# hdelan/MSc-HPC-Final-Project

Measured on AMD Instinct MI355X. Metric: lanczos_iterations_per_sec, higher is better.
Workload: dtype f64

## Files before the change

### msc-hpc-final-project_amd/__init__.py

```python
from __future__ import annotations

import ctypes
import os

import numpy as np

_HERE = os.path.dirname(os.path.abspath(__file__))
LIB_PATH = os.path.join(_HERE, "liblzx.so")
DBG_LIB_PATH = os.path.join(_HERE, "liblzx_dbg.so")
PRODUCT_OPTIONS = ("hub_entries", "propagation_blocking", "overlap_exchange", "sparse_exchange", "exchange_fp32",
                   "lazy_normalisation", "timing_marks_every", "reorthogonalise", "basis_fp32", "reference_order", "placement_trials",
                   "sharded_ingest", "operator")

SHAPE_OPTIONS = ("pb_reduce", "pb_target", "pb_unit", "pb_column_band", "pb_run_align", "pb_taper", "pb_dyn_share", "pb_carry_scan", "pb_scatter_nt", "pb_gather_grid", "pb_gather_nt", "spmv_wgs", "pb_group", "pb_group_force",
                 "narrow_slices", "tie_sort", "long_row", "item_len", "exchange_at_world_1", "isolated_rows", "unnormalised_basis", "fuse_staged", "start_vector_scan", "defer_finish",
                 "multi_row_chunk", "eig_basis_bytes", "solve_state_bytes", "solve_poll", "bfs_state_bytes", "tri_long_list", "tri_state_bytes", "core_long_row", "core_state_bytes",
                 "truss_long_row", "truss_state_bytes", "color_long_row", "lpa_group_row", "lpa_table_row", "lpa_state_bytes")

LZX_COLOR_TIES_BY_ID = 1

_u64p = ctypes.POINTER(ctypes.c_uint64)
_u32p = ctypes.POINTER(ctypes.c_uint32)
_i32p = ctypes.POINTER(ctypes.c_int32)
_u8p = ctypes.POINTER(ctypes.c_uint8)
_f64p = ctypes.POINTER(ctypes.c_double)
_h = ctypes.c_void_p
_hp = ctypes.POINTER(ctypes.c_void_p)


class LzxStats(ctypes.Structure):
    _fields_ = [("loop_ms", ctypes.c_double), ("spmv_ms", ctypes.c_double),
                ("spmv_ms_min", ctypes.c_double), ("vec_ms", ctypes.c_double),
                ("comm_ms", ctypes.c_double), ("iters", ctypes.c_uint32),
                ("spmv_kernels", ctypes.c_uint32), ("spmv_bytes", ctypes.c_uint64)]

    def as_dict(self):
        return {f: getattr(self, f) for f, _ in self._fields_}


class LzxGraphInfo(ctypes.Structure):
    _fields_ = [("n", ctypes.c_uint64), ("nnz", ctypes.c_uint64), ("max_degree", ctypes.c_uint64),
                ("rows_local", ctypes.c_uint64), ("nnz_local", ctypes.c_uint64),
                ("long_rows", ctypes.c_uint64), ("sell_padded", ctypes.c_uint64),
                ("pb_entries", ctypes.c_uint64), ("active_vertices", ctypes.c_uint64),
                ("exchange_slice", ctypes.c_uint64), ("hub_entries", ctypes.c_uint32), ("world", ctypes.c_uint32), ("rank", ctypes.c_uint32),
                ("reserved_", ctypes.c_uint32), ("pb_values", ctypes.c_uint64), ("pb_reduced_entries", ctypes.c_uint64),
                ("exchange_chunk0", ctypes.c_uint64), ("exchange_recv", ctypes.c_uint64),
                ("placement_tried", ctypes.c_uint32), ("placement_kept", ctypes.c_uint32), ("placement_us", ctypes.c_uint32 * 8)]

    def as_dict(self):
        d = {f: getattr(self, f) for f, _ in self._fields_}
        d["placement_us"] = list(d["placement_us"])[:d["placement_tried"]]
        return d


class LzxEigInfo(ctypes.Structure):
    _fields_ = [("converged", ctypes.c_uint32), ("restarts", ctypes.c_uint32), ("matvecs", ctypes.c_uint32), ("m", ctypes.c_uint32),
                ("loop_ms", ctypes.c_double), ("spmv_ms", ctypes.c_double), ("orth_ms", ctypes.c_double), ("host_ms", ctypes.c_double),
                ("norm_est", ctypes.c_double)]

    def as_dict(self):
        return {f: getattr(self, f) for f, _ in self._fields_}


class LzxSolveInfo(ctypes.Structure):
    _fields_ = [("iterations", ctypes.c_uint32), ("launched", ctypes.c_uint32), ("converged", ctypes.c_uint32), ("ns", ctypes.c_uint32),
                ("loop_ms", ctypes.c_double), ("spmv_ms", ctypes.c_double), ("vec_ms", ctypes.c_double), ("bnorm", ctypes.c_double)]

    def as_dict(self):
        return {f: getattr(self, f) for f, _ in self._fields_}


class LzxSolveMultiInfo(ctypes.Structure):
    _fields_ = [("iterations", ctypes.c_uint32), ("launched", ctypes.c_uint32), ("converged", ctypes.c_uint32), ("nb", ctypes.c_uint32),
                ("loop_ms", ctypes.c_double), ("spmv_ms", ctypes.c_double), ("vec_ms", ctypes.c_double), ("bnorm", ctypes.c_double * 16)]

    def as_dict(self):
        d = {f: getattr(self, f) for f, _ in self._fields_}
        d["bnorm"] = np.array(list(d["bnorm"])[:d["nb"]])
        return d


class LzxPagerankInfo(ctypes.Structure):
    _fields_ = [("iterations", ctypes.c_uint32), ("launched", ctypes.c_uint32), ("converged", ctypes.c_uint32), ("nd", ctypes.c_uint32),
                ("loop_ms", ctypes.c_double), ("spmv_ms", ctypes.c_double), ("vec_ms", ctypes.c_double), ("mass", ctypes.c_double * 16)]

    def as_dict(self):
        d = {f: getattr(self, f) for f, _ in self._fields_}
        d["mass"] = np.array(list(d["mass"])[:d["nd"]])
        return d


class LzxComponentsInfo(ctypes.Structure):
    _fields_ = [("n_components", ctypes.c_uint64), ("largest_size", ctypes.c_uint64), ("largest_label", ctypes.c_uint32),
                ("rounds", ctypes.c_uint32), ("loop_ms", ctypes.c_double), ("sweep_ms", ctypes.c_double)]

    def as_dict(self):
        return {f: getattr(self, f) for f, _ in self._fields_}


class LzxBfsInfo(ctypes.Structure):
    _fields_ = [("ns", ctypes.c_uint32), ("batches", ctypes.c_uint32), ("max_level", ctypes.c_uint32), ("sweeps", ctypes.c_uint32),
                ("loop_ms", ctypes.c_double), ("sweep_ms", ctypes.c_double)]

    def as_dict(self):
        return {f: getattr(self, f) for f, _ in self._fields_}


class LzxTrianglesInfo(ctypes.Structure):
    _fields_ = [("triangles", ctypes.c_uint64), ("wedges", ctypes.c_uint64), ("max_triangles", ctypes.c_uint64),
                ("oriented_entries", ctypes.c_uint64), ("oriented_max_degree", ctypes.c_uint32), ("reserved_", ctypes.c_uint32),
                ("avg_clustering", ctypes.c_double), ("loop_ms", ctypes.c_double), ("orient_ms", ctypes.c_double), ("count_ms", ctypes.c_double)]

    def as_dict(self):
        return {f: getattr(self, f) for f, _ in self._fields_ if f != "reserved_"}


class LzxCoreInfo(ctypes.Structure):
    _fields_ = [("main_core_size", ctypes.c_uint64), ("core0", ctypes.c_uint64), ("degeneracy", ctypes.c_uint32), ("levels", ctypes.c_uint32),
                ("rounds", ctypes.c_uint32), ("reserved_", ctypes.c_uint32), ("loop_ms", ctypes.c_double), ("peel_ms", ctypes.c_double)]

    def as_dict(self):
        return {f: getattr(self, f) for f, _ in self._fields_ if f != "reserved_"}


class LzxTrussInfo(ctypes.Structure):
    _fields_ = [("edges", ctypes.c_uint64), ("triangles", ctypes.c_uint64), ("main_truss_edges", ctypes.c_uint64),
                ("max_support", ctypes.c_uint32), ("max_truss", ctypes.c_uint32), ("levels", ctypes.c_uint32), ("rounds", ctypes.c_uint32),
                ("loop_ms", ctypes.c_double), ("support_ms", ctypes.c_double), ("peel_ms", ctypes.c_double)]

    def as_dict(self):
        return {f: getattr(self, f) for f, _ in self._fields_}


class LzxColorInfo(ctypes.Structure):
    _fields_ = [("colors", ctypes.c_uint32), ("rounds", ctypes.c_uint32), ("largest_class", ctypes.c_uint32), ("reserved_", ctypes.c_uint32),
                ("loop_ms", ctypes.c_double), ("color_ms", ctypes.c_double)]

    def as_dict(self):
        return {f: getattr(self, f) for f, _ in self._fields_ if f != "reserved_"}


class LzxCommunitiesInfo(ctypes.Structure):
    _fields_ = [("n_communities", ctypes.c_uint64), ("largest_size", ctypes.c_uint64), ("updates", ctypes.c_uint64),
                ("inner_entries", ctypes.c_uint64), ("entries", ctypes.c_uint64), ("sum_degree_sq", ctypes.c_uint64),
                ("largest_label", ctypes.c_uint32), ("sweeps", ctypes.c_uint32), ("colors", ctypes.c_uint32), ("color_rounds", ctypes.c_uint32),
                ("modularity", ctypes.c_double), ("loop_ms", ctypes.c_double), ("color_ms", ctypes.c_double), ("sweep_ms", ctypes.c_double)]

    def as_dict(self):
        return {f: getattr(self, f) for f, _ in self._fields_}


class LzxModularityInfo(ctypes.Structure):
    _fields_ = [("communities", ctypes.c_uint64), ("inner_entries", ctypes.c_uint64), ("entries", ctypes.c_uint64),
                ("sum_degree_sq", ctypes.c_uint64), ("loop_ms", ctypes.c_double)]

    def as_dict(self):
        return {f: getattr(self, f) for f, _ in self._fields_}


SYMBOLS = [
    ("lzx_create", ctypes.c_int, [_hp, ctypes.c_int]),
    ("lzx_destroy", None, [_h]),
    ("lzx_last_error", ctypes.c_char_p, []),
    ("lzx_comm_unique_id", ctypes.c_int, [_u8p]),
    ("lzx_comm_init_rank", ctypes.c_int, [_h, _u8p, ctypes.c_int, ctypes.c_int]),
    ("lzx_comm_init_local", ctypes.c_int, [_hp, ctypes.c_int]),
    ("lzx_create_group", ctypes.c_int, [_hp, ctypes.c_int, ctypes.POINTER(ctypes.c_int)]),
    ("lzx_comm_ipc_export", ctypes.c_int, [_h, _u8p]),
    ("lzx_comm_ipc_init", ctypes.c_int, [_h, _u8p, ctypes.c_int, ctypes.c_int]),
    ("lzx_set_graph_csr", ctypes.c_int, [_h, ctypes.c_uint64, ctypes.c_uint64, _u64p, _u32p]),
    ("lzx_set_graph_csr32", ctypes.c_int, [_h, ctypes.c_uint32, ctypes.c_uint32, _u32p, _u32p]),
    ("lzx_set_graph_edges", ctypes.c_int, [_h, ctypes.c_uint64, ctypes.c_uint64, _u32p, _u32p]),
    ("lzx_gen_graph", ctypes.c_int, [_h, ctypes.c_int, ctypes.c_uint32, ctypes.c_uint64, ctypes.c_uint64,
                                     ctypes.c_uint64, ctypes.c_uint32, ctypes.c_uint32, ctypes.c_uint32]),
    ("lzx_get_graph_info", ctypes.c_int, [_h, ctypes.POINTER(LzxGraphInfo)]),
    ("lzx_get_graph_csr", ctypes.c_int, [_h, _u64p, _u32p]),
    ("lzx_spmv_f64", ctypes.c_int, [_h, _f64p, _f64p]),
    ("lzx_spmv_f64_local", ctypes.c_int, [_hp, ctypes.c_int, _f64p, _f64p]),
    ("lzx_lanczos_f64", ctypes.c_int, [_h, _f64p, ctypes.c_uint32, _f64p, _f64p, _f64p, _f64p,
                                       ctypes.POINTER(LzxStats)]),
    ("lzx_lanczos_f64_local", ctypes.c_int, [_hp, ctypes.c_int, _f64p, ctypes.c_uint32, _f64p, _f64p, _f64p,
                                             _f64p, ctypes.POINTER(LzxStats)]),
    ("lzx_lanczos_prepare_f64", ctypes.c_int, [_h, _f64p, ctypes.c_uint32, _f64p]),
    ("lzx_lanczos_run", ctypes.c_int, [_h, ctypes.POINTER(LzxStats)]),
    ("lzx_lanczos_fetch_f64", ctypes.c_int, [_h, ctypes.c_uint32, _f64p, _f64p, _f64p]),
    ("lzx_lanczos_fetch_f64_local", ctypes.c_int, [_hp, ctypes.c_int, ctypes.c_uint32, _f64p, _f64p, _f64p]),
    ("lzx_lanczos_run_steps", ctypes.c_int, [_h, ctypes.c_uint32, ctypes.POINTER(LzxStats)]),
    ("lzx_lanczos_run_steps_local", ctypes.c_int, [_hp, ctypes.c_int, ctypes.c_uint32, ctypes.POINTER(LzxStats)]),
    ("lzx_lanczos_prepare_f64_local", ctypes.c_int, [_hp, ctypes.c_int, _f64p, ctypes.c_uint32, _f64p]),
    ("lzx_lanczos_progress", ctypes.c_int, [_h, _u32p, _u32p]),
    ("lzx_multout_change_f64", ctypes.c_int, [_h, _f64p, ctypes.c_uint32, _f64p]),
    ("lzx_multout_change_f64_local", ctypes.c_int, [_hp, ctypes.c_int, _f64p, ctypes.c_uint32, _f64p]),
    ("lzx_device_count", ctypes.c_int, [ctypes.POINTER(ctypes.c_int)]),
    ("lzx_sync", ctypes.c_int, [_h]),
    ("lzx_multout_f64", ctypes.c_int, [_h, _f64p, ctypes.c_uint32, _f64p]),
    ("lzx_multout_f64_local", ctypes.c_int, [_hp, ctypes.c_int, _f64p, ctypes.c_uint32, _f64p]),
    ("lzx_bench_spmv", ctypes.c_int, [_h, ctypes.c_uint32, _f64p, _f64p]),
    ("lzx_bench_stream", ctypes.c_int, [_h, ctypes.c_uint64, ctypes.c_uint32, _f64p, _f64p]),
    ("lzx_set_option", ctypes.c_int, [_h, ctypes.c_char_p, ctypes.c_int64]),
    ("lzx_lanczos_multi_f64", ctypes.c_int, [_h, ctypes.c_uint32, _f64p, ctypes.c_uint32, _f64p, _f64p, _u32p, _f64p, _f64p,
                                             ctypes.POINTER(LzxStats)]),
    ("lzx_multout_multi_f64", ctypes.c_int, [_h, ctypes.c_uint32, _f64p, ctypes.c_uint32, _f64p]),
    ("lzx_spmm_f64", ctypes.c_int, [_h, ctypes.c_uint32, _f64p, _f64p]),
    ("lzx_multi_release", ctypes.c_int, [_h]),
    ("lzx_probes_f64", ctypes.c_int, [_h, ctypes.c_uint64, ctypes.c_uint64, ctypes.c_uint32, _f64p]),
    ("lzx_lanczos_probes_f64", ctypes.c_int, [_h, ctypes.c_uint64, ctypes.c_uint64, ctypes.c_uint32, ctypes.c_uint32, ctypes.c_uint32,
                                              _f64p, _f64p, _u32p, ctypes.POINTER(LzxStats)]),
    ("lzx_probe_diag_f64", ctypes.c_int, [_h, _f64p, ctypes.c_uint32, _f64p]),
    ("lzx_eigsh_f64", ctypes.c_int, [_h, ctypes.c_uint32, ctypes.c_int, ctypes.c_uint32, ctypes.c_double, ctypes.c_uint32, _f64p,
                                     ctypes.c_uint64, _f64p, ctypes.c_uint32, _f64p, _f64p, _f64p, ctypes.POINTER(LzxEigInfo)]),
    ("lzx_solve_shifted_f64", ctypes.c_int, [_h, _f64p, ctypes.c_uint32, _f64p, ctypes.c_double, ctypes.c_uint32, _f64p, ctypes.c_uint32,
                                             _f64p, _u32p, _f64p, ctypes.POINTER(LzxSolveInfo)]),
    ("lzx_solve_multi_f64", ctypes.c_int, [_h, ctypes.c_uint32, _f64p, _f64p, ctypes.c_double, ctypes.c_uint32, _f64p, ctypes.c_uint32,
                                           _f64p, _u32p, _f64p, _u32p, ctypes.POINTER(LzxSolveMultiInfo)]),
    ("lzx_pagerank_f64", ctypes.c_int, [_h, _f64p, ctypes.c_uint32, _f64p, ctypes.c_double, ctypes.c_uint32, _f64p, _u32p, _f64p,
                                        ctypes.POINTER(LzxPagerankInfo)]),
    ("lzx_components", ctypes.c_int, [_h, _u32p, ctypes.POINTER(LzxComponentsInfo)]),
    ("lzx_set_graph_induced", ctypes.c_int, [_h, _h, _u8p, _u32p, _u64p]),
    ("lzx_bfs_multi", ctypes.c_int, [_h, ctypes.c_uint32, _u32p, _i32p, _f64p, _u64p, _u64p, _f64p, _u32p, ctypes.POINTER(LzxBfsInfo)]),
    ("lzx_betweenness_f64", ctypes.c_int, [_h, ctypes.c_uint32, _u32p, _f64p, ctypes.POINTER(LzxBfsInfo)]),
    ("lzx_triangles", ctypes.c_int, [_h, _u64p, _f64p, ctypes.POINTER(LzxTrianglesInfo)]),
    ("lzx_core_numbers", ctypes.c_int, [_h, _u32p, _u32p, ctypes.POINTER(LzxCoreInfo)]),
    ("lzx_truss", ctypes.c_int, [_h, _u32p, _u32p, _u32p, _u32p, ctypes.POINTER(LzxTrussInfo)]),
    ("lzx_color", ctypes.c_int, [_h, ctypes.c_uint64, ctypes.c_uint32, _u32p, ctypes.POINTER(LzxColorInfo)]),
    ("lzx_label_propagation", ctypes.c_int, [_h, ctypes.c_uint64, ctypes.c_uint32, ctypes.c_uint32, _u32p, ctypes.POINTER(LzxCommunitiesInfo)]),
    ("lzx_modularity", ctypes.c_int, [_h, _u32p, _f64p, ctypes.POINTER(LzxModularityInfo)]),
]

_LIB = None
_DBG_LIB = None


class LzxError(RuntimeError):
    pass


def _load(path: str, mode: int) -> ctypes.CDLL:
    if not os.path.exists(path):
        raise LzxError(f"{path} is missing: run __graft_entry__.build() (make -C {_HERE})")
    L = ctypes.CDLL(path, mode=mode)
    for name, res, args in SYMBOLS:
        fn = getattr(L, name)
        fn.restype = res
        fn.argtypes = args
    L.lzx_test_set_shape.restype = ctypes.c_int
    L.lzx_test_set_shape.argtypes = [_h, ctypes.c_char_p, ctypes.c_int64]
    L.lzx_test_get_shape.restype = ctypes.c_int
    L.lzx_test_get_shape.argtypes = [_h, ctypes.c_char_p, ctypes.POINTER(ctypes.c_int64)]
    L.lzx_test_allreduce_latency.restype = ctypes.c_int
    L.lzx_test_allreduce_latency.argtypes = [_h, ctypes.c_uint32, ctypes.POINTER(ctypes.c_double)]
    L.lzx_test_rank_row_sums.restype = ctypes.c_int
    L.lzx_test_rank_row_sums.argtypes = [_h, _f64p, _u32p, _u64p]
    L.lzx_test_sym_eig.restype = ctypes.c_int
    L.lzx_test_sym_eig.argtypes = [ctypes.c_uint32, _f64p, _f64p, _f64p]
    L.lzx_test_eig_ops.restype = ctypes.c_int
    L.lzx_test_eig_ops.argtypes = [_h, ctypes.c_uint32, ctypes.c_uint32, _f64p, _f64p, _f64p, _f64p, _f64p, _f64p, _f64p]
    return L


def lib(debug: bool = False) -> ctypes.CDLL:
    global _LIB, _DBG_LIB
    if debug:
        if _DBG_LIB is None:
            _DBG_LIB = _load(DBG_LIB_PATH, ctypes.RTLD_LOCAL)
        return _DBG_LIB
    if _LIB is None:
        _LIB = _load(LIB_PATH, ctypes.RTLD_GLOBAL)
    return _LIB


def _p(a, ty):
    return a.ctypes.data_as(ty)


def _check(rc: int, what: str, L=None):
    if rc != 0:
        raise LzxError(f"{what} failed ({rc}): {(L or lib()).lzx_last_error().decode(errors='replace')}")


OP_ADJACENCY = 0
OP_LAPLACIAN = 1


def _expm_coefficients(alpha, beta, x_norm, s):
    k = len(alpha)
    kb = k
    zero = np.flatnonzero(np.asarray(beta[:k - 1]) == 0.0)
    if zero.size:
        kb = int(zero[0]) + 1
    T = np.diag(np.asarray(alpha[:kb], dtype=np.float64))
    if kb > 1:
        T += np.diag(beta[:kb - 1], 1) + np.diag(beta[:kb - 1], -1)
    lam, V = np.linalg.eigh(T)
    t = np.zeros(k)
    t[:kb] = V @ (np.exp(s * lam) * (x_norm * V[0, :]))
    return t


PROBE_KEEP_BASIS = 1
EIG_LARGEST = 0
EIG_SMALLEST = 1
ERR_LIMIT = -6
PROBE_BATCH = 16


def _probe_ritz(alpha, beta, m):
    T = np.diag(np.asarray(alpha[:m], dtype=np.float64))
    if m > 1:
        T += np.diag(beta[:m - 1], 1) + np.diag(beta[:m - 1], -1)
    return np.linalg.eigh(T)


def _logsumexp(x):
    m = x.max()
    return m + np.log(np.sum(np.exp(x - m)))

# ... 886 lines not shown
```

### msc-hpc-final-project_amd/csrc/lzx_api.hip

```cpp
#include <algorithm>
#include <atomic>
#include <chrono>
#include <cmath>
#include <cstdlib>
#include <cstring>
#include <string>
#include <thread>

#include "lzx_internal.h"

static thread_local std::string g_err;

void lzx_set_error(const char *fmt, ...)
{
    char buf[1024];
    va_list ap;
    va_start(ap, fmt);
    vsnprintf(buf, sizeof buf, fmt, ap);
    va_end(ap);
    g_err = buf;
}

extern "C" const char *lzx_last_error(void) { return g_err.c_str(); }

extern "C" int lzx_create(lzx_handle *out, int device_id)
{
    if (!out) LZX_FAIL(LZX_ERR_ARG, "lzx_create: null out");
    *out = nullptr;
    int count = 0;
    LZX_HIP(hipGetDeviceCount(&count));
    if (device_id < 0 || device_id >= count)
        LZX_FAIL(LZX_ERR_ARG, "lzx_create: device %d not present (%d visible)", device_id, count);
    LZX_HIP(hipSetDevice(device_id));
    lzx_ctx *c = new (std::nothrow) lzx_ctx;
    if (!c) LZX_FAIL(LZX_ERR_NOMEM, "lzx_create: host allocation failed");
    c->device = device_id;
    hipDeviceProp_t prop;
    hipError_t e = hipGetDeviceProperties(&prop, device_id);
    if (e == hipSuccess) e = hipStreamCreateWithFlags(&c->stream, hipStreamNonBlocking);
    if (e == hipSuccess) e = hipEventCreate(&c->ev_a);
    if (e == hipSuccess) e = hipEventCreate(&c->ev_b);
    if (e == hipSuccess) e = hipEventCreateWithFlags(&c->ev_phase, hipEventDisableTiming);
    if (e == hipSuccess) e = hipStreamCreateWithFlags(&c->stream2, hipStreamNonBlocking);
    if (e == hipSuccess) e = hipEventCreateWithFlags(&c->ev_phase2, hipEventDisableTiming);
    if (e == hipSuccess) e = hipStreamCreateWithFlags(&c->stream3, hipStreamNonBlocking);
    if (e == hipSuccess) e = hipEventCreateWithFlags(&c->ev_fork, hipEventDisableTiming);
    if (e == hipSuccess) e = hipEventCreateWithFlags(&c->ev_join, hipEventDisableTiming);
    if (e == hipSuccess) e = hipEventCreateWithFlags(&c->ev_q, hipEventDisableTiming);
    if (e == hipSuccess) e = hipEventCreateWithFlags(&c->ev_c0, hipEventDisableTiming);
    if (e == hipSuccess) e = hipEventCreateWithFlags(&c->ev_c1, hipEventDisableTiming);
    if (e == hipSuccess) e = hipMalloc(reinterpret_cast<void **>(&c->d_scal), sizeof(double) * (8 + 64));
    if (e != hipSuccess) {
        lzx_set_error("lzx_create: %s", hipGetErrorString(e));
        lzx_destroy(c);
        return LZX_ERR_HIP;
    }
    c->cu_count = prop.multiProcessorCount > 0 ? prop.multiProcessorCount : 256;
    *out = c;
    return LZX_OK;
}

extern "C" void lzx_destroy(lzx_handle c)
{
    if (!c) return;
    (void)hipSetDevice(c->device);
    if (c->stream) (void)hipStreamSynchronize(c->stream);
    lzx_graph_release(c);
    lzx_comm_release(c);
    if (c->d_alpha) (void)hipFree(c->d_alpha);
    if (c->d_beta) (void)hipFree(c->d_beta);
    if (c->d_scal) (void)hipFree(c->d_scal);
    if (c->d_iso) (void)hipFree(c->d_iso);
    if (c->d_Qf) (void)hipFree(c->d_Qf);
    for (double *&r : c->d_ring) { if (r) (void)hipFree(r); r = nullptr; }
    for (double *&r : c->d_ymon) { if (r) (void)hipFree(r); r = nullptr; }
    for (hipEvent_t ev : c->ev_pool) (void)hipEventDestroy(ev);
    for (hipEvent_t ev : {c->ev_a, c->ev_b, c->ev_phase, c->ev_phase2, c->ev_fork, c->ev_join, c->ev_q, c->ev_c0, c->ev_c1})
        if (ev) (void)hipEventDestroy(ev);
    if (c->stream2) { (void)hipStreamSynchronize(c->stream2); (void)hipStreamDestroy(c->stream2); }
    if (c->stream3) { (void)hipStreamSynchronize(c->stream3); (void)hipStreamDestroy(c->stream3); }
    if (c->stream) (void)hipStreamDestroy(c->stream);
    delete c;
}

enum : unsigned { OPT_PRODUCT = 1, OPT_KNOB = 2, OPT_SHAPE = 4, OPT_LOOP = 8 };
struct Option {
    const char *name;
    int64_t lzx_ctx::*field;
    unsigned flags;
};
static const Option g_options[] = {
    {"hub_entries", &lzx_ctx::hub_opt, OPT_PRODUCT},
    {"propagation_blocking", &lzx_ctx::pb_opt, OPT_PRODUCT},
    {"overlap_exchange", &lzx_ctx::overlap_opt, OPT_PRODUCT},
    {"lazy_normalisation", &lzx_ctx::lazy_opt, OPT_PRODUCT},
    {"sparse_exchange", &lzx_ctx::sparse_opt, OPT_PRODUCT},
    {"exchange_fp32", &lzx_ctx::xfp32_opt, OPT_PRODUCT},
    {"timing_marks_every", &lzx_ctx::marks_every_opt, OPT_PRODUCT},
    {"reorthogonalise", &lzx_ctx::reorth_opt, OPT_PRODUCT | OPT_LOOP},
    {"basis_fp32", &lzx_ctx::qf32_opt, OPT_PRODUCT | OPT_LOOP},
    {"reference_order", &lzx_ctx::ref_order_opt, OPT_PRODUCT | OPT_LOOP},
    {"operator", &lzx_ctx::op_opt, OPT_PRODUCT | OPT_LOOP},
    {"placement_trials", &lzx_ctx::place_opt, OPT_PRODUCT},
    {"sharded_ingest", &lzx_ctx::shard_opt, OPT_PRODUCT},
    {"pb_reduce", &lzx_ctx::pb_reduce_opt, OPT_SHAPE | OPT_KNOB},
    {"pb_target", &lzx_ctx::pb_target_opt, OPT_SHAPE | OPT_KNOB},
    {"pb_unit", &lzx_ctx::pb_unit_opt, OPT_SHAPE | OPT_KNOB},
    {"pb_column_band", &lzx_ctx::pb_cb_opt, OPT_SHAPE | OPT_KNOB},
    {"pb_run_align", &lzx_ctx::pb_align_opt, OPT_SHAPE | OPT_KNOB},
    {"pb_taper", &lzx_ctx::pb_taper_opt, OPT_SHAPE | OPT_KNOB},
    {"pb_dyn_share", &lzx_ctx::pb_dyn_opt, OPT_SHAPE | OPT_KNOB},
    {"pb_carry_scan", &lzx_ctx::pb_scan_opt, OPT_SHAPE},
    {"pb_scatter_nt", &lzx_ctx::pb_scatter_nt_opt, OPT_SHAPE},
    {"pb_gather_grid", &lzx_ctx::pb_grid_cap_opt, OPT_SHAPE | OPT_KNOB},
    {"pb_gather_nt", &lzx_ctx::pb_gather_nt_opt, OPT_SHAPE | OPT_KNOB},
    {"spmv_wgs", &lzx_ctx::spmv_wgs_opt, OPT_SHAPE | OPT_KNOB},
    {"pb_group", &lzx_ctx::pb_group_opt, OPT_SHAPE | OPT_KNOB},
    {"pb_group_force", &lzx_ctx::pb_group_force_opt, OPT_SHAPE | OPT_KNOB},
    {"narrow_slices", &lzx_ctx::narrow_opt, OPT_SHAPE | OPT_KNOB},
    {"tie_sort", &lzx_ctx::tie_sort_opt, OPT_SHAPE | OPT_KNOB},
    {"long_row", &lzx_ctx::long_row_opt, OPT_SHAPE | OPT_KNOB},
    {"item_len", &lzx_ctx::item_opt, OPT_SHAPE | OPT_KNOB},
    {"exchange_at_world_1", nullptr, OPT_SHAPE | OPT_KNOB},
    {"isolated_rows", &lzx_ctx::iso_opt, OPT_SHAPE | OPT_KNOB},
    {"unnormalised_basis", &lzx_ctx::basis_u_opt, OPT_SHAPE | OPT_KNOB},
    {"fuse_staged", &lzx_ctx::fuse_opt, OPT_SHAPE | OPT_KNOB},
    {"start_vector_scan", &lzx_ctx::x0_scan_opt, OPT_SHAPE | OPT_KNOB},
    {"defer_finish", &lzx_ctx::defer_opt, OPT_SHAPE | OPT_KNOB},
    {"multi_row_chunk", &lzx_ctx::multi_chunk_opt, OPT_SHAPE},
    {"eig_basis_bytes", &lzx_ctx::eig_basis_cap_opt, OPT_SHAPE},
    {"solve_state_bytes", &lzx_ctx::solve_cap_opt, OPT_SHAPE},
    {"solve_poll", &lzx_ctx::solve_poll_opt, OPT_SHAPE},
    {"bfs_state_bytes", &lzx_ctx::bfs_cap_opt, OPT_SHAPE},
    {"tri_long_list", &lzx_ctx::tri_long_opt, OPT_SHAPE},
    {"tri_state_bytes", &lzx_ctx::tri_cap_opt, OPT_SHAPE},
    {"core_long_row", &lzx_ctx::core_long_opt, OPT_SHAPE},
    {"core_state_bytes", &lzx_ctx::core_cap_opt, OPT_SHAPE},
    {"truss_long_row", &lzx_ctx::truss_long_opt, OPT_SHAPE},
    {"truss_state_bytes", &lzx_ctx::truss_cap_opt, OPT_SHAPE},
    {"color_long_row", &lzx_ctx::color_long_opt, OPT_SHAPE},
    {"lpa_group_row", &lzx_ctx::lpa_group_opt, OPT_SHAPE},
    {"lpa_table_row", &lzx_ctx::lpa_table_opt, OPT_SHAPE},
    {"lpa_state_bytes", &lzx_ctx::lpa_cap_opt, OPT_SHAPE},
#ifdef LZX_DEBUG_KNOBS
    {"wgs_per_cu", &lzx_ctx::wgs_per_cu_opt, OPT_KNOB},
    {"nt_index_loads", &lzx_ctx::nt_opt, OPT_KNOB},
    {"side_stream", &lzx_ctx::side_opt, OPT_KNOB},
    {"pb_stamps", &lzx_ctx::pb_stamps_opt, OPT_KNOB},
    {"pb_order", &lzx_ctx::pb_order_opt, OPT_KNOB},
    {"spmv_deep", &lzx_ctx::deep_opt, OPT_KNOB},
    {"stage_burst", &lzx_ctx::burst_opt, OPT_KNOB},
    {"vec_blocks_per_cu", &lzx_ctx::vec_per_cu_opt, OPT_KNOB},
    {"pb_gather_waves", &lzx_ctx::pb_gwaves_opt, OPT_KNOB},
    {"phase_mask", &lzx_ctx::phase_mask_opt, OPT_KNOB},
#endif
};

static const Option *find_option(const char *name, unsigned accepted)
{
    for (const Option &o : g_options)
        if ((o.flags & accepted) && !strcmp(name, o.name)) return &o;
    return nullptr;
}

static void store_option(lzx_ctx *c, const Option &o, int64_t value)
{
    if (!o.field) c->force_multi = value > 0;
    else if (o.field == &lzx_ctx::shard_opt) c->shard_opt = value < 0 ? 0 : value;
    else c->*o.field = value;
}

extern "C" int lzx_set_option(lzx_handle c, const char *name, int64_t value)
{
    if (!c || !name) LZX_FAIL(LZX_ERR_ARG, "lzx_set_option: bad argument");
#ifdef LZX_DEBUG_KNOBS
    const Option *o = find_option(name, OPT_PRODUCT | OPT_KNOB);
#else
    const Option *o = find_option(name, OPT_PRODUCT);
#endif
    const bool loop_option = o && (o->flags & OPT_LOOP);
    if (o && o->field == &lzx_ctx::op_opt && value != LZX_OP_ADJACENCY && value != LZX_OP_LAPLACIAN)
        LZX_FAIL(LZX_ERR_ARG, "lzx_set_option: operator must be LZX_OP_ADJACENCY (0) or LZX_OP_LAPLACIAN (1), got %lld", (long long)value);
    if (c->d_row_ptr && !loop_option) LZX_FAIL(LZX_ERR_STATE, "options must be set before the graph is handed over");
    if (!o) LZX_FAIL(LZX_ERR_ARG, "lzx_set_option: unknown option '%s'", name);
    if (loop_option) c->k_prep = 0;
    store_option(c, *o, value);
    return LZX_OK;
}

extern "C" int lzx_test_set_shape(lzx_handle c, const char *name, int64_t value)
{
    if (!c || !name) LZX_FAIL(LZX_ERR_ARG, "lzx_test_set_shape: bad argument");
    if (c->d_row_ptr) LZX_FAIL(LZX_ERR_STATE, "shapes must be set before the graph is handed over");
    const Option *o = find_option(name, OPT_SHAPE);
    if (!o) LZX_FAIL(LZX_ERR_ARG, "lzx_test_set_shape: unknown shape '%s'", name);
    store_option(c, *o, value);
    return LZX_OK;
}

extern "C" int lzx_test_get_shape(lzx_handle c, const char *name, int64_t *value)
{
    if (!c || !name || !value) LZX_FAIL(LZX_ERR_ARG, "lzx_test_get_shape: bad argument");
    if (!strcmp(name, "gather_items_dealt")) *value = c->pb ? c->pb_n_static : 0;
    else if (!strcmp(name, "gather_items_drawn")) *value = c->pb ? c->pb_n_dyn : 0;
    else if (!strcmp(name, "gather_workgroups")) *value = c->pb ? c->pb_gather_grid : 0;
    else if (!strcmp(name, "placement_tried")) *value = c->place_tried;
    else if (!strcmp(name, "placement_kept")) *value = c->place_kept;
    else if (!strcmp(name, "start_vector_was_constant")) *value = c->x0_was_constant ? 1 : 0;
    else if (!strcmp(name, "finish_deferrable")) *value = c->pb && c->pb_defer_ok ? 1 : 0;
    else if (!strcmp(name, "finish_launched")) *value = c->pb && c->pb_finish_grid ? 1 : 0;
    else if (!strncmp(name, "placement_us_", 13) && name[13] >= '0' && name[13] <= '7' && !name[14]) *value = (int64_t)(c->place_ms[name[13] - '0'] * 1e3f);
    else LZX_FAIL(LZX_ERR_ARG, "lzx_test_get_shape: unknown shape '%s'", name);
    return LZX_OK;
}

extern "C" int lzx_test_allreduce_latency(lzx_handle c, uint32_t reps, double *us_each)
{
    if (!c || !us_each || reps == 0) LZX_FAIL(LZX_ERR_ARG, "lzx_test_allreduce_latency: bad argument");
    if (c->comm_kind < 2 || !lzx_exchanges(c)) LZX_FAIL(LZX_ERR_STATE, "lzx_test_allreduce_latency: needs a one-process-per-rank communicator");
    std::vector<lzx_ctx *> cs(1, c);
    LZX_HIP(hipSetDevice(c->device));
    LZX_HIP(hipMemsetAsync(c->d_scal, 0, sizeof(double) * 2, c->stream));
    for (u32 i = 0; i < 5; ++i) LZX_TRY(lzx_comm_allreduce_sum(cs, 0, 2));
    LZX_HIP(hipEventRecord(c->ev_a, c->stream));
    for (u32 i = 0; i < reps; ++i) LZX_TRY(lzx_comm_allreduce_sum(cs, 0, 2));
    LZX_HIP(hipEventRecord(c->ev_b, c->stream));
    LZX_HIP(hipStreamSynchronize(c->stream));
    LZX_TRY(lzx_comm_ipc_check(c));
    float ms = 0.f;
    LZX_HIP(hipEventElapsedTime(&ms, c->ev_a, c->ev_b));
    *us_each = (double)ms * 1e3 / reps;
    return LZX_OK;
}

extern "C" int lzx_test_rank_row_sums(lzx_handle c, double *v_local, uint32_t *layout_pos, uint64_t *n_loc_pad)
{
    if (!c || !v_local || !layout_pos || !n_loc_pad) LZX_FAIL(LZX_ERR_ARG, "lzx_test_rank_row_sums: bad argument");
    if (!c->d_row_ptr || !c->d_v) LZX_FAIL(LZX_ERR_STATE, "no graph has been handed over");
    double avg = 0.0;
    LZX_TRY(lzx_bench_spmv(c, 1, &avg, nullptr));
    LZX_HIP(hipSetDevice(c->device));
    LZX_HIP(hipMemcpy(v_local, c->d_v, sizeof(double) * c->n_loc_real, hipMemcpyDeviceToHost));
    LZX_HIP(hipMemcpy(layout_pos, c->d_gidx_of_old, sizeof(u32) * c->n, hipMemcpyDeviceToHost));
    *n_loc_pad = c->n_loc_pad;
    return LZX_OK;
}

static int gather_handles(lzx_handle h, std::vector<lzx_ctx *> &cs)
{
    if (!h) LZX_FAIL(LZX_ERR_ARG, "null handle");
    if (h->comm_kind == 1 && h->world > 1)
        LZX_FAIL(LZX_ERR_STATE, "handle belongs to an in-process communicator: use the *_local entry point");
    cs.assign(1, h);
    return LZX_OK;
}

static int gather_handles_local(lzx_handle *hs, int world, std::vector<lzx_ctx *> &cs)
{
    if (!hs || world < 1) LZX_FAIL(LZX_ERR_ARG, "bad handle list");
    cs.clear();
    for (int p = 0; p < world; ++p) {
        if (!hs[p]) LZX_FAIL(LZX_ERR_ARG, "null handle in list");
        if (hs[p]->world != world || hs[p]->rank != p || (world > 1 && hs[p]->comm_kind != 1))
            LZX_FAIL(LZX_ERR_STATE, "handles are not wired as an in-process communicator of %d", world);
        cs.push_back(hs[p]);
    }
    return LZX_OK;
}

static int check_graphs(std::vector<lzx_ctx *> &cs)
{
    for (lzx_ctx *c : cs) {
        if (!c->d_row_ptr || !c->d_v) LZX_FAIL(LZX_ERR_STATE, "no graph has been handed over");
        if (c->n != cs[0]->n || c->nnz != cs[0]->nnz) LZX_FAIL(LZX_ERR_STATE, "handles hold different graphs");
    }
    if (cs.size() > 1 && cs[0]->comm_kind == 1) LZX_TRY(lzx_comm_check_sparse_local(cs));
    return LZX_OK;
}

static int sync_all(std::vector<lzx_ctx *> &cs)
{
    for (lzx_ctx *c : cs) {
        LZX_HIP(hipSetDevice(c->device));
        LZX_HIP(hipStreamSynchronize(c->stream));
        LZX_HIP(hipStreamSynchronize(c->stream2));
        LZX_TRY(lzx_comm_ipc_check(c));
    }
    return LZX_OK;
}

template <class T>
static void drop(T *&buf, u32 &count)
{
    if (buf) (void)hipFree(buf);
    buf = nullptr;
    count = 0;
}

static int ensure_capacity(lzx_ctx *c, u32 k, bool qf32)
{
    LZX_HIP(hipSetDevice(c->device));
    if (k > c->k_cap) {
        drop(c->d_alpha, c->k_cap);
        drop(c->d_beta, c->k_cap);
        LZX_HIP(hipMalloc(reinterpret_cast<void **>(&c->d_alpha), sizeof(double) * k));
        LZX_HIP(hipMalloc(reinterpret_cast<void **>(&c->d_beta), sizeof(double) * k));
        c->k_cap = k;
    }
    if (qf32) {
        drop(c->d_Q, c->q_cols);
        if (k > c->qf_cols) {
            drop(c->d_Qf, c->qf_cols);
            LZX_HIP(hipMalloc(reinterpret_cast<void **>(&c->d_Qf), sizeof(float) * (size_t)k * c->ldq));
            c->qf_cols = k;
        }
        for (double *&r : c->d_ring)
            if (!r) LZX_HIP(hipMalloc(reinterpret_cast<void **>(&r), sizeof(double) * c->ldq));
        return LZX_OK;
    }
    drop(c->d_Qf, c->qf_cols);
    for (double *&r : c->d_ring) { if (r) (void)hipFree(r); r = nullptr; }
    if (k > c->q_cols) {
        drop(c->d_Q, c->q_cols);
        LZX_HIP(hipMalloc(reinterpret_cast<void **>(&c->d_Q), sizeof(double) * (size_t)k * c->ldq));
        c->q_cols = k;
    }
    return LZX_OK;
}

static bool loop_is_lazy(const lzx_ctx *c0)
{
    if (c0->reorth_opt > 0) return false;
    if (c0->ref_order_opt > 0) return false;
    if (c0->qf32_opt > 0 && c0->lazy_opt != 0) return true;
    return c0->lazy_opt > 0 || (c0->lazy_opt < 0 && (lzx_exchanges(c0) || c0->codes16));
}
static inline double *basis_col(const lzx_ctx *c, u32 j)
{
    return c->qf32 ? c->d_ring[j % 3] : c->d_Q + (size_t)j * c->ldq;
}

enum { CAT_NONE = 0, CAT_SPMV = 1, CAT_VEC = 2, CAT_COMM = 3 };
struct Marks {
    lzx_ctx *c;
    size_t used = 0;
    std::vector<int> cat;
    bool on = true;
    u32 sampled = 0;
    int begin_iteration(u32 j, u32 every)
    {
        on = every <= 1 || j % every == 0;
        if (on) ++sampled;
        return tick(CAT_NONE);
    }
    int tick(int category)
    {
        if (!on) return LZX_OK;
        LZX_HIP(hipSetDevice(c->device));
        if (used == c->ev_pool.size()) {
            hipEvent_t ev;
            LZX_HIP(hipEventCreate(&ev));
            c->ev_pool.push_back(ev);
        }
        LZX_HIP(hipEventRecord(c->ev_pool[used], c->stream));
        cat.push_back(category);
        ++used;
        return LZX_OK;
    }
};

static u64 spmv_algorithmic_bytes(const lzx_ctx *c)
{
    return 4ull * c->nnz_local + 4ull * ((u64)c->n_loc_real + 1) + 8ull * c->n + 8ull * c->n_loc_real;
}

struct X0Scan {
    bool constant = false, exact = false;
    double sum_sq = 0.0;
};
static X0Scan scan_start_vector(const double *x0, u64 n)
{
    X0Scan out;
    if (n == 0) return out;
    const u32 hw = std::max(1u, std::thread::hardware_concurrency());
    const u32 T = (u32)std::min<u64>(std::min<u32>(8u, hw), n / (1u << 18) + 1);
    std::vector<double> part(T, 0.0);
    std::atomic<bool> all_const{true}, all_int{true};
    const double first = x0[0];
    auto work = [&](u32 t) {
        const u64 a = n * t / T, b = n * (t + 1) / T;
        double acc[4] = {0.0, 0.0, 0.0, 0.0};
        bool cst = true, itg = true;
        for (u64 i0 = a; i0 < b; i0 += 4096) {
            const u64 i1 = std::min<u64>(b, i0 + 4096);
            u64 i = i0;
            for (; i + 4 <= i1; i += 4) {
#pragma unroll
                for (int u = 0; u < 4; ++u) {
                    const double v = x0[i + u];
                    cst &= v == first;
                    const bool small = std::fabs(v) <= 67108864.0;
                    itg &= small && (double)(int64_t)(small ? v : 0.0) == v;
                    acc[u] += v * v;
                }
            }
            for (; i < i1; ++i) {
                const double v = x0[i];
                cst &= v == first;
                const bool small = std::fabs(v) <= 67108864.0;
                itg &= small && (double)(int64_t)(small ? v : 0.0) == v;
                acc[0] += v * v;
            }
            if (!cst) all_const.store(false, std::memory_order_relaxed);
            if (!itg) all_int.store(false, std::memory_order_relaxed);
            if (!all_const.load(std::memory_order_relaxed) && !all_int.load(std::memory_order_relaxed)) return;
        }
        part[t] = (acc[0] + acc[1]) + (acc[2] + acc[3]);
    };
    {
        std::vector<std::thread> th;
        for (u32 t = 1; t < T; ++t) th.emplace_back(work, t);
        work(0);
        for (auto &t : th) t.join();
    }
    out.constant = all_const.load();
    if (all_int.load()) {
        double s = 0.0;
        for (u32 t = 0; t < T; ++t) s += part[t];
        if (s < 9007199254740992.0) {
            out.exact = true;
            out.sum_sq = s;
        }
    }
    return out;
}

static int lanczos_prepare(std::vector<lzx_ctx *> &cs, const double *x0, u32 k, double *x_norm_out)
{
    if (!x0 || k == 0) LZX_FAIL(LZX_ERR_ARG, "lzx_lanczos: bad argument");
    LZX_TRY(check_graphs(cs));
    lzx_ctx *c0 = cs[0];
    const u64 n = c0->n;
    const bool multi = lzx_exchanges(c0);
    const bool lazy = loop_is_lazy(c0);
    static const bool trace = getenv("LZX_TRACE_PREPARE") != nullptr;
    auto t_last = std::chrono::steady_clock::now();
    auto lap = [&](const char *what) {
        if (!trace) return;
        for (lzx_ctx *c : cs) { (void)hipSetDevice(c->device); (void)hipStreamSynchronize(c->stream); }
        const auto t = std::chrono::steady_clock::now();
        fprintf(stderr, "[lzx prepare] %-34s %8.3f ms\n", what, std::chrono::duration<double, std::milli>(t - t_last).count());
        t_last = t;
    };
    for (lzx_ctx *c : cs) {
        if (c->reorth_opt != c0->reorth_opt || c->qf32_opt != c0->qf32_opt) LZX_FAIL(LZX_ERR_STATE, "handles carry different loop options");
        if (c->qf32_opt > 0 && c->op_opt == LZX_OP_LAPLACIAN)
            LZX_FAIL(LZX_ERR_STATE, "basis_fp32 stores the unnormalised basis, which operator laplacian does not keep (its breakdown stop leaves beta = 0 to divide by)");
        if (c->qf32_opt > 0 && (!lazy || c->basis_u_opt == 0))
            LZX_FAIL(LZX_ERR_STATE, "basis_fp32 needs the lazy loop (not with lazy_normalisation = 0, not together with reorthogonalise)");
        if (c->ref_order_opt > 0 && (multi || cs.size() > 1))
            LZX_FAIL(LZX_ERR_STATE, "option reference_order runs on one rank");
        if (c->ref_order_opt > 0 && c->qf32_opt > 0)
            LZX_FAIL(LZX_ERR_STATE, "option reference_order keeps the fp64 basis (not together with basis_fp32)");
        if (c->op_opt != c0->op_opt) LZX_FAIL(LZX_ERR_STATE, "handles carry different operators");
        if (c->op_opt == LZX_OP_LAPLACIAN) LZX_TRY(lzx_ensure_degrees(c));
    }
    for (lzx_ctx *c : cs) {
        c->k_prep = 0;
        c->k_last = c->k_done = 0;
        c->ymon_valid = 0;
        c->qf32 = false;
    }
    const bool want_qf32 = c0->qf32_opt > 0;
    for (lzx_ctx *c : cs) LZX_TRY(ensure_capacity(c, k, want_qf32));
    for (lzx_ctx *c : cs) c->qf32 = want_qf32;
    lap("checks, basis sized");

    const X0Scan scan = c0->x0_scan_opt != 0 ? scan_start_vector(x0, n) : X0Scan{};
    lap("look at x0");
    double ss = scan.sum_sq;
    struct Joiner {
        std::thread t;
        ~Joiner() { if (t.joinable()) t.join(); }
    } norm_thread;
    if (!scan.exact)
        norm_thread.t = std::thread([&ss, x0, n]() {
            double acc = 0.0;
            for (u64 i = 0; i < n; ++i) acc += x0[i] * x0[i];
            ss = acc;
        });

    for (lzx_ctx *c : cs) {
        LZX_HIP(hipSetDevice(c->device));
        if (c->qf32) {
            for (double *r : c->d_ring) LZX_HIP(hipMemsetAsync(r, 0, sizeof(double) * c->ldq, c->stream));
        } else {
            LZX_HIP(hipMemsetAsync(c->d_Q, 0, sizeof(double) * c->ldq, c->stream));
            if (k > 1)
                LZX_HIP(hipMemset2DAsync(c->d_Q + c->ldq + c->n_loc_pad, sizeof(double) * c->ldq, 0, sizeof(double) * LZX_TAIL, k - 1, c->stream));
        }
        if (scan.constant) LZX_TRY(lzx_launch_fill(c, c->d_io, x0[0], n));
        else LZX_HIP(hipMemcpyAsync(c->d_io, x0, sizeof(double) * n, hipMemcpyHostToDevice, c->stream));
        c->x0_was_constant = scan.constant;
    }
    lap("clears + x0 on the device");
    if (norm_thread.t.joinable()) norm_thread.t.join();
    lap("serial norm chain (if any)");
    const double x_norm = std::sqrt(ss);
// ... 906 lines not shown
```

### msc-hpc-final-project_amd/csrc/lzx_internal.h

```cpp
#pragma once

#include <hip/hip_runtime.h>

#include <algorithm>
#include <chrono>
#include <cmath>
#include <cstdarg>
#include <cstdint>
#include <cstdio>
#include <vector>

#include "lzx.h"

typedef uint32_t u32;
typedef uint64_t u64;
typedef unsigned long long ull;

void lzx_set_error(const char *fmt, ...);

#define LZX_HIP(call)                                                                          \
    do {                                                                                       \
        hipError_t e_ = (call);                                                                \
        if (e_ != hipSuccess) {                                                                \
            lzx_set_error("%s:%d: %s -> %s", __FILE__, __LINE__, #call, hipGetErrorString(e_)); \
            return (e_ == hipErrorOutOfMemory) ? LZX_ERR_NOMEM : LZX_ERR_HIP;                   \
        }                                                                                      \
    } while (0)

#define LZX_TRY(call)              \
    do {                           \
        int rc_ = (call);          \
        if (rc_ != LZX_OK) return rc_; \
    } while (0)

#define LZX_FAIL(code, ...)       \
    do {                          \
        lzx_set_error(__VA_ARGS__); \
        return (code);            \
    } while (0)

static constexpr u32 LZX_SLICE = 64;
static constexpr u32 LZX_LONG_ROW = 128;
static constexpr u32 LZX_ITEM = 2048;
static constexpr u32 LZX_SPMV_BLOCK = 1024;
static constexpr u32 LZX_VEC_BLOCK = 256;
static constexpr u32 LZX_TAIL = 64;
static constexpr u32 LZX_PB_CB = 16384;
static constexpr u32 LZX_PB_CB_WIDE = 18432;
static constexpr u32 LZX_PB_RB = 1024;
static constexpr u32 LZX_PB_TARGET = 32768;
static constexpr u32 LZX_PB_ALIGN = 4;
static constexpr u32 LZX_PB_GATHER_BLOCK = 512;
static constexpr u32 LZX_PB_GROUP = 16384;
static constexpr unsigned long long LZX_PB_NT_BYTES = 128ull << 20;
static constexpr u32 LZX_PB_DYN_SHARE = 0;
static constexpr u32 LZX_PB_ITEM_GROUP = 0xfffffffeu, LZX_PB_ITEM_NONE = 0xfffffffdu;
static constexpr u64 LZX_PB_SLOT_LIMIT = (1ull << 32) - (1ull << 24);
static constexpr u32 LZX_PBR_STEP = 512;
static constexpr u32 LZX_PBR_MIN_RUN = 384;
static constexpr bool LZX_PB_SCATTER_NT = true;
static constexpr bool LZX_PB_CARRY_SCAN = true;

static constexpr int LZX_IPC_BUFS = 3;
struct lzx_ipc_state {
    void *win = nullptr;
    bool finegrained = false;
    void *peer_win[64] = {};
    bool win_opened[64] = {};
    u64 seq[2] = {0, 0};
    u64 mail_seq = 0, board_seq = 0;
    u64 deadline = 0;
    bool broken = false;
    struct Buf { void *mine = nullptr; size_t bytes = 0; void *peer[64] = {}; size_t peer_bytes[64] = {}; bool opened[64] = {}; } buf[LZX_IPC_BUFS];
    std::vector<u64> sx_dst_off;
};

struct lzx_ctx {
    int device = 0;
    int cu_count = 256;
    hipStream_t stream = nullptr;
    hipStream_t stream2 = nullptr;
    hipEvent_t ev_q = nullptr, ev_c0 = nullptr, ev_c1 = nullptr;
    hipStream_t stream3 = nullptr;
    hipEvent_t ev_fork = nullptr, ev_join = nullptr;
    hipEvent_t ev_phase2 = nullptr;
    hipEvent_t ev_a = nullptr, ev_b = nullptr;
    hipEvent_t ev_phase = nullptr;
    std::vector<hipEvent_t> ev_pool;
    hipEvent_t trace_ev[6] = {};
    bool trace = false;

    int world = 1, rank = 0;
    int comm_kind = 0;
    struct lzx_ipc_state *ipc = nullptr;
    bool publish_pending = false;
    lzx_ctx **peers = nullptr;
    void *nccl_comm = nullptr;
    double *d_mail = nullptr;
    bool mail_ok = false;
    void *nccl_comm2 = nullptr;
    bool agree_pending = false;

    u64 n = 0, nnz = 0, max_degree = 0;
    u64 *d_row_ptr = nullptr;
    u32 *d_col_idx = nullptr;
    struct lzx_key_source {
        int kind = -1;
        u32 scale = 0, ta = 0, tab = 0, tabc = 0;
        u64 n = 0, draws = 0, seed = 0;
        const u32 *d_src = nullptr, *d_dst = nullptr;
        u64 m = 0;
        const u64 *h_row_ptr = nullptr;
        const u32 *h_col_idx = nullptr;
    } shard;
    u32 *d_shard_deg = nullptr;
    bool sharded = false;
    int64_t shard_opt = 0;

    u32 n_loc_real = 0;
    u32 n_loc_pad = 0;
    u32 ldq = 0;
    u32 xs = 0;
    u32 xs0 = 0;
    int64_t sparse_opt = -1;
    bool sparse = false;
    u64 xc1 = 0;
    std::vector<u32> sx_recv_off;
    std::vector<u32> sx_send_off;
    std::vector<u64> sx_send_hash, sx_recv_hash;
    u32 *d_sx_send_idx = nullptr;
    double *d_sx_sendbuf = nullptr;
    u32 *d_sx_map = nullptr;
    int64_t xfp32_opt = -1;
    bool xfp32 = false;
    float *d_xf32_send = nullptr;
    float *d_xf32_full = nullptr;
    u64 n_active = 0;
    u32 rows_live = 0;
    u64 xlen = 0;
    u64 iolen = 0;
    u64 nnz_local = 0;
    u32 *d_gidx_of_old = nullptr;
    u32 hub = 0;
    int64_t hub_opt = -1;
    int64_t wgs_per_cu_opt = -1;
    int64_t nt_opt = -1;
    int64_t pb_opt = -1;
    int64_t overlap_opt = -1;
    bool overlap = false;
    u32 pb_units0 = 0;
    int64_t pb_target_opt = -1;
    int64_t pb_align_opt = -1;
    int64_t marks_every_opt = -1;
    bool force_multi = false;
    int64_t lazy_opt = -1;
    int64_t side_opt = -1;
    int64_t pb_cb_opt = -1;
    u32 pb_cb = LZX_PB_CB;
    int64_t pb_taper_opt = -1;
    int64_t pb_unit_opt = -1;
    int64_t pb_reduce_opt = -1;
    int64_t long_row_opt = -1;
    int64_t phase_mask_opt = 3;

    u32 n_long64 = 0;
    u32 n_long_true = 0;
    u32 n_slices = 0;
    u64 sell_elems = 0;
    u64 *d_slice_off = nullptr;
    u32 *d_slice_w = nullptr;
    u32 *d_slice_perm = nullptr;
    u32 ns_wide = 0, ns_w8 = 0, ns_w4 = 0;
    std::vector<u32> h_slice_w0;
    int64_t fuse_opt = -1;
    int64_t narrow_opt = -1;
    bool codes16 = false;
    u32 *d_sell_cols = nullptr;

    u32 n_items = 0;
    u64 long_elems = 0;
    u32 *d_long_cols = nullptr;
    u64 *d_item_beg = nullptr;
    u32 *d_item_len = nullptr;
    u32 *d_item_first = nullptr;
    double *d_long_partial = nullptr;

    bool pb = false;
    u32 hub_real = 0;
    u64 pb_entries = 0;
    u32 pb_nr = 0;
    u32 pb_units = 0;
    uint16_t *d_pb_lcol = nullptr;
    u32 *d_pb_dst = nullptr;
    uint16_t *d_pb_lrow = nullptr;
    double *d_pb_val = nullptr;
    u32 *d_pb_unit = nullptr;
    u32 *d_pb_row0 = nullptr;
    u32 *d_pb_rep = nullptr;
    u32 *d_pb_beg = nullptr;
    u32 *d_pb_items = nullptr;
    u32 *d_pb_multi = nullptr;
    double *d_pb_part = nullptr;
    uint8_t *d_pb_long_multi = nullptr;
    int64_t pb_stamps_opt = -1;
    unsigned long long *d_pb_gstamps = nullptr;
    int64_t tie_sort_opt = -1;
    int64_t item_opt = -1;
    int64_t vec_per_cu_opt = -1;
    int64_t burst_opt = -1;
    int64_t deep_opt = -1;
    int64_t pb_order_opt = -1;
    int64_t pb_group_opt = -1;
    int64_t pb_group_force_opt = -1;
    int64_t pb_gwaves_opt = -1;
    u32 pb_gather_block = 512;
    u32 pb_n_items = 0, pb_n_multi = 0;
    u32 pb_gather_grid = 0, pb_finish_grid = 0;
    uint4 *d_pb_mrow = nullptr;
    u32 pb_multi_limit = 0;
    bool pb_defer_ok = false, pb_deferring = false;
    int64_t defer_opt = -1;
    double *d_pb_item_dot = nullptr;
    u32 pb_n_static = 0, pb_n_dyn = 0;
    u32 *d_pb_gcounter = nullptr;
    int64_t spmv_wgs_opt = -1;
    int64_t pb_gather_nt_opt = -1;
    int64_t pb_grid_cap_opt = -1;
    int64_t pb_scatter_nt_opt = -1;
    int64_t pb_scan_opt = -1;
    int64_t pb_dyn_opt = -1;
    u64 pb_values = 0;
    u64 pbr_entries = 0;
    uint4 *d_pbr_code = nullptr;
    u32 *d_pbr_base = nullptr;
    u32 pbr_steps = 0;

    double *d_v = nullptr;
    u32 np2_last = 0;
    bool basis_u = false;
    int64_t basis_u_opt = -1;
    bool iso_on = false;
    bool iso_filled = false;
    u32 iso_cols_filled = 1;
    double *d_iso = nullptr;
    u32 iso_cap = 0;
    int64_t iso_opt = -1;
    double *d_u[2] = {nullptr, nullptr};
    double *d_Q = nullptr;
    u32 q_cols = 0;
    u32 k_last = 0;
    u32 k_prep = 0;
    u32 k_done = 0;
    int64_t reorth_opt = -1;
    int64_t ref_order_opt = -1;
    int64_t op_opt = 0;
    u32 *d_deg = nullptr;
    int64_t place_opt = -1;
    int64_t x0_scan_opt = -1;
    bool x0_was_constant = false;
    u32 place_tried = 0;
    float place_ms[8] = {};
    u32 place_kept = 0;
    int64_t qf32_opt = -1;
    bool qf32 = false;
    float *d_Qf = nullptr;
    u32 qf_cols = 0;
    double *d_ring[3] = {nullptr, nullptr, nullptr};
    double *d_ymon[2] = {nullptr, nullptr};
    u32 ymon_valid = 0;
    double *d_xbuf = nullptr;
    double *d_ybuf = nullptr;
    double *d_io = nullptr;
    double *d_partials = nullptr;
    double *d_partials2 = nullptr;
    double *d_partials3 = nullptr;
    u32 np_cap = 0;
    double *d_alpha = nullptr, *d_beta = nullptr;
    u32 k_cap = 0;
    double *d_scal = nullptr;

    u32 spmv_grid = 0;
    u32 fin_grid = 0;
    size_t spmv_lds = 0;

    struct lzx_multi_state *multi = nullptr;
    int64_t multi_chunk_opt = -1;
    int64_t eig_basis_cap_opt = -1;
    int64_t solve_cap_opt = -1;
    int64_t solve_poll_opt = -1;
    int64_t bfs_cap_opt = -1;
    int64_t tri_long_opt = -1;
    int64_t tri_cap_opt = -1;
    int64_t core_long_opt = -1;
    int64_t truss_long_opt = -1;
    int64_t truss_cap_opt = -1;
    int64_t core_cap_opt = -1;
    int64_t color_long_opt = -1;
    int64_t lpa_group_opt = -1;
    int64_t lpa_table_opt = -1;
    int64_t lpa_cap_opt = -1;
};

int lzx_graph_release(lzx_ctx *c);
int lzx_graph_prepare(lzx_ctx *c);

void lzx_multi_free(lzx_ctx *c, bool with_tables);

struct LzxCgsScratch {
    u32 G;
    double *part;
    double *h1, *h2;
    double *npart;
};
u32 lzx_cgs_grid(const lzx_ctx *c);
int lzx_cgs2(lzx_ctx *c, const double *Q, u32 J, double *w, const LzxCgsScratch &s, double *hsum = nullptr, u32 nw = 0);
int lzx_cgs_normalise(lzx_ctx *c, const double *w, double *q, const LzxCgsScratch &s, double *beta_out, double stop);
int lzx_cgs_orthonormalise(lzx_ctx *c, double *Q, u32 i, const LzxCgsScratch &s, double *beta_out);

static constexpr u32 LZX_SOLVE_MAX_NS = 16;
struct CgState {
    double rr;
    double alpha_prev, beta_prev;
    double curv;
    double zeta[LZX_SOLVE_MAX_NS];
    double zeta_prev[LZX_SOLVE_MAX_NS];
    u32 live;
    u32 done;
    u32 err_iter;
    u32 iters[LZX_SOLVE_MAX_NS];
};
struct CgMid {
    double alpha, curv;
    u32 err;
};
struct CgArgs {
    double *r, *p, *x0;
    const double *w;
    const u32 *deg;
    double *X, *P;
    u32 ldq, n;
    u32 ns;
    double sigma0, sgn;
    double tolb;
    double delta[LZX_SOLVE_MAX_NS];
    const double *pp;
    u32 npp;
    const double *pm;
    u32 npm;
    double *rr_part, *pp_part;
    CgState *st;
    CgMid *mid;
};
__device__ __forceinline__ double lzx_deg_weight(u32 d) { return d ? (double)d : 1.0; }

struct LzxCgRun {
    lzx_ctx *c = nullptr;
    double *d_V = nullptr;
    double *d_s = nullptr;
    std::vector<hipEvent_t> ev;
    void release()
    {
        if (c) {
            (void)hipSetDevice(c->device);
            (void)hipStreamSynchronize(c->stream);
        }
        if (d_V) (void)hipFree(d_V);
        if (d_s) (void)hipFree(d_s);
        for (hipEvent_t e : ev) (void)hipEventDestroy(e);
        d_V = d_s = nullptr;
        ev.clear();
    }
    ~LzxCgRun() { release(); }
};
struct LzxCgLoop {
    u32 launched = 0;
    double spmv_ms = 0.0, vec_ms = 0.0;
};
inline double lzx_ms_since(std::chrono::steady_clock::time_point t)
{
    return std::chrono::duration<double, std::milli>(std::chrono::steady_clock::now() - t).count();
}
std::vector<double> lzx_cg_distinct(const double *v, u32 n, bool descending, std::vector<u32> &slot);
int lzx_cg_multishift(LzxCgRun &run, CgArgs a, const double *b, double bb, bool lap, u32 maxiter, CgState &hs, LzxCgLoop &t);

template <typename State, typename Op, typename Vec, typename Over>
int lzx_cg_polled_loop(LzxCgRun &run, const State *d_st, State &hs, u32 maxiter, LzxCgLoop &t, Op op, Vec vec, Over over)
{
    lzx_ctx *c = run.c;
    const u32 poll = c->solve_poll_opt > 0 ? (u32)std::min<int64_t>(c->solve_poll_opt, 1024) : 16;
    for (u32 i = 0; i < 2 * poll + 1; ++i) {
        hipEvent_t ev;
        LZX_HIP(hipEventCreate(&ev));
        run.ev.push_back(ev);
    }
    u32 k = 0;
    LZX_HIP(hipEventRecord(run.ev[0], c->stream));
    for (u32 j = 0; j < maxiter; ++j) {
        LZX_TRY(op(j));
        LZX_HIP(hipEventRecord(run.ev[2 * k + 1], c->stream));
        LZX_TRY(vec(j));
        LZX_HIP(hipGetLastError());
        LZX_HIP(hipEventRecord(run.ev[2 * k + 2], c->stream));
        ++k;
        t.launched = j + 1;
        if (k == poll || t.launched == maxiter) {
            LZX_HIP(hipMemcpyAsync(&hs, d_st + (t.launched & 1), sizeof(hs), hipMemcpyDeviceToHost, c->stream));
            LZX_HIP(hipStreamSynchronize(c->stream));
            for (u32 i = 0; i < k; ++i) {
                float x = 0.f, y = 0.f;
                LZX_HIP(hipEventElapsedTime(&x, run.ev[2 * i], run.ev[2 * i + 1]));
                LZX_HIP(hipEventElapsedTime(&y, run.ev[2 * i + 1], run.ev[2 * i + 2]));
                t.spmv_ms += x;
                t.vec_ms += y;
            }
            k = 0;
            if (over(hs)) break;
            LZX_HIP(hipEventRecord(run.ev[0], c->stream));
        }
    }
    return LZX_OK;
}

int lzx_pb_prepare(lzx_ctx *c, const u32 *d_code, const u32 *d_old_of_local, const u32 *d_deg_local,
                   const u32 *d_nh_off, const std::vector<u32> &h_nh, u64 total);
void lzx_pb_release(lzx_ctx *c);
int lzx_pb_place_values(lzx_ctx *c);
struct SpmvArgs;
bool lzx_pb_can_fuse(const lzx_ctx *c);
int lzx_pb_launch(lzx_ctx *c, const double *x, const double *q_loc, double *v, double *partials, hipEvent_t chunk1_ready,
                  hipEvent_t v_ready, int phases = 3, const struct SpmvArgs *fuse = nullptr, u32 fuse_blocks = 0, bool *fused = nullptr);
u32 lzx_pb_partials(const lzx_ctx *c);

struct SpmvLaunch {
    const double *x;
    const double *q_loc;
    double *v;
    double *partials;
    hipEvent_t chunk1_ready = nullptr;
    bool live_rows_only = false;
};
int lzx_launch_spmv(lzx_ctx *c, const SpmvLaunch &a);
u32 lzx_spmv_partials(const lzx_ctx *c);
int lzx_launch_reduce(lzx_ctx *c, const double *partials, u32 np, double *out, int do_sqrt);
int lzx_launch_reduce2(lzx_ctx *c, const double *pa, u32 na, const double *pb, u32 nb, double *out2);
struct MailPeers { double *slot[64]; };
int lzx_launch_reduce2_mail(lzx_ctx *c, const double *pa, u32 na, const double *pb, u32 nb, const MailPeers &peers, u32 world);
int lzx_launch_iso_prepare(lzx_ctx *c, u32 k);
int lzx_launch_iso_fill(lzx_ctx *c, u32 k);
struct LazyDeferred {
    const uint4 *mrow = nullptr;
    u32 limit = 0;
    const double *part = nullptr;
    const u32 *item_first = nullptr;
    const double *long_partial = nullptr;
    const uint8_t *long_mode = nullptr;
    u32 n_long = 0;
};
int lzx_launch_lazy_update(lzx_ctx *c, const double *w, u32 w_rows, const double *u, const double *q_prev, const double *scal2, int first,
                           double *alpha_out, double *beta_out, double *q_out, double *u_next, double *partials_out, u32 *np_out, const double *prev_div = nullptr,
                           float *f32_next = nullptr, u32 mail_world = 0);
int lzx_launch_lazy_update_local(lzx_ctx *c, const double *w, u32 w_rows, const double *u, const double *q_prev, const double *pa, u32 na,
                                 const double *pb, u32 nb, int first, double *alpha_out, double *beta_out, double *q_out,
                                 double *u_next, double *partials_out, u32 *np_out, const double *prev_div = nullptr, float *f32_next = nullptr);
int lzx_launch_axpy_norm(lzx_ctx *c, double *v, const double *qj, const double *qjm1,
                         const double *partials_in, u32 np_in, double *alpha_out,
                         const double *beta_prev, double *partials_out, u32 *np_out);
int lzx_launch_scale(lzx_ctx *c, const double *v, double *q_next, const double *partials_in,
                     u32 np_in, double *beta_out, double stop = -1.0);
int lzx_ensure_degrees(lzx_ctx *c);
int lzx_launch_lap_apply(lzx_ctx *c, double *v, const double *q, double *partials, u32 np, u32 rows);
inline double lzx_stop_threshold(const lzx_ctx *c) { return c->op_opt == LZX_OP_LAPLACIAN ? ldexp(2.0 * (double)c->max_degree, -40) : -1.0; }
int lzx_launch_permute_in(lzx_ctx *c, const double *io_old_order, double *full, double scale);
int lzx_launch_fill(lzx_ctx *c, double *out, double value, u64 count);
int lzx_launch_permute_out(lzx_ctx *c, const double *full, double *io_old_order, const double *div = nullptr);
int lzx_launch_relayout(lzx_ctx *c, const double *io_layout, double *exchange_layout);
int lzx_launch_multout(lzx_ctx *c, const double *t_dev, u32 k, double *out_loc);
int lzx_launch_mgs_step(lzx_ctx *c, double *v, const double *q_m, const double *d_partials, u32 d_np, const double *d_scal,
                        const double *q_next, double *partials_out, u32 *np_out);
int lzx_launch_change(lzx_ctx *c, const double *y, const double *y_prev, double *out2);
int lzx_launch_ref_spmv(lzx_ctx *c, const double *x, double *y);
int lzx_launch_ref_dot(lzx_ctx *c, const double *a, const double *b, double *out);
int lzx_launch_widen_col(lzx_ctx *c, u32 col, double *out);

__host__ __device__ __forceinline__ double lzx_probe_value(u64 seed, u64 p, u64 i)
{
    u64 h = seed + 0x9E3779B97F4A7C15ull * ((p << 32) + i + 1);
    h ^= h >> 30;
    h *= 0xBF58476D1CE4E5B9ull;
    h ^= h >> 27;
    h *= 0x94D049BB133111EBull;
    h ^= h >> 31;
    return (h >> 63) ? -1.0 : 1.0;
}

inline u64 lzx_mix64(u64 z)
{
    z = (z ^ (z >> 30)) * 0xBF58476D1CE4E5B9ull;
    z = (z ^ (z >> 27)) * 0x94D049BB133111EBull;
    return z ^ (z >> 31);
}
void lzx_sx_check_message(const lzx_ctx *c, std::vector<u32> &mine);
int lzx_sx_check_pairs(const std::vector<u32> &all, u32 world);
inline bool lzx_exchanges(const lzx_ctx *c) { return c->world > 1 || (c->force_multi && c->comm_kind >= 2); }
int lzx_comm_allreduce_sum(std::vector<lzx_ctx *> &cs, u32 slot, u32 count = 1);
int lzx_comm_allgather(std::vector<lzx_ctx *> &cs, const double *const *src_loc, double *const *dst_full, size_t count,
                       bool on_stream2 = false, bool peers_idle = false);
int lzx_comm_sparse_chunk1(std::vector<lzx_ctx *> &cs, const double *const *slice_loc, bool peers_idle = false);
int lzx_launch_sx_pack(lzx_ctx *c, const double *slice_loc, hipStream_t st);
int lzx_comm_check_sparse(lzx_ctx *c);
int lzx_comm_check_sparse_local(std::vector<lzx_ctx *> &cs);
int lzx_comm_agree(lzx_ctx *c, bool ok, bool *all_ok);
int lzx_comm_ipc_publish(lzx_ctx *c, bool ok);
struct lzx_agree_guard {
    lzx_ctx *c;
    explicit lzx_agree_guard(lzx_ctx *c_) : c(c_) { if (c) c->agree_pending = c->comm_kind >= 2 && lzx_exchanges(c); }
    ~lzx_agree_guard()
    {
        if (c && c->agree_pending) {
            bool all = false;
            c->agree_pending = false;
            (void)lzx_comm_agree(c, false, &all);
        }
        if (c && c->publish_pending) {
            c->publish_pending = false;
            (void)lzx_comm_ipc_publish(c, false);
        }
    }
    lzx_agree_guard(const lzx_agree_guard &) = delete;
    lzx_agree_guard &operator=(const lzx_agree_guard &) = delete;
};
int lzx_comm_allgather_fp32(std::vector<lzx_ctx *> &cs, const double *const *slice_loc, bool peers_idle = false);
int lzx_launch_to_f32(lzx_ctx *c, const double *in, float *out, u64 count);
int lzx_launch_to_f64(lzx_ctx *c, const float *in, double *out, u64 count);
int lzx_comm_order(std::vector<lzx_ctx *> &cs, bool from_stream2, bool to_stream2);
bool lzx_comm_mail_usable(std::vector<lzx_ctx *> &cs);
int lzx_comm_mail_reduce2(std::vector<lzx_ctx *> &cs, u32 parity, bool first);
bool lzx_comm_fused_reduce2(const lzx_ctx *c);
int lzx_comm_reduce2_allreduce(lzx_ctx *c, const double *pa, u32 na, const double *pb, u32 nb);
// ... 12 lines not shown
```

### msc-hpc-final-project_amd/csrc/lzx_pb.hip

```cpp
#include <hipcub/hipcub.hpp>

#include <algorithm>
#include <cstdlib>
#include <queue>
#include <utility>

#include "lzx_internal.h"
#include "lzx_spmv_body.h"
#include "lzx_pb_shared.h"

namespace {

constexpr u32 KEY_LCOL_BITS = 15, KEY_LROW_SHIFT = KEY_LCOL_BITS, KEY_CBAND_SHIFT = KEY_LROW_SHIFT + 10, KEY_RBAND_SHIFT = KEY_CBAND_SHIFT + 16;
constexpr u32 KEY_LCOL_MASK = (1u << KEY_LCOL_BITS) - 1u;
__device__ __forceinline__ u64 pack_key(u32 rband, u32 cband, u32 lrow, u32 lcol)
{
    return ((u64)rband << KEY_RBAND_SHIFT) | ((u64)cband << KEY_CBAND_SHIFT) | ((u64)lrow << KEY_LROW_SHIFT) | (u64)lcol;
}

__global__ void __launch_bounds__(64)
k_pb_emit(const u64 *row_ptr, const u32 *col_idx, const u32 *code_of_old, const u32 *old_of_local,
          const u32 *deg_local, const u32 *nh_off, u32 n_rows, u32 hub, const u32 *band_row0, u32 nr, u32 cb, u64 *keys)
{
    const u32 lane = threadIdx.x;
    for (u32 l = blockIdx.x; l < n_rows; l += gridDim.x) {
        const u32 d = deg_local[l];
        u32 lo = 0, hi = nr;
        while (hi - lo > 1) {
            const u32 mid = (lo + hi) >> 1;
            if (band_row0[mid] <= l) lo = mid; else hi = mid;
        }
        const u32 R = lo, lrow = l - band_row0[lo];
        const u64 base = row_ptr[old_of_local[l]];
        u32 out = nh_off[l];
        for (u32 k0 = 0; k0 < d; k0 += 64) {
            const u32 k = k0 + lane;
            u32 cde = 0;
            bool keep = false;
            if (k < d) {
                cde = code_of_old[col_idx[base + k]];
                keep = cde >= hub;
            }
            const unsigned long long m = __ballot(keep);
            if (keep) {
                const u32 p = cde - hub;
                const u32 pre = __popcll(m & ((1ull << lane) - 1ull));
                keys[out + pre] = pack_key(R, p / cb, lrow, p % cb);
            }
            out += __popcll(m);
        }
    }
}

__global__ void k_pb_heads(const u64 *keys, u64 count, u32 *head)
{
    const u64 i = (u64)blockIdx.x * blockDim.x + threadIdx.x;
    if (i >= count) return;
    head[i] = (i == 0 || (keys[i] >> KEY_CBAND_SHIFT) != (keys[i - 1] >> KEY_CBAND_SHIFT)) ? 1u : 0u;
}

__global__ void k_pb_runstarts(const u32 *head, const u32 *runid_incl, u64 count, u32 *runstart)
{
    const u64 i = (u64)blockIdx.x * blockDim.x + threadIdx.x;
    if (i >= count) return;
    if (head[i]) runstart[runid_incl[i] - 1] = (u32)i;
}

__global__ void k_pb_run_format(const u32 *runstart, u32 nruns, u64 count, u32 min_run, uint8_t *fmt, u32 *epad)
{
    const u32 r = blockIdx.x * blockDim.x + threadIdx.x;
    if (r >= nruns) return;
    const u32 len = ((r + 1 < nruns) ? runstart[r + 1] : (u32)count) - runstart[r];
    const bool red = len >= min_run;
    fmt[r] = red ? 1 : 0;
    epad[r] = red ? ((len + LZX_PBR_STEP - 1) & ~(LZX_PBR_STEP - 1)) : 0u;
}

__global__ void k_pb_run_values(const u32 *runstart, u32 nruns, u64 count, const uint8_t *fmt, const u32 *estart,
                                const u32 *step_excl, u32 align, u32 *vcount)
{
    const u32 r = blockIdx.x * blockDim.x + threadIdx.x;
    if (r >= nruns) return;
    u32 n;
    if (fmt[r]) n = step_excl[estart[r + 1] / LZX_PBR_STEP] - step_excl[estart[r] / LZX_PBR_STEP];
    else n = ((r + 1 < nruns) ? runstart[r + 1] : (u32)count) - runstart[r];
    vcount[r] = (n + align - 1u) & ~(align - 1u);
}

__global__ void k_pb_place(const u64 *keys, const u32 *runid_incl, const u32 *runstart, const u32 *vpos, const uint8_t *fmt,
                           u64 count, uint16_t *prow, uint16_t *plcol, uint16_t *quad_cband)
{
    const u64 i = (u64)blockIdx.x * blockDim.x + threadIdx.x;
    if (i >= count) return;
    const u32 r = runid_incl[i] - 1;
    if (fmt[r]) return;
    const u32 pos = vpos[r] + ((u32)i - runstart[r]);
    const u64 k = keys[i];
    prow[pos] = (uint16_t)((k >> KEY_LROW_SHIFT) & 0x3ffu);
    plcol[pos] = (uint16_t)(k & KEY_LCOL_MASK);
    if ((pos & 3u) == 0) quad_cband[pos >> 2] = (uint16_t)((k >> KEY_CBAND_SHIFT) & 0xffffu);
}

__global__ void k_pb_fill16(uint16_t *a, u64 count, uint16_t v)
{
    const u64 i = (u64)blockIdx.x * blockDim.x + threadIdx.x;
    if (i < count) a[i] = v;
}

__global__ void k_pb_iota_widen(const uint16_t *in, u64 count, u32 *key, u32 *idx)
{
    const u64 i = (u64)blockIdx.x * blockDim.x + threadIdx.x;
    if (i < count) {
        key[i] = in[i];
        idx[i] = (u32)i;
    }
}

__global__ void k_pb_quads(const u32 *qsorted, const uint16_t *plcol, u64 nquads, uint2 *q_lcol, u32 *q_dst)
{
    const u64 j = (u64)blockIdx.x * blockDim.x + threadIdx.x;
    if (j >= nquads) return;
    const u32 q = qsorted[j];
    q_lcol[j] = *reinterpret_cast<const uint2 *>(plcol + (size_t)q * 4);
    q_dst[j] = q * 4u;
}

__global__ void k_pb_bounds_u32(const u32 *keys, u64 count, u32 targets, u32 *out)
{
    const u32 t = blockIdx.x * blockDim.x + threadIdx.x;
    if (t > targets) return;
    u64 lo = 0, hi = count;
    while (lo < hi) {
        const u64 mid = (lo + hi) >> 1;
        if (keys[mid] < t) lo = mid + 1; else hi = mid;
    }
    out[t] = (u32)lo;
}

__global__ void k_pb_bounds_u64(const u64 *keys, u64 count, u32 shift, u32 targets, u32 *out)
{
    const u32 t = blockIdx.x * blockDim.x + threadIdx.x;
    if (t > targets) return;
    u64 lo = 0, hi = count;
    while (lo < hi) {
        const u64 mid = (lo + hi) >> 1;
        if ((keys[mid] >> shift) < t) lo = mid + 1; else hi = mid;
    }
    out[t] = (u32)lo;
}

__global__ void k_pb_band_pos(const u32 *rstart, const u32 *runid_incl, const u32 *vpos, u32 nr, u64 count, u32 len, u32 *band_pos)
{
    const u32 R = blockIdx.x * blockDim.x + threadIdx.x;
    if (R > nr) return;
    const u32 i = rstart[R];
    band_pos[R] = i < count ? vpos[runid_incl[i] - 1] : len;
}

__device__ __forceinline__ u32 pb_group_position(u32 band_beg, u32 band_end, u32 g, u32 lane)
{
    const u32 whole = (band_end - band_beg) / 128u;
    if (g < whole * 2u) return band_beg + (g >> 1) * 128u + lane * 2u + (g & 1u);
    return band_beg + whole * 128u + (g - whole * 2u) * 64u + lane;
}

__global__ void __launch_bounds__(64)
k_pb_occurrence(const uint16_t *prow, const u32 *rstart_pad, const u32 *band_step0, u32 nr, uint8_t *occ, u32 *band_rep)
{
    const u32 step = blockIdx.x, lane = threadIdx.x;
    u32 lo = 0, hi = nr;
    while (hi - lo > 1) {
        const u32 mid = (lo + hi) >> 1;
        if (band_step0[mid] <= step) lo = mid; else hi = mid;
    }
    const u32 R = lo;
    const u32 i = pb_group_position(rstart_pad[R], rstart_pad[R + 1], step - band_step0[R], lane);
    const u32 r = i < rstart_pad[R + 1] ? (u32)prow[i] : 0xffffu;
    const bool live = r != 0xffffu;
    u32 k = 0;
    unsigned long long todo = __ballot(live);
    while (todo) {
        const int leader = __builtin_ctzll(todo);
        const u32 r0 = __shfl(r, leader, 64);
        const unsigned long long same = __ballot(live && r == r0);
        if (live && r == r0) k = __popcll(same & ((1ull << lane) - 1ull));
        todo &= ~same;
    }
    if (live) occ[i] = (uint8_t)k;
    u32 m = live ? k + 1 : 0;
    for (int o = 32; o > 0; o >>= 1) m = max(m, (u32)__shfl_xor((int)m, o, 64));
    if (lane == 0 && m > 1) atomicMax(&band_rep[R], m);
}

__global__ void k_pb_slots(const uint16_t *prow, const uint8_t *occ, const u32 *rstart_pad, const u32 *band_rep, u32 nr,
                           u64 count, uint16_t *lslot, const u32 no_rounds )
{
    const u64 p = (u64)blockIdx.x * blockDim.x + threadIdx.x;
    if (p >= count) return;
    const u32 r = prow[p];
    if (r == 0xffffu) {
        lslot[p] = 0;
        return;
    }
    u32 lo = 0, hi = nr;
    while (hi - lo > 1) {
        const u32 mid = (lo + hi) >> 1;
        if (rstart_pad[mid] <= p) lo = mid; else hi = mid;
    }
    const u32 rep = band_rep[lo];
    lslot[p] = (uint16_t)((r * rep + (occ[p] % rep)) | (no_rounds ? 0u : (occ[p] / rep) << 10));
}


__global__ void k_pbr_place(const u64 *keys, const u32 *runid_incl, const u32 *runstart, const u32 *estart, const uint8_t *fmt,
                            u64 count, uint16_t *rcode, uint16_t *rrow, uint16_t *step_cband, u32 *step_run)
{
    const u64 i = (u64)blockIdx.x * blockDim.x + threadIdx.x;
    if (i >= count) return;
    const u32 r = runid_incl[i] - 1;
    if (!fmt[r]) return;
    const u32 off = (u32)i - runstart[r];
    const u32 pos = estart[r] + off;
    const u64 k = keys[i];
    const u32 lrow = (u32)((k >> KEY_LROW_SHIFT) & 0x3ffu);
    const bool last = (off & (LZX_PBR_STEP - 1)) == LZX_PBR_STEP - 1 || i + 1 == count || runid_incl[i + 1] - 1 != r ||
                      (u32)((keys[i + 1] >> KEY_LROW_SHIFT) & 0x3ffu) != lrow;
    rcode[pos] = (uint16_t)((k & KEY_LCOL_MASK) | (last ? 0x8000u : 0u));
    rrow[pos] = (uint16_t)lrow;
    if ((off & (LZX_PBR_STEP - 1)) == 0) {
        step_cband[pos / LZX_PBR_STEP] = (uint16_t)((k >> KEY_CBAND_SHIFT) & 0xffffu);
        step_run[pos / LZX_PBR_STEP] = r;
    }
}

__global__ void k_pbr_step_base(const u32 *step_run, const u32 *estart, const u32 *step_excl, const u32 *vpos, u32 nsteps, u32 *step_base)
{
    const u32 s = blockIdx.x * blockDim.x + threadIdx.x;
    if (s >= nsteps) return;
    const u32 r = step_run[s];
    step_base[s] = vpos[r] + step_excl[s] - step_excl[estart[r] / LZX_PBR_STEP];
}

__global__ void __launch_bounds__(64) k_pbr_count(const uint4 *rcode, u32 *cnt)
{
    const uint4 c = rcode[(size_t)blockIdx.x * 64 + threadIdx.x];
    u32 n = __popc(c.x & 0x80008000u) + __popc(c.y & 0x80008000u) + __popc(c.z & 0x80008000u) + __popc(c.w & 0x80008000u);
    for (int o = 32; o > 0; o >>= 1) n += (u32)__shfl_xor((int)n, o, 64);
    if (threadIdx.x == 0) cnt[blockIdx.x] = n;
}

__global__ void __launch_bounds__(64) k_pbr_rows(const uint4 *rcode, const uint4 *rrow, const u32 *step_base, uint16_t *prow)
{
    const uint4 c = rcode[(size_t)blockIdx.x * 64 + threadIdx.x];
    const uint4 r = rrow[(size_t)blockIdx.x * 64 + threadIdx.x];
    u32 base = step_base[blockIdx.x];
#pragma unroll
    for (int e = 0; e < 8; ++e) {
        const bool f = pbr_flag(c, e) != 0;
        const unsigned long long m = __ballot(f);
        if (f) prow[base + lanes_below(m)] = (uint16_t)pbr_half(r, e);
        base += (u32)__popcll(m);
    }
}

__global__ void __launch_bounds__(64) k_pbr_steps(const u32 *ssorted, const uint4 *rcode, const u32 *step_base, uint4 *scode, u32 *sbase)
{
    const u32 s = ssorted[blockIdx.x];
    scode[(size_t)blockIdx.x * 64 + threadIdx.x] = rcode[(size_t)s * 64 + threadIdx.x];
    if (threadIdx.x == 0) sbase[blockIdx.x] = step_base[s];
}

template <int CTRL, int ROW_MASK>
__device__ __forceinline__ double dpp_f64(double v)
{
    const int lo = __builtin_amdgcn_update_dpp(0, __double2loint(v), CTRL, ROW_MASK, 0xf, false);
    const int hi = __builtin_amdgcn_update_dpp(0, __double2hiint(v), CTRL, ROW_MASK, 0xf, false);
    return __hiloint2double(hi, lo);
}
template <int CTRL, int ROW_MASK>
__device__ __forceinline__ u32 dpp_u32(u32 v)
{
    return (u32)__builtin_amdgcn_update_dpp(0, (int)v, CTRL, ROW_MASK, 0xf, false);
}
__device__ __forceinline__ double pbr_carry_scan(double tail, bool has)
{
    double P = tail;
    u32 F = has ? 1u : 0u;
#define LZX_SCAN_STEP(CTRL, RM)                          \
    {                                                    \
        const double ps = dpp_f64<CTRL, RM>(P);          \
        const u32 fs = dpp_u32<CTRL, RM>(F);             \
        P += F ? 0.0 : ps;                               \
        F |= fs;                                         \
    }
    const unsigned long long nh = ~__ballot(has);
    if (nh) {
        LZX_SCAN_STEP(0x111, 0xf)
        const unsigned long long q2 = nh & (nh << 1);
        if (q2) {
            LZX_SCAN_STEP(0x112, 0xf)
            const unsigned long long q4 = q2 & (q2 << 2);
            if (q4) {
                LZX_SCAN_STEP(0x114, 0xf)
                const unsigned long long q8 = q4 & (q4 << 4);
                if (q8) LZX_SCAN_STEP(0x118, 0xf)
            }
        }
        if (nh & ((1ull << 16) | (1ull << 48))) LZX_SCAN_STEP(0x142, 0xa)
        if (nh & ((1ull << 32) | (1ull << 48))) LZX_SCAN_STEP(0x143, 0xc)
    }
#undef LZX_SCAN_STEP
    return dpp_f64<0x138, 0xf>(P);
}

template <bool NTC> __device__ __forceinline__ uint4 sld(const uint4 *p)
{
    typedef unsigned int u4v __attribute__((ext_vector_type(4)));
    if (!NTC) return *p;
    const u4v t = __builtin_nontemporal_load(reinterpret_cast<const u4v *>(p));
    return make_uint4(t.x, t.y, t.z, t.w);
}
template <bool NTC> __device__ __forceinline__ uint2 sld(const uint2 *p)
{
    typedef unsigned int u2v __attribute__((ext_vector_type(2)));
    if (!NTC) return *p;
    const u2v t = __builtin_nontemporal_load(reinterpret_cast<const u2v *>(p));
    return make_uint2(t.x, t.y);
}
template <bool NTC> __device__ __forceinline__ u32 sld(const u32 *p) { return NTC ? __builtin_nontemporal_load(p) : *p; }

template <u32 CB, bool SCAN, bool NTC>
__device__ __forceinline__ void
pb_scatter_body(const u32 *unit, const uint4 *scode, const u32 *sbase, const uint2 *q_lcol, const u32 *q_dst,
                const double *__restrict__ x, u64 xlen, double *val, const u32 ublock)
{
    extern __shared__ __attribute__((aligned(16))) double tile[];
    const u32 band = unit[5 * ublock];
    const u64 base = (u64)band * CB;
    if (base + CB <= xlen) {
        const double2 *src = reinterpret_cast<const double2 *>(x + base);
        double2 t[CB / 2048];
#pragma unroll
        for (u32 u = 0; u < CB / 2048; ++u) t[u] = src[threadIdx.x + u * 1024];
#pragma unroll
        for (u32 u = 0; u < CB / 2048; ++u) reinterpret_cast<double2 *>(tile)[threadIdx.x + u * 1024] = t[u];
    } else {
        for (u32 j = threadIdx.x; j < CB; j += 1024) tile[j] = base + j < xlen ? x[base + j] : 0.0;
    }
    if (threadIdx.x < 2) tile[CB + threadIdx.x] = 0.0;
    if (!SCAN)
        for (u32 j = threadIdx.x; j < 16 * 66; j += 1024) tile[CB + 2 + j] = 0.0;
    __syncthreads();
    const u32 lane = threadIdx.x & 63;
    const u32 wv = (u32)__builtin_amdgcn_readfirstlane((int)(threadIdx.x >> 6));
    constexpr u32 W = 1024 / 64;

    {
        const u32 beg = unit[5 * ublock + 1], end = unit[5 * ublock + 2];
        double *carry = tile + CB + 2 + wv * 66;
        auto body_scan = [&](const uint4 &c, u32 pos) {
            const u32 w[4] = {c.x, c.y, c.z, c.w};
            double xv[8];
            bool f[8];
#pragma unroll
            for (int e = 0; e < 8; ++e) {
                xv[e] = tile[pbr_half(c, e) & 0x7fffu];
                f[e] = (e & 1) ? ((int)w[e >> 1] < 0) : ((w[e >> 1] & 0x8000u) != 0u);
            }
            const bool has = ((c.x | c.y | c.z | c.w) & 0x80008000u) != 0u;
            double pv[8];
            double run = 0.0;
#pragma unroll
            for (int e = 0; e < 8; ++e) {
                run += xv[e];
                pv[e] = run;
                run = f[e] ? 0.0 : run;
            }
            double carry = pbr_carry_scan(run, has);
            double *out = val + pos;
            u32 done = 0;
#pragma unroll
            for (int e = 0; e < 8; ++e) {
                const unsigned long long m = __ballot(f[e]);
                if (m) {
                    if (f[e]) {
                        out[done + lanes_below(m)] = pv[e] + carry;
                        carry = 0.0;
                    }
                    done += (u32)__popcll(m);
                }
            }
        };
        auto body_lds = [&](const uint4 &c, u32 pos) {
            double xv[8];
#pragma unroll
            for (int e = 0; e < 8; ++e) xv[e] = tile[pbr_half(c, e) & 0x7fffu];
            u32 ends = 0;
#pragma unroll
            for (int e = 0; e < 8; ++e) ends |= pbr_flag(c, e) << e;
            const bool has = ends != 0;
            const int last = has ? 31 - __clz((int)ends) : -1;
            double tail = 0.0;
#pragma unroll
            for (int e = 0; e < 8; ++e)
                if (e > last) tail += xv[e];
            double s;
            if (SCAN) {
                const double carried = pbr_carry_scan(tail, has);
                s = has ? carried : 0.0;
            } else {
                const unsigned long long holders = __ballot(has);
                const unsigned long long before = holders & ((1ull << lane) - 1ull);
                const u32 from = before ? 64u - (u32)__clzll((long long)before) : 0u;
                atomicAdd(&carry[has ? lane + 1 : from], tail);
                __builtin_amdgcn_wave_barrier();
                s = has ? carry[from] : 0.0;
                __builtin_amdgcn_wave_barrier();
                if (has) carry[from] = 0.0;
            }
            double *out = val + pos;
            u32 done = 0;
#pragma unroll
            for (int e = 0; e < 8; ++e) {
                const bool f = (ends >> e) & 1u;
                s += xv[e];
                const unsigned long long m = __ballot(f);
                if (m) {
                    if (f) {
                        out[done + lanes_below(m)] = s;
                        s = 0.0;
                    }
                    done += (u32)__popcll(m);
                }
            }
        };
        u32 s = beg + wv;
        for (; s + 3 * W < end; s += 4 * W) {
            uint4 c[4];
            u32 b[4];
#pragma unroll
            for (int u = 0; u < 4; ++u) {
                c[u] = sld<NTC>(scode + (size_t)(s + u * W) * 64 + lane);
                b[u] = (u32)__builtin_amdgcn_readfirstlane((int)sbase[s + u * W]);
            }
#pragma unroll
            for (int u = 0; u < 4; ++u) {
                if (SCAN) body_scan(c[u], b[u]);
                else body_lds(c[u], b[u]);
            }
        }
        if (s < end) {
            uint4 c[3];
            u32 b[3];
#pragma unroll
            for (int u = 0; u < 3; ++u) {
                if (s + u * W < end) {
                    c[u] = sld<NTC>(scode + (size_t)(s + u * W) * 64 + lane);
                    b[u] = (u32)__builtin_amdgcn_readfirstlane((int)sbase[s + u * W]);
                }
            }
#pragma unroll
            for (int u = 0; u < 3; ++u)
                if (s + u * W < end) {
                    if (SCAN) body_scan(c[u], b[u]);
                    else body_lds(c[u], b[u]);
                }
        }
    }

    {
        const u32 beg = unit[5 * ublock + 3], end = unit[5 * ublock + 4];
        for (u32 blk = beg + wv * 256u; blk < end; blk += W * 256u) {
        const u32 wend = blk + 256u < end ? blk + 256u : end;
        u32 j = blk + lane;
        for (; j + 3 * 64 < wend; j += 4 * 64) {
            uint2 c[4];
            u32 d[4];
#pragma unroll
            for (int u = 0; u < 4; ++u) {
                c[u] = sld<NTC>(q_lcol + j + u * 64);
                d[u] = sld<NTC>(q_dst + j + u * 64);
            }
#pragma unroll
            for (int u = 0; u < 4; ++u) {
                double2 lo, hi;
                lo.x = tile[c[u].x & 0xffffu];
                lo.y = tile[c[u].x >> 16];
                hi.x = tile[c[u].y & 0xffffu];
                hi.y = tile[c[u].y >> 16];
                double2 *out = reinterpret_cast<double2 *>(val + d[u]);
                out[0] = lo;
                out[1] = hi;
            }
        }
        if (wend < blk + 256u) {
            uint2 c[3];
            u32 d[3];
#pragma unroll
            for (int u = 0; u < 3; ++u) {
                const u32 jj = j + u * 64 < wend ? j + u * 64 : blk;
                c[u] = sld<NTC>(q_lcol + jj);
                d[u] = sld<NTC>(q_dst + jj);
            }
#pragma unroll
            for (int u = 0; u < 3; ++u) {
                if (j + u * 64 < wend) {
                    double2 lo, hi;
                    lo.x = tile[c[u].x & 0xffffu];
                    lo.y = tile[c[u].x >> 16];
                    hi.x = tile[c[u].y & 0xffffu];
                    hi.y = tile[c[u].y >> 16];
                    double2 *out = reinterpret_cast<double2 *>(val + d[u]);
                    out[0] = lo;
                    out[1] = hi;
                }
            }
        }
        }
    }
}

template <u32 CB, bool SCAN, bool NTC>
__global__ void __launch_bounds__(1024)
k_pb_scatter(const u32 *unit, const uint4 *scode, const u32 *sbase, const uint2 *q_lcol, const u32 *q_dst,
             const double *__restrict__ x, u64 xlen, double *val)
{
    pb_scatter_body<CB, SCAN, NTC>(unit, scode, sbase, q_lcol, q_dst, x, xlen, val, blockIdx.x);
}

template <u32 CB, bool SCAN, bool NTC>
__global__ void __launch_bounds__(1024)
k_pb_scatter_spmv(const u32 *unit, u32 n_units, const uint4 *scode, const u32 *sbase, const uint2 *q_lcol, const u32 *q_dst,
                  const double *__restrict__ x, u64 xlen, double *val, const SpmvArgs a, const u32 spmv_first)
{
    const u32 spmv_blocks = gridDim.x - n_units;
    if (spmv_first) {
        if (blockIdx.x < spmv_blocks) spmv_body<2, false>(a, blockIdx.x, spmv_blocks);
        else pb_scatter_body<CB, SCAN, NTC>(unit, scode, sbase, q_lcol, q_dst, x, xlen, val, blockIdx.x - spmv_blocks);
        return;
    }
    if (blockIdx.x < n_units) pb_scatter_body<CB, SCAN, NTC>(unit, scode, sbase, q_lcol, q_dst, x, xlen, val, blockIdx.x);
    else spmv_body<2, false>(a, blockIdx.x - n_units, spmv_blocks);
}

template <bool NT>
__device__ __forceinline__ double2 gld_val2(const double *p)
{
    typedef double d2v __attribute__((ext_vector_type(2)));
    const d2v t = NT ? __builtin_nontemporal_load(reinterpret_cast<const d2v *>(p)) : *reinterpret_cast<const d2v *>(p);
    return make_double2(t.x, t.y);
}
template <bool NT>
__device__ __forceinline__ u32 gld_slot2(const uint16_t *p)
{
    return NT ? __builtin_nontemporal_load(reinterpret_cast<const u32 *>(p)) : *reinterpret_cast<const u32 *>(p);
}

__device__ __forceinline__ void tile_add2(double *ytile, u32 lane, u32 sv, double ax, double ay)
{
    const u32 s0 = sv & 0xffffu, s1 = sv >> 16;
    const u32 spare = LZX_PB_RB + lane;
    atomicAdd(&ytile[min(s0, spare)], ax);
    atomicAdd(&ytile[min(s1, spare)], ay);
    if (__ballot((s0 | s1) >= 1024u)) {
        u32 r = 1;
        unsigned long long more;
        do {
            if ((s0 >> 10) == r) atomicAdd(&ytile[s0 & 1023u], ax);
            if ((s1 >> 10) == r) atomicAdd(&ytile[s1 & 1023u], ay);
            more = __ballot((s0 >> 10) > r || (s1 >> 10) > r);
            ++r;
        } while (more);
    }
}
__device__ __forceinline__ void tile_add1(double *ytile, u32 lane, u32 s0, double a)
{
    atomicAdd(&ytile[min(s0, LZX_PB_RB + lane)], a);
    if (__ballot(s0 >= 1024u)) {
        u32 r = 1;
        unsigned long long more;
        do {
            if ((s0 >> 10) == r) atomicAdd(&ytile[s0 & 1023u], a);
            more = __ballot((s0 >> 10) > r);
            ++r;
        } while (more);
    }
}

template <bool STAMP, bool NT, bool NOSLOT = false>
__global__ void __launch_bounds__(LZX_PB_GATHER_BLOCK, 4)
k_pb_gather(const uint4 *items, u32 n_static, u32 n_dyn, u32 *counter, double *item_dot, const u32 *band_row0, const u32 *band_rep,
            const u32 *band_beg, const uint16_t *lslot, const double *val, double *v, const double *__restrict__ q_loc, double *part,
            double *partials, unsigned long long *stamps, const u32 probe_l2g, const u32 *item_first, const double *long_partial,
            const uint8_t *long_mode, const u32 n_long)
{
    auto close_split_rows = [&](u32 row0, u32 rows, u32 first, u32 stride, double &dot, u32 mode) {
        if (row0 >= n_long) return;
        const u32 lim = min(rows, n_long - row0);
        for (u32 j = first; j < lim; j += stride) {
            const u32 row = row0 + j;
            if (long_mode[row] != mode) continue;
            double sl = 0.0;
            for (u32 it = item_first[row]; it < item_first[row + 1]; ++it) sl += long_partial[it];
            if (mode == 0) v[row] += sl;
            dot += sl * q_loc[row];
        }
    };
    unsigned long long t_start = 0, t_mark = 0, t_zero = 0, t_stream = 0, t_bar = 0, t_fold = 0, n_vals = 0;
    u32 n_it = 0;
#define GSTAMP(acc) do { if (STAMP) { const unsigned long long t_ = wall_clock64(); acc += t_ - t_mark; t_mark = t_; } } while (0)
    unsigned long long c_start = 0;
    if (STAMP) { t_start = t_mark = wall_clock64(); c_start = __builtin_amdgcn_s_memtime(); }
    extern __shared__ __attribute__((aligned(16))) double lds[];
    constexpr u32 WAVES = LZX_PB_GATHER_BLOCK / 64;
    constexpr u32 TILE = LZX_PB_RB + 64;
    const u32 tid = threadIdx.x, lane = tid & 63;
    const u32 wv = (u32)__builtin_amdgcn_readfirstlane((int)(tid >> 6));
    double *ytile = lds + (size_t)wv * TILE;
    double *wsum = lds + (size_t)WAVES * TILE;
    double dot = 0.0;
    constexpr u32 MAXR = 16;
    u32 *lrec = reinterpret_cast<u32 *>(wsum + WAVES);
    u32 *ltick = lrec + MAXR * WAVES * 8;
    auto uni = [](u32 x) { return (u32)__builtin_amdgcn_readfirstlane((int)x); };
    u32 it0 = blockIdx.x;
    bool dyn = false;
    for (;;) {
    if (!dyn && it0 >= n_static) dyn = true;
    if (dyn && n_dyn == 0) break;
    __syncthreads();
    u32 base = it0, stride = gridDim.x, limit = n_static, nrounds = MAXR, ticket = 0;
    if (dyn) {
        if (tid == 0) *ltick = atomicAdd(counter, 1u);
        __syncthreads();
        ticket = uni(*ltick);
        if (ticket >= n_dyn) {
            if (tid == 0 && ticket == n_dyn + gridDim.x - 1) *counter = 0u;
            break;
        }
        base = n_static + ticket; stride = 0; limit = base + 1; nrounds = 1;
        __syncthreads();
    }
    for (u32 t = tid; t < nrounds * WAVES; t += LZX_PB_GATHER_BLOCK) {
        const u32 r = t / WAVES, w = t % WAVES;
        const u32 it = base + r * stride;
        u32 *o = lrec + (size_t)t * 8;
        uint4 item = make_uint4(0u, 0u, 0u, LZX_PB_ITEM_NONE);
        if (it < limit) item = items[it];
        o[5] = item.w;
        o[6] = 0u;
        o[7] = 1u;
        if (item.w == LZX_PB_ITEM_GROUP) {
            const u32 y = item.y, split = y <= 1u ? 8u : y <= 2u ? 4u : y <= 4u ? 2u : 1u;
            o[7] = split;
            if (w < y * split) {
                const u32 R = item.x + w % y;
                const u32 r0 = band_row0[R];
                o[0] = band_beg[R]; o[1] = band_beg[R + 1]; o[2] = r0; o[3] = band_row0[R + 1] - r0; o[4] = band_rep[R]; o[6] = 1u + (w / y) + (y << 8);
            }
        } else if (item.w != LZX_PB_ITEM_NONE) {
            const u32 R = item.x;
            const u32 r0 = band_row0[R];
            o[0] = item.y; o[1] = item.z; o[2] = r0; o[3] = band_row0[R + 1] - r0; o[4] = band_rep[R];
            o[6] = 1u + (item.y == band_beg[R] ? 2u : 0u);
        }
    }
    __syncthreads();
    const double dot_static = dot;
    if (dyn) dot = 0.0;
    for (u32 rr = 0; rr < nrounds && base + rr * stride < limit; ++rr) {
        const u32 *rec = lrec + ((size_t)rr * WAVES + wv) * 8;
        const u32 r_beg = uni(rec[0]), r_end = uni(rec[1]), r_row0 = uni(rec[2]), r_rows = uni(rec[3]), r_rep = uni(rec[4]);
        const u32 item_w = uni(rec[5]), r_live = uni(rec[6]), r_split = uni(rec[7]);
        if (item_w == LZX_PB_ITEM_NONE) continue;
        if (item_w == LZX_PB_ITEM_GROUP) {
            __syncthreads();
            const u32 part = r_live ? (r_live & 0xffu) - 1u : 0u, gy = r_live >> 8;
            if (r_live) {
                const u32 rows = r_rows, rep = r_rep;
                const u32 beg = r_beg, end = r_end;
                const u32 slots = rows * rep;
                for (u32 j = lane; j < slots; j += 64) ytile[j] = 0.0;
                __builtin_amdgcn_wave_barrier();
                if (STAMP && part == 0) { ++n_it; n_vals += end - beg; }
                GSTAMP(t_zero);
                const u32 blocks = (end - beg) / 128u;
                u32 kb = part;
                for (; kb + 7 * r_split < blocks; kb += 8 * r_split) {
                    double2 av[8];
                    u32 sv[8];
#pragma unroll
                    for (int u = 0; u < 8; ++u) {
                        const u32 p = beg + (kb + u * r_split) * 128u + lane * 2;
                        av[u] = gld_val2<NT>(val + p);
                        sv[u] = NOSLOT ? (lane * 2u) | ((lane * 2u + 1u) << 16) : gld_slot2<NT>(lslot + p);
                    }
#pragma unroll
                    for (int u = 0; u < 8; ++u) tile_add2(ytile, lane, sv[u], av[u].x, av[u].y);
                }
                {
                    double2 av[7];
                    u32 sv[7];
                    double tv[2] = {0.0, 0.0};
                    u32 ts[2] = {0u, 0u};
#pragma unroll
                    for (int u = 0; u < 7; ++u) {
                        if (kb + u * r_split < blocks) {
                            const u32 p = beg + (kb + u * r_split) * 128u + lane * 2;
                            av[u] = gld_val2<NT>(val + p);
                            sv[u] = NOSLOT ? (lane * 2u) | ((lane * 2u + 1u) << 16) : gld_slot2<NT>(lslot + p);
                        }
                    }
#pragma unroll
                    for (int u = 0; u < 2; ++u) {
                        const u32 i = beg + blocks * 128u + lane + u * 64;
                        if (part == 0 && i < end) {
                            tv[u] = val[i];
                            ts[u] = lslot[i];
                        }
                    }
#pragma unroll
                    for (int u = 0; u < 7; ++u) {
                        if (kb + u * r_split < blocks) tile_add2(ytile, lane, sv[u], av[u].x, av[u].y);
                    }
                    tile_add1(ytile, lane, ts[0], tv[0]);
                    __builtin_amdgcn_wave_barrier();
                    tile_add1(ytile, lane, ts[1], tv[1]);
                }
#ifdef LZX_DEBUG_KNOBS
                if (probe_l2g) {
                    const double *xt = q_loc + 16384;
                    for (u32 i = lane; i < probe_l2g; i += 64 * 8) {
                        double t8[8];
                        u32 h8[8];
#pragma unroll
                        for (int u = 0; u < 8; ++u) {
                            h8[u] = ((i + u * 64) * 2654435761u + r_row0 * 40503u) >> 7;
                            t8[u] = xt[h8[u] & 0x1ffffu];
                        }
#pragma unroll
                        for (int u = 0; u < 8; ++u)
                            if (i + u * 64 < probe_l2g) tile_add1(ytile, lane, (h8[u] >> 17) % slots, t8[u]);
                    }
                }
#endif
                __builtin_amdgcn_wave_barrier();
                GSTAMP(t_stream);
            }
            if (r_split > 1u) __syncthreads();
            if (r_live && part == 0u) {
                const u32 row0 = r_row0, rows = r_rows, rep = r_rep;
                for (u32 j0 = lane; j0 < rows; j0 += 256) {
                    double vv[4], qq[4];
#pragma unroll
                    for (int u = 0; u < 4; ++u) {
                        const u32 j = j0 + u * 64;
                        vv[u] = j < rows ? v[row0 + j] : 0.0;
                        qq[u] = j < rows ? q_loc[row0 + j] : 0.0;
                    }
#pragma unroll
                    for (int u = 0; u < 4; ++u) {
                        const u32 j = j0 + u * 64;
                        if (j < rows) {
                            double y = 0.0;
                            for (u32 pt = 0; pt < r_split; ++pt)
                                for (u32 t = 0; t < rep; ++t) y += ytile[(size_t)pt * gy * TILE + j * rep + t];
                            v[row0 + j] = vv[u] + y;
                            dot += y * qq[u];
                        }
                    }
                }
                close_split_rows(row0, rows, lane, 64u, dot, 0u);
                GSTAMP(t_fold);
            }
            continue;
        }
        const u32 beg = r_beg, end = r_end;
        if (STAMP) { ++n_it; n_vals += end - beg; }
        const u32 row0 = r_row0, rows = r_rows;
        if (rows == 1) {
            double acc = 0.0;
            u32 i = beg + tid;
            for (; i + 7 * LZX_PB_GATHER_BLOCK < end; i += 8 * LZX_PB_GATHER_BLOCK) {
                double a[8];
#pragma unroll
                for (int u = 0; u < 8; ++u) a[u] = val[i + u * LZX_PB_GATHER_BLOCK];
#pragma unroll
                for (int u = 0; u < 8; ++u) acc += a[u];
            }
            for (; i < end; i += LZX_PB_GATHER_BLOCK) acc += val[i];
            acc = wave_sum_pb(acc);
            __syncthreads();
            if (lane == 0) wsum[wv] = acc;
            __syncthreads();
            if (tid == 0) {
                double t = 0.0;
                for (u32 w = 0; w < WAVES; ++w) t += wsum[w];
                if (item_w == 0xffffffffu) {
                    double vr = v[row0] + t;
                    dot += t * q_loc[row0];
                    if (row0 < n_long && long_mode[row0] == 0) {
                        double sl = 0.0;
                        for (u32 it = item_first[row0]; it < item_first[row0 + 1]; ++it) sl += long_partial[it];
                        vr += sl;
                        dot += sl * q_loc[row0];
                    }
                    v[row0] = vr;
                } else {
                    part[item_w] = t;
                    dot += t * q_loc[row0];
                    if ((r_live & 2u) && row0 < n_long && long_mode[row0] == 1) {
                        double sl = 0.0;
                        for (u32 it = item_first[row0]; it < item_first[row0 + 1]; ++it) sl += long_partial[it];
                        dot += sl * q_loc[row0];
                    }
                }
            }
            continue;
        }
        const u32 rep = r_rep;
        const u32 slots = rows * rep;
        __syncthreads();
        for (u32 j = lane; j < slots; j += 64) ytile[j] = 0.0;
        __builtin_amdgcn_wave_barrier();
        GSTAMP(t_zero);
        const u32 blocks = (end - beg) / 128u;
        u32 kb = wv;
        for (; kb + 7 * WAVES < blocks; kb += 8 * WAVES) {
            double2 av[8];
            u32 sv[8];
#pragma unroll
            for (int u = 0; u < 8; ++u) {
                const u32 p = beg + (kb + u * WAVES) * 128u + lane * 2;
                av[u] = gld_val2<NT>(val + p);
                sv[u] = NOSLOT ? (lane * 2u) | ((lane * 2u + 1u) << 16) : gld_slot2<NT>(lslot + p);
            }
#pragma unroll
            for (int u = 0; u < 8; ++u) tile_add2(ytile, lane, sv[u], av[u].x, av[u].y);
        }
        for (; kb < blocks; kb += WAVES) {
            const u32 p = beg + kb * 128u + lane * 2;
            const double2 a = gld_val2<NT>(val + p);
            const u32 s = NOSLOT ? (lane * 2u) | ((lane * 2u + 1u) << 16) : gld_slot2<NT>(lslot + p);
            tile_add2(ytile, lane, s, a.x, a.y);
        }
        if (wv == 0)
            for (u32 i0 = beg + blocks * 128u; i0 < end; i0 += 64) {
                const u32 i = i0 + lane;
                tile_add1(ytile, lane, i < end ? (u32)lslot[i] : 0u, i < end ? val[i] : 0.0);
            }
        GSTAMP(t_stream);
        __syncthreads();
        GSTAMP(t_bar);
        if (item_w == 0xffffffffu) {
            for (u32 j0 = tid; j0 < rows; j0 += 2 * LZX_PB_GATHER_BLOCK) {
                double vv[2], qq[2];
#pragma unroll
                for (int u = 0; u < 2; ++u) {
                    const u32 j = j0 + u * LZX_PB_GATHER_BLOCK;
                    vv[u] = j < rows ? v[row0 + j] : 0.0;
                    qq[u] = j < rows ? q_loc[row0 + j] : 0.0;
                }
#pragma unroll
                for (int u = 0; u < 2; ++u) {
                    const u32 j = j0 + u * LZX_PB_GATHER_BLOCK;
                    if (j < rows) {
                        double y = 0.0;
                        for (u32 w = 0; w < WAVES; ++w)
                            for (u32 t = 0; t < rep; ++t) y += lds[(size_t)w * TILE + j * rep + t];
                        v[row0 + j] = vv[u] + y;
                        dot += y * qq[u];
                    }
                }
            }
            close_split_rows(row0, rows, tid, LZX_PB_GATHER_BLOCK, dot, 0u);
        } else {
            for (u32 j = tid; j < rows; j += LZX_PB_GATHER_BLOCK) {
                double y = 0.0;
                for (u32 w = 0; w < WAVES; ++w)
                    for (u32 t = 0; t < rep; ++t) y += lds[(size_t)w * TILE + j * rep + t];
                part[item_w + j] = y;
                dot += y * q_loc[row0 + j];
            }
            if (r_live & 2u) close_split_rows(row0, rows, tid, LZX_PB_GATHER_BLOCK, dot, 1u);
        }
        GSTAMP(t_fold);
    }
    if (dyn) {
        const double idot = wave_sum_pb(dot);
        dot = dot_static;
        __syncthreads();
        if (lane == 0) wsum[wv] = idot;
        __syncthreads();
        if (tid == 0) {
            double t = 0.0;
            for (u32 w = 0; w < WAVES; ++w) t += wsum[w];
            item_dot[ticket] = t;
        }
    } else {
        it0 += MAXR * gridDim.x;
    }
    }
    if (STAMP && tid == 0) {
        unsigned long long *o = stamps + 8 * (size_t)blockIdx.x;
        o[0] = t_start; o[1] = wall_clock64(); o[2] = t_zero; o[3] = t_stream; o[4] = t_bar; o[5] = t_fold;
        o[6] = (unsigned long long)n_it | ((__builtin_amdgcn_s_memtime() - c_start) << 16);
        o[7] = n_vals;
    }
#undef GSTAMP
    dot = wave_sum_pb(dot);
    __syncthreads();
    if (lane == 0) wsum[wv] = dot;
    __syncthreads();
    if (tid == 0) {
        double s = 0.0;
        for (u32 i = 0; i < WAVES; ++i) s += wsum[i];
        partials[blockIdx.x] = s;
    }
}

__global__ void __launch_bounds__(LZX_VEC_BLOCK)
k_pb_finish(const uint4 *multi , u32 n_multi, const double *part,
            const u32 *item_first, const double *long_partial, const uint8_t *long_mode, u32 n_long, double *v,
            const double *q_loc, double *partials, const double *item_dot, u32 n_item_dot)
{
    __shared__ double sh[4];
    const u32 t = blockIdx.x * LZX_VEC_BLOCK + threadIdx.x;
    double dot = 0.0;
    const double idot = t < n_item_dot ? item_dot[t] : 0.0;
    if (t < n_multi) {
        const uint4 m = multi[t];
        const u32 row = m.x;
        double s = 0.0;
        for (u32 k = 0; k < m.z; ++k) s += part[m.y + (size_t)k * m.w];
        if (row < n_long)
            for (u32 it = item_first[row]; it < item_first[row + 1]; ++it) s += long_partial[it];
        v[row] += s;
    } else if (t - n_multi < n_long && long_mode[t - n_multi] == 2) {
        const u32 r = t - n_multi;
        double s = 0.0;
        for (u32 it = item_first[r]; it < item_first[r + 1]; ++it) s += long_partial[it];
        v[r] += s;
        dot = s * q_loc[r];
    }
    dot += idot;
    dot = wave_sum_pb(dot);
    if ((threadIdx.x & 63) == 0) sh[threadIdx.x >> 6] = dot;
    __syncthreads();
    if (threadIdx.x == 0) partials[blockIdx.x] = ((sh[0] + sh[1]) + sh[2]) + sh[3];
}



}

int lzx_pb_place_values(lzx_ctx *c)
{
    c->place_tried = c->place_kept = 0;
    const size_t bytes = sizeof(double) * (c->pb_values + 8);
    const u32 trials = (u32)std::min<u64>(c->place_opt >= 0 ? (u64)std::min<int64_t>(c->place_opt, 7) : 2ull,
                                          c->place_opt >= 0 ? 7ull : std::max<u64>(1, (16ull << 30) / std::max<size_t>(bytes, 1)));
    if (!c->pb || !c->d_pb_val || trials == 0 || bytes < LZX_PB_NT_BYTES) return LZX_OK;
    LZX_HIP(hipSetDevice(c->device));
    const bool multi = lzx_exchanges(c);
    SpmvLaunch l{multi ? c->d_xbuf : c->d_ybuf, c->d_ybuf + (size_t)c->rank * c->n_loc_pad, c->d_v, c->d_partials};
    auto time_spmv = [&](float *best) -> int {
        *best = 1e30f;
        for (int r = 0; r < 4; ++r) {
            LZX_HIP(hipEventRecord(c->ev_a, c->stream));
            LZX_TRY(lzx_launch_spmv(c, l));
            LZX_HIP(hipEventRecord(c->ev_b, c->stream));
            LZX_HIP(hipEventSynchronize(c->ev_b));
            float ms = 0.f;
            LZX_HIP(hipEventElapsedTime(&ms, c->ev_a, c->ev_b));
            if (r > 0 && ms < *best) *best = ms;
        }
        return LZX_OK;
    };
    double *best_buf = c->d_pb_val, *loser = nullptr;
    u32 kept = 0;
    int rc = time_spmv(&c->place_ms[0]);
    for (u32 t = 1; rc == LZX_OK && t <= trials; ++t) {
        size_t free_b = 0, total_b = 0;
        if (hipMemGetInfo(&free_b, &total_b) != hipSuccess || free_b < 2 * bytes + (4ull << 30)) break;
        double *fresh = nullptr;
        if (hipMalloc(reinterpret_cast<void **>(&fresh), bytes) != hipSuccess) { (void)hipGetLastError(); break; }
        if (loser) { (void)hipFree(loser); loser = nullptr; }
        if (hipMemsetAsync(fresh, 0, bytes, c->stream) != hipSuccess) { (void)hipGetLastError(); loser = fresh; break; }
        c->d_pb_val = fresh;
        rc = time_spmv(&c->place_ms[t]);
        if (rc != LZX_OK) { loser = fresh; break; }
        c->place_tried = t + 1;
        if (c->place_ms[t] < c->place_ms[kept]) {
            kept = t;
            loser = best_buf;
            best_buf = fresh;
        } else {
            loser = fresh;
        }
    }
    if (c->place_tried == 0) c->place_tried = 1;
    (void)hipStreamSynchronize(c->stream);
    if (loser) (void)hipFree(loser);
    c->d_pb_val = best_buf;
    c->place_kept = kept;
    LZX_HIP(hipMemsetAsync(c->d_v, 0, sizeof(double) * c->ldq, c->stream));
    LZX_HIP(hipMemsetAsync(c->d_pb_val, 0, bytes, c->stream));
    LZX_HIP(hipStreamSynchronize(c->stream));
    return rc;
}

void lzx_pb_release(lzx_ctx *c)
{
    pb_free(c->d_pb_lcol);
    pb_free(c->d_pb_dst);
    pb_free(c->d_pb_lrow);
    pb_free(c->d_pb_val);
    pb_free(c->d_pb_unit);
    pb_free(c->d_pb_row0);
    pb_free(c->d_pb_rep);
    pb_free(c->d_pb_beg);
    pb_free(c->d_pb_items);
    pb_free(c->d_pb_gstamps);
    pb_free(c->d_pb_item_dot);
    pb_free(c->d_pb_gcounter);
    pb_free(c->d_pb_multi);
    pb_free(c->d_pb_part);
    pb_free(c->d_pb_long_multi);
    pb_free(c->d_pb_mrow);
    c->pb_multi_limit = 0;
    c->pb_defer_ok = c->pb_deferring = false;
    pb_free(c->d_pbr_code);
    pb_free(c->d_pbr_base);
    c->pb = false;
    c->pb_entries = c->pb_values = c->pbr_entries = 0;
    c->pb_units = c->pb_units0 = c->pb_nr = c->pb_gather_grid = c->pb_n_items = c->pb_n_static = c->pb_n_dyn = c->pb_n_multi = c->pb_finish_grid = 0;
    c->pbr_steps = 0;
}

u32 lzx_pb_partials(const lzx_ctx *c) { return c->pb ? c->pb_gather_grid + c->pb_finish_grid : 0; }

namespace {
struct Arena {
    std::vector<void *> ptrs;
    template <typename T> int get(T **p, u64 count)
    {
        LZX_TRY(pb_alloc(p, count));
        ptrs.push_back(*p);
        return LZX_OK;
    }
    template <typename T> void drop(T *&p)
    {
        for (auto &q : ptrs)
            if (q == p) q = nullptr;
        pb_free(p);
    }
    ~Arena()
    {
        for (void *q : ptrs)
            if (q) (void)hipFree(q);
    }
};
#define GRID(n) dim3((u32)(((u64)(n) + 255) / 256)), dim3(256), 0, st

int pb_sort_keys(hipStream_t st, u64 *in, u64 *out, u64 count)
{
    size_t tb = 0;
    void *tmp = nullptr;
    LZX_HIP(hipcub::DeviceRadixSort::SortKeys(nullptr, tb, in, out, count, 0, 64, st));
    LZX_HIP(hipMalloc(&tmp, tb ? tb : 16));
    hipError_t e = hipcub::DeviceRadixSort::SortKeys(tmp, tb, in, out, count, 0, 64, st);
    if (e == hipSuccess) e = hipStreamSynchronize(st);
    (void)hipFree(tmp);
    LZX_HIP(e);
    return LZX_OK;
}
int pb_sort_pairs16(hipStream_t st, u32 *kin, u32 *kout, u32 *vin, u32 *vout, u64 count)
{
    size_t tb = 0;
    void *tmp = nullptr;
    LZX_HIP(hipcub::DeviceRadixSort::SortPairs(nullptr, tb, kin, kout, vin, vout, count, 0, 16, st));
    LZX_HIP(hipMalloc(&tmp, tb ? tb : 16));
    hipError_t e = hipcub::DeviceRadixSort::SortPairs(tmp, tb, kin, kout, vin, vout, count, 0, 16, st);
    if (e == hipSuccess) e = hipStreamSynchronize(st);
    (void)hipFree(tmp);
    LZX_HIP(e);
    return LZX_OK;
}
int pb_scan(hipStream_t st, bool inclusive, u32 *in, u32 *out, u64 count)
{
    size_t tb = 0;
    void *tmp = nullptr;
    if (inclusive) LZX_HIP(hipcub::DeviceScan::InclusiveSum(nullptr, tb, in, out, count, st));
    else LZX_HIP(hipcub::DeviceScan::ExclusiveSum(nullptr, tb, in, out, count, st));
    LZX_HIP(hipMalloc(&tmp, tb ? tb : 16));
    hipError_t e = inclusive ? hipcub::DeviceScan::InclusiveSum(tmp, tb, in, out, count, st)
                             : hipcub::DeviceScan::ExclusiveSum(tmp, tb, in, out, count, st);
    if (e == hipSuccess) e = hipStreamSynchronize(st);
    (void)hipFree(tmp);
    LZX_HIP(e);
    return LZX_OK;
}

int pb_units(lzx_ctx *c, hipStream_t st, const std::vector<u32> &sstart, const std::vector<u32> &qstart, u32 nb, u32 cap)
{
    std::vector<u32> units;
    u64 all = 0, done = 0;
    for (u32 b = 0; b < nb; ++b)
        all += (u64)((sstart.empty() ? 0 : sstart[b + 1] - sstart[b])) * LZX_PBR_STEP + (u64)((qstart.empty() ? 0 : qstart[b + 1] - qstart[b])) * 4;
    for (u32 b = 0; b < nb; ++b) {
        const u32 s0 = sstart.empty() ? 0 : sstart[b], s1 = sstart.empty() ? 0 : sstart[b + 1];
        const u32 q0 = qstart.empty() ? 0 : qstart[b], q1 = qstart.empty() ? 0 : qstart[b + 1];
        const u64 entries = (u64)(s1 - s0) * LZX_PBR_STEP + (u64)(q1 - q0) * 4;
        if (entries == 0) continue;
        u64 capb = cap;
        if (c->pb_taper_opt != 0) capb = done * 10 < all * 7 ? 2ull * cap : done * 10 < all * 9 ? cap : std::max<u64>(16384, cap / 2);
        done += entries;
        const u32 parts = (u32)((entries + capb - 1) / capb);
        for (u32 i = 0; i < parts; ++i) {
            units.push_back(b);
            units.push_back(s0 + (u32)((u64)(s1 - s0) * i / parts));
            units.push_back(s0 + (u32)((u64)(s1 - s0) * (i + 1) / parts));
            units.push_back(q0 + (u32)((u64)(q1 - q0) * i / parts));
            units.push_back(q0 + (u32)((u64)(q1 - q0) * (i + 1) / parts));
        }
    }
    c->pb_units = (u32)(units.size() / 5);
    c->pb_units0 = c->pb_units;
    if (c->overlap) {
        const u64 chunk0_end = (u64)c->world * c->xs0;
        u32 u0 = 0;
        while (u0 < c->pb_units && ((u64)units[5 * u0] + 1) * c->pb_cb <= chunk0_end) ++u0;
        c->pb_units0 = u0;
    }
    LZX_TRY(pb_alloc(&c->d_pb_unit, units.size()));
    if (!units.empty())
        LZX_HIP(hipMemcpyAsync(c->d_pb_unit, units.data(), sizeof(u32) * units.size(), hipMemcpyHostToDevice, st));
    LZX_HIP(hipStreamSynchronize(st));
    return LZX_OK;
}

int pb_download(hipStream_t st, const u32 *d, size_t count, std::vector<u32> &h)
{
    h.resize(count);
    LZX_HIP(hipMemcpyAsync(h.data(), d, sizeof(u32) * count, hipMemcpyDeviceToHost, st));
    LZX_HIP(hipStreamSynchronize(st));
    return LZX_OK;
}

int pb_prepare_impl(lzx_ctx *c, const u32 *d_code, const u32 *d_old_of_local, const u32 *d_deg_local,
                    const u32 *d_nh_off, const std::vector<u32> &h_nh, u64 total)
{
    hipStream_t st = c->stream;
    if (total >= LZX_PB_SLOT_LIMIT) LZX_FAIL(LZX_ERR_LIMIT, "propagation blocking: %llu entries do not fit 32-bit slots", (unsigned long long)total);
    c->pb_cb = (c->pb_cb_opt == 8192 || c->pb_cb_opt == 16384 || c->pb_cb_opt == LZX_PB_CB_WIDE) ? (u32)c->pb_cb_opt
               : (c->xlen * sizeof(double) <= (16u << 20) && (c->overlap || c->fuse_opt == 0) ? 8192u : LZX_PB_CB_WIDE);
    const u32 nb = (u32)((c->xlen + c->pb_cb - 1) / c->pb_cb);
    if (nb >= (1u << 16)) LZX_FAIL(LZX_ERR_LIMIT, "propagation blocking: %u column bands (limit 65535)", nb);
    u32 target = LZX_PB_TARGET;
    {
        const u64 want = total / ((u64)c->cu_count * 8);
        target = (u32)std::min<u64>(8 * LZX_PB_TARGET, std::max<u64>(LZX_PB_TARGET, (want + 1023) & ~1023ull));
    }
    if (c->pb_target_opt > 0) target = (u32)c->pb_target_opt;
    u32 unit_cap = (u32)std::min<u64>(131072, std::max<u64>(32768, (total / ((u64)c->cu_count * 4) + 511) & ~511ull));
    if (c->xlen * sizeof(double) <= (16u << 20))
        unit_cap = (u32)std::min<u64>(65536, std::max<u64>(8192, (total / ((u64)c->cu_count * 2) + 511) & ~511ull));
    if (c->pb_unit_opt > 0) unit_cap = (u32)c->pb_unit_opt;

    const bool reduce = c->pb_reduce_opt != 0;
    const u32 min_run = !reduce ? 0xffffffffu : c->pb_reduce_opt > 1 ? (u32)c->pb_reduce_opt : LZX_PBR_MIN_RUN;
    const u32 band_rows = std::min(c->n_loc_real, c->rows_live);
    std::vector<u32> row0;
    row0.push_back(0);
    if (reduce) {
        u32 l = 0;
        while (l < band_rows) {
            u32 rep = 1;
            for (;;) {
                const u32 e = (u32)std::min<u64>((u64)l + LZX_PB_RB / rep, band_rows);
                u32 heaviest = 0;
                for (u32 j = l; j < e; ++j) heaviest = std::max(heaviest, h_nh[j]);
                u32 need = rep;
                while (need < 64 && (u64)need * 2 * nb < heaviest) need <<= 1;
                if (need == rep) break;
                rep = need;
            }
            l = (u32)std::min<u64>((u64)l + LZX_PB_RB / rep, band_rows);
            row0.push_back(l);
        }
    } else {
        u32 rows = 0;
        u64 cnt = 0;
        for (u32 l = 0; l < band_rows; ++l) {
            const u32 nh = h_nh[l];
            if (rows > 0 && (cnt + nh > target || rows == LZX_PB_RB)) {
                row0.push_back(l);
                rows = 0;
                cnt = 0;
            }
            ++rows;
            cnt += nh;
        }
        if (rows > 0) row0.push_back(band_rows);
    }
    if (row0.size() == 1) row0.push_back(band_rows);
    const u32 nr = (u32)row0.size() - 1;
    if (nr >= (1u << 24)) LZX_FAIL(LZX_ERR_LIMIT, "propagation blocking: %u row bands (limit 2^24)", nr);
    LZX_TRY(pb_alloc(&c->d_pb_row0, (u64)nr + 1));
    LZX_HIP(hipMemcpyAsync(c->d_pb_row0, row0.data(), sizeof(u32) * ((size_t)nr + 1), hipMemcpyHostToDevice, st));

    Arena ar;
    u64 *d_keys = nullptr, *d_sorted = nullptr;
    LZX_TRY(ar.get(&d_keys, total)); LZX_TRY(ar.get(&d_sorted, total));
    if (c->n_loc_real)
        hipLaunchKernelGGL(k_pb_emit, dim3(std::min<u32>(c->n_loc_real, 1u << 22)), dim3(64), 0, st, c->d_row_ptr, c->d_col_idx, d_code,
                           d_old_of_local, d_deg_local, d_nh_off, c->n_loc_real, c->hub_real, c->d_pb_row0, nr, c->pb_cb, d_keys);
    LZX_TRY(pb_sort_keys(st, d_keys, d_sorted, total));
    ar.drop(d_keys);

    u32 *d_head = nullptr, *d_runid = nullptr, *d_runstart = nullptr, *d_epad = nullptr, *d_estart = nullptr;
    uint8_t *d_fmt = nullptr;
    u32 nruns = 0, epad_total = 0;
    LZX_TRY(ar.get(&d_head, total)); LZX_TRY(ar.get(&d_runid, total));
    hipLaunchKernelGGL(k_pb_heads, GRID(total), d_sorted, total, d_head);
    LZX_TRY(pb_scan(st, true, d_head, d_runid, total));
    LZX_HIP(hipMemcpy(&nruns, d_runid + (total - 1), sizeof(u32), hipMemcpyDeviceToHost));
    LZX_TRY(ar.get(&d_runstart, (u64)nruns + 1)); LZX_TRY(ar.get(&d_epad, (u64)nruns + 1)); LZX_TRY(ar.get(&d_estart, (u64)nruns + 1));
    LZX_TRY(ar.get(&d_fmt, (u64)nruns + 1));
    hipLaunchKernelGGL(k_pb_runstarts, GRID(total), d_head, d_runid, total, d_runstart);
    ar.drop(d_head);
    LZX_HIP(hipMemsetAsync(d_epad + nruns, 0, sizeof(u32), st));
    hipLaunchKernelGGL(k_pb_run_format, GRID(nruns), d_runstart, nruns, total, min_run, d_fmt, d_epad);
    {
        std::vector<u32> h;
        LZX_TRY(pb_download(st, d_epad, nruns, h));
        u64 sum = 0;
        for (u32 v : h) sum += v;
        if (sum >= LZX_PB_SLOT_LIMIT) LZX_FAIL(LZX_ERR_LIMIT, "propagation blocking: %llu padded entries do not fit 32-bit slots", (unsigned long long)sum);
        epad_total = (u32)sum;
    }
    LZX_TRY(pb_scan(st, false, d_epad, d_estart, (u64)nruns + 1));
    ar.drop(d_epad);
    const u32 nsteps = epad_total / LZX_PBR_STEP;

    uint16_t *d_rcode = nullptr, *d_rrow = nullptr, *d_step_cband = nullptr;
    u32 *d_step_run = nullptr, *d_step_cnt = nullptr, *d_step_excl = nullptr;
    LZX_TRY(ar.get(&d_rcode, (u64)epad_total + 8)); LZX_TRY(ar.get(&d_rrow, (u64)epad_total + 8));
    LZX_TRY(ar.get(&d_step_cband, (u64)nsteps + 1)); LZX_TRY(ar.get(&d_step_run, (u64)nsteps + 1));
    LZX_TRY(ar.get(&d_step_cnt, (u64)nsteps + 1)); LZX_TRY(ar.get(&d_step_excl, (u64)nsteps + 1));
    if (nsteps) {
        hipLaunchKernelGGL(k_pb_fill16, GRID(epad_total), d_rcode, epad_total, (uint16_t)c->pb_cb);
        hipLaunchKernelGGL(k_pb_fill16, GRID(epad_total), d_rrow, epad_total, (uint16_t)0xffffu);
        hipLaunchKernelGGL(k_pbr_place, GRID(total), d_sorted, d_runid, d_runstart, d_estart, d_fmt, total, d_rcode, d_rrow,
                           d_step_cband, d_step_run);
        hipLaunchKernelGGL(k_pbr_count, dim3(nsteps), dim3(64), 0, st, reinterpret_cast<const uint4 *>(d_rcode), d_step_cnt);
    }
    LZX_HIP(hipMemsetAsync(d_step_cnt + nsteps, 0, sizeof(u32), st));
    LZX_TRY(pb_scan(st, false, d_step_cnt, d_step_excl, (u64)nsteps + 1));
    ar.drop(d_step_cnt);

    const u32 run_align = (c->pb_align_opt == 4 || c->pb_align_opt == 8 || c->pb_align_opt == 16) ? (u32)c->pb_align_opt : LZX_PB_ALIGN;
    u32 *d_vcount = nullptr, *d_vpos = nullptr;
    LZX_TRY(ar.get(&d_vcount, (u64)nruns + 1)); LZX_TRY(ar.get(&d_vpos, (u64)nruns + 1));
    LZX_HIP(hipMemsetAsync(d_vcount + nruns, 0, sizeof(u32), st));
    hipLaunchKernelGGL(k_pb_run_values, GRID(nruns), d_runstart, nruns, total, d_fmt, d_estart, d_step_excl, run_align, d_vcount);
    u64 len = 0, red_entries = 0;
    {
        std::vector<u32> h;
        LZX_TRY(pb_download(st, d_vcount, nruns, h));
        for (u32 v : h) len += v;
        if (len >= LZX_PB_SLOT_LIMIT) LZX_FAIL(LZX_ERR_LIMIT, "propagation blocking: %llu values do not fit 32-bit slots", (unsigned long long)len);
    }
    LZX_TRY(pb_scan(st, false, d_vcount, d_vpos, (u64)nruns + 1));
    ar.drop(d_vcount);
    const u64 nquads = len / 4;
    uint16_t *d_prow = nullptr, *d_plcol = nullptr, *d_qcband = nullptr;
    u32 *d_step_base = nullptr;
    LZX_TRY(ar.get(&d_prow, len + 8)); LZX_TRY(ar.get(&d_plcol, len + 8)); LZX_TRY(ar.get(&d_qcband, nquads + 2));
    LZX_TRY(ar.get(&d_step_base, (u64)nsteps + 1));
    hipLaunchKernelGGL(k_pb_fill16, GRID(len + 8), d_prow, len + 8, (uint16_t)0xffffu);
    hipLaunchKernelGGL(k_pb_fill16, GRID(len + 8), d_plcol, len + 8, (uint16_t)c->pb_cb);
    hipLaunchKernelGGL(k_pb_fill16, GRID(nquads + 2), d_qcband, nquads + 2, (uint16_t)0xffffu);
    if (nsteps) {
        hipLaunchKernelGGL(k_pbr_step_base, GRID(nsteps), d_step_run, d_estart, d_step_excl, d_vpos, nsteps, d_step_base);
        hipLaunchKernelGGL(k_pbr_rows, dim3(nsteps), dim3(64), 0, st, reinterpret_cast<const uint4 *>(d_rcode),
                           reinterpret_cast<const uint4 *>(d_rrow), d_step_base, d_prow);
    }
    hipLaunchKernelGGL(k_pb_place, GRID(total), d_sorted, d_runid, d_runstart, d_vpos, d_fmt, total, d_prow, d_plcol, d_qcband);
    std::vector<u32> rstart;
    {
        u32 *d_rstart = nullptr, *d_band_pos = nullptr;
        LZX_TRY(ar.get(&d_rstart, (u64)nr + 1)); LZX_TRY(ar.get(&d_band_pos, (u64)nr + 1));
        hipLaunchKernelGGL(k_pb_bounds_u64, GRID(nr + 1), d_sorted, total, KEY_RBAND_SHIFT, nr, d_rstart);
        hipLaunchKernelGGL(k_pb_band_pos, GRID(nr + 1), d_rstart, d_runid, d_vpos, nr, total, (u32)len, d_band_pos);
        LZX_TRY(pb_download(st, d_band_pos, (size_t)nr + 1, rstart));
        ar.drop(d_rstart); ar.drop(d_band_pos);
    }
#ifdef LZX_DEBUG_KNOBS
    if (getenv("LZX_PB_STATS")) {
        std::vector<u32> rs;
        LZX_TRY(pb_download(st, d_runstart, nruns, rs));
        u64 cls[14] = {0}, cnt[14] = {0};
        for (u32 r = 0; r < nruns; ++r) {
            const u32 rl = (r + 1 < nruns ? rs[r + 1] : (u32)total) - rs[r];
            u32 b = 0;
            while ((2u << b) <= rl && b < 13) ++b;
            cls[b] += rl;
            ++cnt[b];
        }
        for (u32 b = 0; b < 14; ++b)
            fprintf(stderr, "[lzx pb stats] runs of %u..%u entries: %llu runs, %llu entries (%.1f %%)\n", 1u << b, (2u << b) - 1,
                    (unsigned long long)cnt[b], (unsigned long long)cls[b], 100.0 * cls[b] / (double)total);
    }
#endif
    {
        std::vector<u32> rs;
        std::vector<uint8_t> fm(nruns);
        LZX_TRY(pb_download(st, d_runstart, nruns, rs));
        LZX_HIP(hipMemcpy(fm.data(), d_fmt, nruns, hipMemcpyDeviceToHost));
        for (u32 r = 0; r < nruns; ++r)
            if (fm[r]) red_entries += (r + 1 < nruns ? rs[r + 1] : (u32)total) - rs[r];
    }
#ifdef LZX_DEBUG_KNOBS
    if (getenv("LZX_PB_STATS")) {
        std::vector<u32> rs;
        std::vector<uint8_t> fm(nruns);
        LZX_TRY(pb_download(st, d_runstart, nruns, rs));
        LZX_HIP(hipMemcpy(fm.data(), d_fmt, nruns, hipMemcpyDeviceToHost));
        u64 nred = 0, npl = 0, pl_entries = 0, pl_pad8 = 0;
        for (u32 r = 0; r < nruns; ++r) {
            const u32 rl = (r + 1 < nruns ? rs[r + 1] : (u32)total) - rs[r];
            if (fm[r]) ++nred; else { ++npl; pl_entries += rl; pl_pad8 += (rl + 7u) & ~7u; }
        }
        std::vector<u32> se;
        LZX_TRY(pb_download(st, d_step_excl, (size_t)nsteps + 1, se));
        fprintf(stderr, "[lzx pb stats] entries %llu: reduced %llu in %llu runs -> %u steps = %llu padded entries (%.1f %% padding), %u pieces; "
                "plain %llu in %llu runs -> %llu padded to 8; values incl. run alignment %llu (quads %llu); row bands %u, column bands %u, runs %u\n",
                (unsigned long long)total, (unsigned long long)red_entries, (unsigned long long)nred, nsteps, (unsigned long long)epad_total,
                100.0 * ((double)epad_total - (double)red_entries) / std::max<double>(1.0, (double)epad_total), nsteps ? se[nsteps] : 0u,
                (unsigned long long)pl_entries, (unsigned long long)npl, (unsigned long long)pl_pad8, (unsigned long long)len,
                (unsigned long long)nquads, nr, nb, nruns);
    }
#endif
    LZX_HIP(hipStreamSynchronize(st));
    ar.drop(d_sorted); ar.drop(d_runid); ar.drop(d_runstart); ar.drop(d_estart); ar.drop(d_fmt); ar.drop(d_vpos);
    ar.drop(d_rrow); ar.drop(d_step_run); ar.drop(d_step_excl);

    std::vector<u32> sstart, qstart;
    if (nsteps) {
        u32 *skey = nullptr, *skey_s = nullptr, *sidx = nullptr, *ssorted = nullptr, *bstart = nullptr;
        LZX_TRY(ar.get(&skey, nsteps)); LZX_TRY(ar.get(&skey_s, nsteps)); LZX_TRY(ar.get(&sidx, nsteps)); LZX_TRY(ar.get(&ssorted, nsteps));
        hipLaunchKernelGGL(k_pb_iota_widen, GRID(nsteps), d_step_cband, nsteps, skey, sidx);
        LZX_TRY(pb_sort_pairs16(st, skey, skey_s, sidx, ssorted, nsteps));
        LZX_TRY(pb_alloc(&c->d_pbr_code, (u64)nsteps * 64 + 1));
        LZX_TRY(pb_alloc(&c->d_pbr_base, (u64)nsteps + 1));
        hipLaunchKernelGGL(k_pbr_steps, dim3(nsteps), dim3(64), 0, st, ssorted, reinterpret_cast<const uint4 *>(d_rcode), d_step_base,
                           c->d_pbr_code, c->d_pbr_base);
        LZX_TRY(ar.get(&bstart, (u64)nb + 1));
        hipLaunchKernelGGL(k_pb_bounds_u32, GRID(nb + 1), skey_s, nsteps, nb, bstart);
        LZX_TRY(pb_download(st, bstart, (size_t)nb + 1, sstart));
        ar.drop(skey); ar.drop(skey_s); ar.drop(sidx); ar.drop(ssorted); ar.drop(bstart);
    }
    ar.drop(d_rcode); ar.drop(d_step_cband); ar.drop(d_step_base);
    c->pbr_steps = nsteps;
    if (nquads) {
        u32 *qkey = nullptr, *qkey_s = nullptr, *qidx = nullptr, *qsorted = nullptr, *bstart = nullptr;
        LZX_TRY(ar.get(&qkey, nquads)); LZX_TRY(ar.get(&qkey_s, nquads)); LZX_TRY(ar.get(&qidx, nquads)); LZX_TRY(ar.get(&qsorted, nquads));
        hipLaunchKernelGGL(k_pb_iota_widen, GRID(nquads), d_qcband, nquads, qkey, qidx);
        LZX_TRY(pb_sort_pairs16(st, qkey, qkey_s, qidx, qsorted, nquads));
        ar.drop(qkey); ar.drop(qidx);
        LZX_TRY(ar.get(&bstart, (u64)nb + 1));
        hipLaunchKernelGGL(k_pb_bounds_u32, GRID(nb + 1), qkey_s, nquads, nb, bstart);
        LZX_TRY(pb_download(st, bstart, (size_t)nb + 1, qstart));
        const u64 live = qstart[nb];
        {
            uint2 *q_lcol = nullptr;
            LZX_TRY(pb_alloc(&q_lcol, live + 1));
            c->d_pb_lcol = reinterpret_cast<uint16_t *>(q_lcol);
        }
        LZX_TRY(pb_alloc(&c->d_pb_dst, live + 1));
        if (live)
            hipLaunchKernelGGL(k_pb_quads, GRID(live), qsorted, d_plcol, live, reinterpret_cast<uint2 *>(c->d_pb_lcol), c->d_pb_dst);
        LZX_HIP(hipStreamSynchronize(st));
        ar.drop(qkey_s); ar.drop(qsorted); ar.drop(bstart);
    }
    ar.drop(d_plcol); ar.drop(d_qcband);
    LZX_TRY(pb_units(c, st, sstart, qstart, nb, unit_cap));
    LZX_HIP(hipGetLastError());

    u32 *d_rstart_pad = nullptr, *d_step0 = nullptr;
    uint8_t *d_occ = nullptr;
    LZX_TRY(ar.get(&d_rstart_pad, (u64)nr + 1));
    LZX_HIP(hipMemcpyAsync(d_rstart_pad, rstart.data(), sizeof(u32) * ((size_t)nr + 1), hipMemcpyHostToDevice, st));
    LZX_TRY(pb_alloc(&c->d_pb_lrow, len + 8)); LZX_TRY(pb_alloc(&c->d_pb_rep, (u64)nr));
    std::vector<u32> rep((size_t)nr, 1u);
    {
        std::vector<u32> step0((size_t)nr + 1);
        u64 steps = 0;
        for (u32 R = 0; R < nr; ++R) {
            step0[R] = (u32)steps;
            steps += (rstart[R + 1] - rstart[R] + 63u) / 64u;
        }
        step0[nr] = (u32)steps;
        LZX_TRY(ar.get(&d_step0, (u64)nr + 1)); LZX_TRY(ar.get(&d_occ, len + 8));
        LZX_HIP(hipMemcpyAsync(d_step0, step0.data(), sizeof(u32) * ((size_t)nr + 1), hipMemcpyHostToDevice, st));
        LZX_HIP(hipMemcpyAsync(c->d_pb_rep, rep.data(), sizeof(u32) * nr, hipMemcpyHostToDevice, st));
        LZX_HIP(hipMemsetAsync(d_occ, 0, len + 8, st));
        if (steps)
            hipLaunchKernelGGL(k_pb_occurrence, dim3((u32)steps), dim3(64), 0, st, d_prow, d_rstart_pad, d_step0, nr, d_occ,
                               c->d_pb_rep);
        LZX_HIP(hipMemcpyAsync(rep.data(), c->d_pb_rep, sizeof(u32) * nr, hipMemcpyDeviceToHost, st));
        LZX_HIP(hipStreamSynchronize(st));
        for (u32 R = 0; R < nr; ++R) {
            const u32 rows = row0[R + 1] - row0[R];
            const u32 room = std::max(1u, LZX_PB_RB / std::max(rows, 1u));
            rep[R] = std::max(1u, std::min(std::min(rep[R], room), 64u));
        }
        LZX_HIP(hipMemcpyAsync(c->d_pb_rep, rep.data(), sizeof(u32) * nr, hipMemcpyHostToDevice, st));
        u32 no_rounds = 0;
#ifdef LZX_DEBUG_KNOBS
        if (getenv("LZX_PB_NO_ROUNDS")) no_rounds = 1;
#endif
        hipLaunchKernelGGL(k_pb_slots, GRID(len), d_prow, d_occ, d_rstart_pad, c->d_pb_rep, nr, len, c->d_pb_lrow, no_rounds);
        LZX_HIP(hipStreamSynchronize(st));
#ifdef LZX_DEBUG_KNOBS
        if (getenv("LZX_PB_STATS")) {
            std::vector<uint16_t> hs(len);
            LZX_HIP(hipMemcpy(hs.data(), c->d_pb_lrow, sizeof(uint16_t) * len, hipMemcpyDeviceToHost));
            u64 late = 0, blocks_late = 0, maxr = 0;
            for (u64 b0 = 0; b0 < len; b0 += 128) {
                bool any = false;
                for (u64 i = b0; i < std::min<u64>(len, b0 + 128); ++i) {
                    const u32 r = hs[i] >> 10;
                    if (r) { ++late; any = true; maxr = std::max<u64>(maxr, r); }
                }
                blocks_late += any ? 1 : 0;
            }
            {
                std::vector<uint16_t> hp(len);
                LZX_HIP(hipMemcpy(hp.data(), d_prow, sizeof(uint16_t) * len, hipMemcpyDeviceToHost));
                int shown = 0;
                for (u64 i = 0; i < len && shown < 6; ++i)
                    if (hs[i] >> 10) {
                        u32 R = 0;
                        while (R + 1 < nr && rstart[R + 1] <= i) ++R;
                        fprintf(stderr, "[lzx pb stats]   late value at %llu (band %u begins at %u, offset in band %llu, block offset %llu, rep %u): rows",
                                (unsigned long long)i, R, rstart[R], (unsigned long long)(i - rstart[R]), (unsigned long long)((i - rstart[R]) % 128), rep[R]);
                        for (u64 j = (i >= 6 ? i - 6 : 0); j < std::min<u64>(len, i + 3); ++j) fprintf(stderr, " %s%u/%u", j == i ? "*" : "", (unsigned)hp[j], (unsigned)(hs[j] >> 10));
                        fprintf(stderr, "\n");
                        ++shown;
                    }
            }
            u64 rep1 = 0;
            for (u32 R = 0; R < nr; ++R) rep1 += rep[R] == 1 ? 1 : 0;
            fprintf(stderr, "[lzx pb stats] gather slots: %llu values, %llu of them (%.3f %%) in a round > 0 (highest round %llu), %llu of %llu 128-value blocks (%.2f %%) "
                    "take the slow path; %llu of %u row bands have one slot per row\n", (unsigned long long)len, (unsigned long long)late, 100.0 * late / std::max<double>(1.0, (double)len),
                    (unsigned long long)maxr, (unsigned long long)blocks_late, (unsigned long long)((len + 127) / 128), 100.0 * blocks_late / std::max<double>(1.0, (double)((len + 127) / 128)),
                    (unsigned long long)rep1, nr);
        }
#endif
    }

    std::vector<u32> items, multi;
    u64 slots = 0;
    for (u32 R = 0; R < nr; ++R) {
        const u32 beg = rstart[R], end = rstart[R + 1];
        if (beg == end) continue;
        const u32 rows = row0[R + 1] - row0[R];
        if (end - beg > 2 * target) {
            const u32 cnt = (end - beg + target - 1) / target;
            const u32 piece = ((end - beg + cnt - 1) / cnt + 127u) & ~127u;
            u32 made = 0;
            for (u32 s = beg; s < end; s += piece, ++made) {
                items.push_back(R); items.push_back(s); items.push_back(std::min(end, s + piece));
                items.push_back((u32)(slots + (u64)made * rows));
            }
            for (u32 j = 0; j < rows; ++j) {
                multi.push_back(row0[R] + j); multi.push_back((u32)(slots + j)); multi.push_back(made); multi.push_back(rows);
            }
            slots += (u64)made * rows;
            if (slots >= 0xffffffffull) LZX_FAIL(LZX_ERR_LIMIT, "propagation blocking: item totals overflow 32-bit slots");
        } else {
            items.push_back(R); items.push_back(beg); items.push_back(end); items.push_back(0xffffffffu);
        }
    }
    c->pb_n_items = c->pb_n_static = (u32)(items.size() / 4);
    c->pb_n_dyn = 0;
    c->pb_n_multi = (u32)(multi.size() / 4);
    c->pb_gather_block = c->pb_gwaves_opt == 4 ? 256u : 512u;
    c->pb_gather_grid = std::min<u32>((u32)c->cu_count * (1024u / c->pb_gather_block), std::max(1u, c->pb_n_items));
    if (c->pb_grid_cap_opt > 0) c->pb_gather_grid = std::min<u32>(c->pb_gather_grid, (u32)c->pb_grid_cap_opt);
    LZX_TRY(pb_alloc(&c->d_pb_beg, (u64)nr + 1));
    LZX_HIP(hipMemcpyAsync(c->d_pb_beg, rstart.data(), sizeof(u32) * ((size_t)nr + 1), hipMemcpyHostToDevice, st));
    const u32 group_cap = c->pb_group_opt >= 0 ? (u32)c->pb_group_opt : LZX_PB_GROUP;
    if (group_cap > 0 && c->pb_gather_block == 512u) {
        std::vector<u32> out;
        auto small = [&](size_t i) {
            const u32 R = items[4 * i];
            return items[4 * i + 3] == 0xffffffffu && row0[R + 1] - row0[R] > 1 && items[4 * i + 2] - items[4 * i + 1] <= group_cap;
        };
        std::vector<u64> cost;
        const size_t ni = items.size() / 4;
        size_t n_small = 0;
        for (size_t i = 0; i < ni; ++i) n_small += small(i) ? 1 : 0;
        const size_t per_group = c->pb_group_force_opt > 0 ? std::min<size_t>(8, std::max<size_t>(2, (size_t)c->pb_group_force_opt)) : std::min<size_t>(8, (n_small + c->pb_gather_grid - 1) / std::max<u32>(1u, c->pb_gather_grid));
        for (size_t i = 0; i < ni;) {
            if (per_group < 2 || !small(i)) {
                const u32 R = items[4 * i];
                out.insert(out.end(), items.begin() + 4 * i, items.begin() + 4 * i + 4);
                cost.push_back(10ull * (items[4 * i + 2] - items[4 * i + 1]) + 24ull * (row0[R + 1] - row0[R]) + 40000ull);
                ++i;
                continue;
            }
            size_t j = i;
            u64 vals = 0, rows = 0, widest = 0;
            while (j < ni && j - i < per_group && small(j) && items[4 * j] == items[4 * i] + (u32)(j - i)) {
                const u32 R = items[4 * j];
                vals += items[4 * j + 2] - items[4 * j + 1];
                widest = std::max<u64>(widest, items[4 * j + 2] - items[4 * j + 1]);
                rows += row0[R + 1] - row0[R];
                ++j;
            }
            out.push_back(items[4 * i]); out.push_back((u32)(j - i)); out.push_back((u32)vals); out.push_back(LZX_PB_ITEM_GROUP);
            const u64 nbands = j - i, split = nbands <= 1 ? 8 : nbands <= 2 ? 4 : nbands <= 4 ? 2 : 1;
            cost.push_back(std::max<u64>(10ull * vals + 24ull * rows, 80ull * widest / split) + 40000ull);
            i = j;
        }
        const u32 G = c->pb_gather_grid;
        const size_t no = cost.size();
        std::vector<u32> order(no);
        for (size_t i = 0; i < no; ++i) order[i] = (u32)i;
        std::stable_sort(order.begin(), order.end(), [&](u32 a, u32 b2) { return cost[a] > cost[b2]; });
        size_t n_tail = 0;
        {
            const u64 share = c->pb_dyn_opt >= 0 ? (u64)std::min<int64_t>(90, c->pb_dyn_opt) : LZX_PB_DYN_SHARE;
            u64 all = 0, tail = 0;
            for (u64 x : cost) all += x;
            if (share > 0 && no > (c->pb_dyn_opt > 0 ? 1 : 2) * (size_t)G)
                while (n_tail + G < no && (tail + cost[order[no - 1 - n_tail]]) * 100 <= all * share) tail += cost[order[no - 1 - n_tail++]];
        }
        const size_t n_dealt = no - n_tail;
        std::vector<std::vector<u32>> lists(G);
        std::priority_queue<std::pair<u64, u32>, std::vector<std::pair<u64, u32>>, std::greater<std::pair<u64, u32>>> heap;
        for (u32 w = 0; w < G; ++w) heap.push({0ull, w});
        size_t rounds = 0;
        for (size_t oi = 0; oi < n_dealt; ++oi) {
            const u32 i = order[oi];
            auto [load, w] = heap.top();
            heap.pop();
            lists[w].push_back(i);
            rounds = std::max(rounds, lists[w].size());
            heap.push({load + cost[i], w});
        }
        items.assign(rounds * G * 4, 0u);
        for (size_t r = 0; r < rounds; ++r)
            for (u32 w = 0; w < G; ++w) {
                u32 *o = &items[4 * (r * G + w)];
                if (r < lists[w].size()) {
                    const u32 *it = &out[4 * (size_t)lists[w][r]];
                    o[0] = it[0]; o[1] = it[1]; o[2] = it[2]; o[3] = it[3];
                } else {
                    o[3] = LZX_PB_ITEM_NONE;
                }
            }
        c->pb_n_static = (u32)(items.size() / 4);
        for (size_t oi = n_dealt; oi < no; ++oi) {
            const u32 *it = &out[4 * (size_t)order[oi]];
            items.insert(items.end(), it, it + 4);
        }
        c->pb_n_dyn = (u32)n_tail;
        c->pb_n_items = (u32)(items.size() / 4);
    }
#ifdef LZX_DEBUG_KNOBS
    if (c->pb_stamps_opt > 0) {
        LZX_TRY(pb_alloc(&c->d_pb_gstamps, 8 * (u64)c->pb_gather_grid));
        LZX_HIP(hipMemsetAsync(c->d_pb_gstamps, 0, sizeof(unsigned long long) * 8 * c->pb_gather_grid, st));
    }
#endif
    u32 n_uncovered = 0;
    {
        std::vector<uint8_t> flag((size_t)c->n_long64 + 1, 2);
        for (u32 R = 0; R < nr; ++R)
            if (rstart[R] != rstart[R + 1])
                for (u32 r = row0[R]; r < std::min<u32>(row0[R + 1], c->n_long64); ++r) flag[r] = 0;
        for (size_t i = 0; i < multi.size(); i += 4)
            if (multi[i] < c->n_long64) flag[multi[i]] = 1;
        for (u32 r = 0; r < c->n_long64; ++r) n_uncovered += flag[r] == 2 ? 1 : 0;
        LZX_TRY(pb_alloc(&c->d_pb_long_multi, flag.size()));
        LZX_HIP(hipMemcpyAsync(c->d_pb_long_multi, flag.data(), flag.size(), hipMemcpyHostToDevice, st));
        LZX_HIP(hipStreamSynchronize(st));
    }
    LZX_TRY(pb_alloc(&c->d_pb_items, items.size())); LZX_TRY(pb_alloc(&c->d_pb_multi, multi.size())); LZX_TRY(pb_alloc(&c->d_pb_part, slots));
    {
        u32 limit = 0;
        for (size_t i = 0; i < multi.size(); i += 4) limit = std::max(limit, multi[i] + 1);
        limit = (limit + 1u) & ~1u;
        std::vector<u32> mrow((size_t)limit * 4, 0u);
        for (size_t i = 0; i < multi.size(); i += 4)
            for (int u = 0; u < 4; ++u) mrow[(size_t)multi[i] * 4 + u] = multi[i + u];
        c->pb_multi_limit = limit;
        LZX_TRY(pb_alloc(&c->d_pb_mrow, (u64)std::max<u32>(limit, 1u)));
        if (limit) LZX_HIP(hipMemcpyAsync(c->d_pb_mrow, mrow.data(), sizeof(u32) * mrow.size(), hipMemcpyHostToDevice, st));
        LZX_HIP(hipStreamSynchronize(st));
    }
    if (!items.empty())
        LZX_HIP(hipMemcpyAsync(c->d_pb_items, items.data(), sizeof(u32) * items.size(), hipMemcpyHostToDevice, st));
    if (!multi.empty())
        LZX_HIP(hipMemcpyAsync(c->d_pb_multi, multi.data(), sizeof(u32) * multi.size(), hipMemcpyHostToDevice, st));

    LZX_TRY(pb_alloc(&c->d_pb_gcounter, 4));
    LZX_HIP(hipMemsetAsync(c->d_pb_gcounter, 0, sizeof(u32) * 4, st));
    if (c->pb_n_dyn) {
        LZX_TRY(pb_alloc(&c->d_pb_item_dot, c->pb_n_dyn));
        LZX_HIP(hipMemsetAsync(c->d_pb_item_dot, 0, sizeof(double) * c->pb_n_dyn, st));
    }
    LZX_TRY(pb_alloc(&c->d_pb_val, len + 8));
    LZX_HIP(hipMemsetAsync(c->d_pb_val, 0, sizeof(double) * (len + 8), st));
    LZX_HIP(hipStreamSynchronize(st));
    LZX_HIP(hipGetLastError());

    c->pb = true;
    c->pb_entries = total;
    c->pbr_entries = red_entries;
    c->pb_values = len;
    c->pb_nr = nr;
    constexpr u32 waves_per_wg = LZX_PB_GATHER_BLOCK / 64;
    (void)waves_per_wg;
    c->pb_finish_grid = (c->pb_n_multi + (n_uncovered ? c->n_long64 : 0u) + LZX_VEC_BLOCK - 1) / LZX_VEC_BLOCK;
    c->pb_defer_ok = c->pb_n_multi > 0 && n_uncovered == 0 && c->pb_n_dyn == 0;
    if (c->pb_n_dyn) c->pb_finish_grid = std::max<u32>(c->pb_finish_grid, (c->pb_n_dyn + LZX_VEC_BLOCK - 1) / LZX_VEC_BLOCK);
    return LZX_OK;
}
#undef GRID
}

int lzx_pb_prepare(lzx_ctx *c, const u32 *d_code, const u32 *d_old_of_local, const u32 *d_deg_local,
                   const u32 *d_nh_off, const std::vector<u32> &h_nh, u64 total)
{
    const int rc = pb_prepare_impl(c, d_code, d_old_of_local, d_deg_local, d_nh_off, h_nh, total);
    if (rc != LZX_OK) {
        (void)hipStreamSynchronize(c->stream);
        lzx_pb_release(c);
    }
    return rc;
}

bool lzx_pb_can_fuse(const lzx_ctx *c)
{
    if (!c->pb || !(c->pb_cb == LZX_PB_CB || c->pb_cb == 8192 || c->pb_cb == LZX_PB_CB_WIDE)) return false;
#ifdef LZX_DEBUG_KNOBS
    if (c->phase_mask_opt & (4 | 8)) return false;
#endif
    return true;
}

int lzx_pb_launch(lzx_ctx *c, const double *x, const double *q_loc, double *v, double *partials, hipEvent_t chunk1_ready,
                  hipEvent_t v_ready, int phases, const SpmvArgs *fuse, u32 fuse_blocks, bool *fused)
{
    if (fused) *fused = false;
    const bool do_scatter = phases & 1, do_gather = phases & 2;
    if (!c->pb) {
        if (chunk1_ready && do_scatter) LZX_HIP(hipStreamWaitEvent(c->stream, chunk1_ready, 0));
        return LZX_OK;
    }
    const bool scan = c->pb_scan_opt >= 0 ? c->pb_scan_opt > 0 : LZX_PB_CARRY_SCAN;
    const size_t lds1 = ((size_t)c->pb_cb + 2 + (scan ? 0 : 16 * 66)) * sizeof(double);
    const bool ntc = c->pb_scatter_nt_opt >= 0 ? c->pb_scatter_nt_opt > 0
                                               : (LZX_PB_SCATTER_NT && 10ull * c->pb_values > LZX_PB_NT_BYTES && 2 * c->pbr_entries > c->pb_entries);
    using scatter_fn = void (*)(const u32 *, const uint4 *, const u32 *, const uint2 *, const u32 *, const double *, u64, double *);
    auto pick_scatter = [&]() -> scatter_fn {
        if (c->pb_cb == 8192) {
            if (scan) return ntc ? k_pb_scatter<8192, true, true> : k_pb_scatter<8192, true, false>;
            return ntc ? k_pb_scatter<8192, false, true> : k_pb_scatter<8192, false, false>;
        }
        if (c->pb_cb == LZX_PB_CB_WIDE) return ntc ? k_pb_scatter<LZX_PB_CB_WIDE, true, true> : k_pb_scatter<LZX_PB_CB_WIDE, true, false>;
        if (scan) return ntc ? k_pb_scatter<LZX_PB_CB, true, true> : k_pb_scatter<LZX_PB_CB, true, false>;
        return ntc ? k_pb_scatter<LZX_PB_CB, false, true> : k_pb_scatter<LZX_PB_CB, false, false>;
    };
    scatter_fn kern = pick_scatter();
    if (c->pb_units)
        LZX_HIP(hipFuncSetAttribute(reinterpret_cast<const void *>(kern), hipFuncAttributeMaxDynamicSharedMemorySize, (int)lds1));
    auto scatter = [&](u32 u0, u32 u1, bool may_fuse) {
        if (u1 <= u0 && !(may_fuse && fuse && fused)) return;
        if (may_fuse && fuse && fused && (c->pb_cb == LZX_PB_CB || c->pb_cb == 8192 || c->pb_cb == LZX_PB_CB_WIDE) && u0 == 0) {
            using fused_fn = void (*)(const u32 *, u32, const uint4 *, const u32 *, const uint2 *, const u32 *, const double *, u64, double *, const SpmvArgs, const u32);
            fused_fn kf;
            if (c->pb_cb == 8192) {
                if (scan) kf = ntc ? k_pb_scatter_spmv<8192, true, true> : k_pb_scatter_spmv<8192, true, false>;
                else kf = ntc ? k_pb_scatter_spmv<8192, false, true> : k_pb_scatter_spmv<8192, false, false>;
            } else if (c->pb_cb == LZX_PB_CB_WIDE) {
                kf = ntc ? k_pb_scatter_spmv<LZX_PB_CB_WIDE, true, true> : k_pb_scatter_spmv<LZX_PB_CB_WIDE, true, false>;
            } else {
                if (scan) kf = ntc ? k_pb_scatter_spmv<LZX_PB_CB, true, true> : k_pb_scatter_spmv<LZX_PB_CB, true, false>;
                else kf = ntc ? k_pb_scatter_spmv<LZX_PB_CB, false, true> : k_pb_scatter_spmv<LZX_PB_CB, false, false>;
            }
            const size_t ldsf = std::max(lds1, c->spmv_lds);
            (void)hipFuncSetAttribute(reinterpret_cast<const void *>(kf), hipFuncAttributeMaxDynamicSharedMemorySize, (int)ldsf);
            hipLaunchKernelGGL(kf, dim3(u1 + fuse_blocks), dim3(1024), ldsf, c->stream, c->d_pb_unit, u1, c->d_pbr_code, c->d_pbr_base,
                               reinterpret_cast<const uint2 *>(c->d_pb_lcol), c->d_pb_dst, x, c->xlen, c->d_pb_val, *fuse, c->fuse_opt == 1 ? 0u : 1u);
            *fused = true;
            return;
        }
        hipLaunchKernelGGL(kern, dim3(u1 - u0), dim3(1024), lds1, c->stream, c->d_pb_unit + 5 * (size_t)u0, c->d_pbr_code,
                           c->d_pbr_base, reinterpret_cast<const uint2 *>(c->d_pb_lcol), c->d_pb_dst, x, c->xlen, c->d_pb_val);
    };
    if ((c->phase_mask_opt & 4) || !do_scatter) {
    } else if (chunk1_ready) {
        scatter(0, c->pb_units0, true);
        LZX_HIP(hipStreamWaitEvent(c->stream, chunk1_ready, 0));
        scatter(c->pb_units0, c->pb_units, false);
    } else {
        scatter(0, c->pb_units, true);
    }
    if (c->trace && do_scatter) LZX_HIP(hipEventRecord(c->trace_ev[3], c->stream));
    if (!do_gather) {
        LZX_HIP(hipGetLastError());
        return LZX_OK;
    }
    if (v_ready) LZX_HIP(hipStreamWaitEvent(c->stream, v_ready, 0));
    const size_t lds2 = ((size_t)(LZX_PB_GATHER_BLOCK / 64) * (LZX_PB_RB + 64) + LZX_PB_GATHER_BLOCK / 64) * sizeof(double) +
                        16 * (LZX_PB_GATHER_BLOCK / 64) * 8 * sizeof(u32) + 16;
    const bool nt = c->pb_gather_nt_opt >= 0 ? c->pb_gather_nt_opt > 0 : 10ull * c->pb_values > LZX_PB_NT_BYTES;
    u32 probe_l2g = 0;
#ifdef LZX_DEBUG_KNOBS
    if (const char *pe = getenv("LZX_PROBE_L2G")) probe_l2g = (u32)atoi(pe);
#endif
    auto gather = [&](auto kern, unsigned long long *stamps) -> int {
        LZX_HIP(hipFuncSetAttribute(reinterpret_cast<const void *>(kern), hipFuncAttributeMaxDynamicSharedMemorySize, (int)lds2));
        hipLaunchKernelGGL(kern, dim3(c->pb_gather_grid), dim3(LZX_PB_GATHER_BLOCK), lds2, c->stream,
                           reinterpret_cast<const uint4 *>(c->d_pb_items), c->pb_n_static, c->pb_n_dyn, c->d_pb_gcounter, c->d_pb_item_dot, c->d_pb_row0,
                           c->d_pb_rep, c->d_pb_beg, c->d_pb_lrow, c->d_pb_val, v, q_loc, c->d_pb_part, partials, stamps, probe_l2g,
                           c->d_item_first, c->d_long_partial, c->d_pb_long_multi, c->n_long64);
        return LZX_OK;
    };
    bool gathered = false;
#ifdef LZX_DEBUG_KNOBS
    if (!(c->phase_mask_opt & 8)) {
        if (getenv("LZX_ABLATE_SLOTS")) {
            LZX_TRY(nt ? gather(k_pb_gather<false, true, true>, nullptr) : gather(k_pb_gather<false, false, true>, nullptr));
            gathered = true;
        } else
        if (c->pb_stamps_opt > 0 && c->d_pb_gstamps) {
            LZX_TRY(nt ? gather(k_pb_gather<true, true>, c->d_pb_gstamps) : gather(k_pb_gather<true, false>, c->d_pb_gstamps));
            gathered = true;
        }
    }
#endif
    if (c->phase_mask_opt & 8) {
    } else if (!gathered)
        LZX_TRY(nt ? gather(k_pb_gather<false, true>, nullptr) : gather(k_pb_gather<false, false>, nullptr));
    if (c->pb_finish_grid && !(c->pb_deferring && c->pb_defer_ok))
        hipLaunchKernelGGL(k_pb_finish, dim3(c->pb_finish_grid), dim3(LZX_VEC_BLOCK), 0, c->stream,
                           reinterpret_cast<const uint4 *>(c->d_pb_multi), c->pb_n_multi, c->d_pb_part, c->d_item_first,
                           c->d_long_partial, c->d_pb_long_multi, c->n_long64, v, q_loc, partials + c->pb_gather_grid,
                           c->pb_n_dyn ? c->d_pb_item_dot : nullptr, c->pb_n_dyn);
    LZX_HIP(hipGetLastError());
    return LZX_OK;
}
```

Before: 1804.

## Pack partially filled reduced-run steps into shared 64-lane steps

Adds tail packing for the propagation-blocking reduced-run code: steps whose 64 lanes are only partly filled are bin-packed on the host (in 16-lane granules, up to four segments) into combined steps. The scatter kernel gains a packed-step loop that recovers each segment's base and lane mask via readlane and restricts the output ballot to that segment. The goal is less padding, so fewer step loads and wavefronts per scatter, at the cost of an extra per-step record read, mask arithmetic, a wider unit descriptor and more preprocessing.

```diff
diff --git a/msc-hpc-final-project_amd/__init__.py b/msc-hpc-final-project_amd/__init__.py
--- a/msc-hpc-final-project_amd/__init__.py
+++ b/msc-hpc-final-project_amd/__init__.py
@@ -12,7 +12,7 @@
                    "lazy_normalisation", "timing_marks_every", "reorthogonalise", "basis_fp32", "reference_order", "placement_trials",
                    "sharded_ingest", "operator")
 
-SHAPE_OPTIONS = ("pb_reduce", "pb_target", "pb_unit", "pb_column_band", "pb_run_align", "pb_taper", "pb_dyn_share", "pb_carry_scan", "pb_scatter_nt", "pb_gather_grid", "pb_gather_nt", "spmv_wgs", "pb_group", "pb_group_force",
+SHAPE_OPTIONS = ("pb_reduce", "pb_target", "pb_unit", "pb_column_band", "pb_run_align", "pb_taper", "pb_dyn_share", "pb_carry_scan", "pb_pack_tails", "pb_pack_segments", "pb_scatter_nt", "pb_gather_grid", "pb_gather_nt", "spmv_wgs", "pb_group", "pb_group_force",
                  "narrow_slices", "tie_sort", "long_row", "item_len", "exchange_at_world_1", "isolated_rows", "unnormalised_basis", "fuse_staged", "start_vector_scan", "defer_finish",
                  "multi_row_chunk", "eig_basis_bytes", "solve_state_bytes", "solve_poll", "bfs_state_bytes", "tri_long_list", "tri_state_bytes", "core_long_row", "core_state_bytes",
                  "truss_long_row", "truss_state_bytes", "color_long_row", "lpa_group_row", "lpa_table_row", "lpa_state_bytes")
diff --git a/msc-hpc-final-project_amd/csrc/lzx_api.hip b/msc-hpc-final-project_amd/csrc/lzx_api.hip
--- a/msc-hpc-final-project_amd/csrc/lzx_api.hip
+++ b/msc-hpc-final-project_amd/csrc/lzx_api.hip
@@ -111,6 +111,8 @@
     {"pb_taper", &lzx_ctx::pb_taper_opt, OPT_SHAPE | OPT_KNOB},
     {"pb_dyn_share", &lzx_ctx::pb_dyn_opt, OPT_SHAPE | OPT_KNOB},
     {"pb_carry_scan", &lzx_ctx::pb_scan_opt, OPT_SHAPE},
+    {"pb_pack_tails", &lzx_ctx::pb_pack_opt, OPT_SHAPE | OPT_KNOB},
+    {"pb_pack_segments", &lzx_ctx::pb_pack_seg_opt, OPT_SHAPE | OPT_KNOB},
     {"pb_scatter_nt", &lzx_ctx::pb_scatter_nt_opt, OPT_SHAPE},
     {"pb_gather_grid", &lzx_ctx::pb_grid_cap_opt, OPT_SHAPE | OPT_KNOB},
     {"pb_gather_nt", &lzx_ctx::pb_gather_nt_opt, OPT_SHAPE | OPT_KNOB},
@@ -204,6 +206,10 @@
     if (!strcmp(name, "gather_items_dealt")) *value = c->pb ? c->pb_n_static : 0;
     else if (!strcmp(name, "gather_items_drawn")) *value = c->pb ? c->pb_n_dyn : 0;
     else if (!strcmp(name, "gather_workgroups")) *value = c->pb ? c->pb_gather_grid : 0;
+    else if (!strcmp(name, "pbr_steps")) *value = c->pb ? c->pbr_steps : 0;
+    else if (!strcmp(name, "pbr_packed_steps")) *value = c->pb ? c->pbr_packed : 0;
+    else if (!strcmp(name, "pbr_packed_segments_max")) *value = c->pb ? c->pbr_packed_seg_max : 0;
+    else if (!strcmp(name, "pbr_padding_entries")) *value = c->pb ? (int64_t)((u64)c->pbr_steps * LZX_PBR_STEP - c->pbr_entries) : 0;
     else if (!strcmp(name, "placement_tried")) *value = c->place_tried;
     else if (!strcmp(name, "placement_kept")) *value = c->place_kept;
     else if (!strcmp(name, "start_vector_was_constant")) *value = c->x0_was_constant ? 1 : 0;
diff --git a/msc-hpc-final-project_amd/csrc/lzx_internal.h b/msc-hpc-final-project_amd/csrc/lzx_internal.h
--- a/msc-hpc-final-project_amd/csrc/lzx_internal.h
+++ b/msc-hpc-final-project_amd/csrc/lzx_internal.h
@@ -58,6 +58,11 @@
 static constexpr u64 LZX_PB_SLOT_LIMIT = (1ull << 32) - (1ull << 24);
 static constexpr u32 LZX_PBR_STEP = 512;
 static constexpr u32 LZX_PBR_MIN_RUN = 384;
+static constexpr bool LZX_PBR_PACK_TAILS = true;
+static constexpr u32 LZX_PBR_SEG_MAX = 4;
+static constexpr u32 LZX_PBR_PACK_SEGMENTS = LZX_PBR_SEG_MAX;
+static constexpr u32 LZX_PBR_PACK_WORDS = LZX_PBR_SEG_MAX + LZX_PBR_SEG_MAX / 4;
+static constexpr u32 LZX_PB_UNIT_WORDS = 7;
 static constexpr bool LZX_PB_SCATTER_NT = true;
 static constexpr bool LZX_PB_CARRY_SCAN = true;
 
@@ -234,6 +239,11 @@
     uint4 *d_pbr_code = nullptr;
     u32 *d_pbr_base = nullptr;
     u32 pbr_steps = 0;
+    u32 *d_pbr_pack = nullptr;
+    u32 pbr_packed = 0;
+    u32 pbr_packed_seg_max = 0;
+    int64_t pb_pack_opt = -1;
+    int64_t pb_pack_seg_opt = -1;
 
     double *d_v = nullptr;
     u32 np2_last = 0;
diff --git a/msc-hpc-final-project_amd/csrc/lzx_pb.hip b/msc-hpc-final-project_amd/csrc/lzx_pb.hip
--- a/msc-hpc-final-project_amd/csrc/lzx_pb.hip
+++ b/msc-hpc-final-project_amd/csrc/lzx_pb.hip
@@ -8,6 +8,7 @@
 #include "lzx_internal.h"
 #include "lzx_spmv_body.h"
 #include "lzx_pb_shared.h"
+#include "lzx_pb_pack.h"
 
 namespace {
 
@@ -270,6 +271,38 @@
     if (threadIdx.x == 0) sbase[blockIdx.x] = step_base[s];
 }
 
+__global__ void __launch_bounds__(64) k_pbr_lanes(const u32 *ssorted, const uint4 *rcode, u32 pad_code, uint8_t *lanes)
+{
+    const uint4 c = rcode[(size_t)ssorted[blockIdx.x] * 64 + threadIdx.x];
+    const unsigned long long m = __ballot((c.x & 0xffffu) != pad_code);
+    if (threadIdx.x == 0) lanes[blockIdx.x] = (uint8_t)__popcll(m);
+}
+
+__global__ void __launch_bounds__(64) k_pbr_steps_kept(const u32 *keep, const u32 *ssorted, const uint4 *rcode, const u32 *step_base, uint4 *scode, u32 *sbase)
+{
+    const u32 s = ssorted[keep[blockIdx.x]];
+    scode[(size_t)blockIdx.x * 64 + threadIdx.x] = rcode[(size_t)s * 64 + threadIdx.x];
+    if (threadIdx.x == 0) sbase[blockIdx.x] = step_base[s];
+}
+
+__global__ void __launch_bounds__(64) k_pbr_packed(const u32 *plan, const u32 *ssorted, const uint4 *rcode, const u32 *step_base, uint4 *pcode, u32 *prec)
+{
+    const u32 *pl = plan + (size_t)blockIdx.x * LZX_PBR_PACK_WORDS;
+    const u32 lane = threadIdx.x;
+    u32 src = 0, lo = 0;
+    for (u32 k = 0; k < LZX_PBR_SEG_MAX; ++k) {
+        const u32 sk = (pl[LZX_PBR_SEG_MAX + (k >> 2)] >> (8 * (k & 3))) & 0xffu;
+        if (lane >= sk) {
+            src = pl[k];
+            lo = sk;
+        }
+    }
+    pcode[(size_t)blockIdx.x * 64 + lane] = rcode[(size_t)ssorted[src] * 64 + (lane - lo)];
+    u32 *rec = prec + (size_t)blockIdx.x * LZX_PBR_PACK_WORDS;
+    if (lane < LZX_PBR_SEG_MAX) rec[lane] = pl[lane] != 0xffffffffu ? step_base[ssorted[pl[lane]]] : 0u;
+    else if (lane < LZX_PBR_PACK_WORDS) rec[lane] = pl[lane];
+}
+
 template <int CTRL, int ROW_MASK>
 __device__ __forceinline__ double dpp_f64(double v)
 {
@@ -329,13 +362,21 @@
 }
 template <bool NTC> __device__ __forceinline__ u32 sld(const u32 *p) { return NTC ? __builtin_nontemporal_load(p) : *p; }
 
+struct StepWhole {
+    __device__ __forceinline__ unsigned long long operator()(unsigned long long m) const { return m; }
+};
+struct StepSegment {
+    unsigned long long mask;
+    __device__ __forceinline__ unsigned long long operator()(unsigned long long m) const { return m & mask; }
+};
+
 template <u32 CB, bool SCAN, bool NTC>
 __device__ __forceinline__ void
-pb_scatter_body(const u32 *unit, const uint4 *scode, const u32 *sbase, const uint2 *q_lcol, const u32 *q_dst,
+pb_scatter_body(const u32 *unit, const uint4 *scode, const u32 *sbase, const uint4 *pcode, const u32 *prec, const uint2 *q_lcol, const u32 *q_dst,
                 const double *__restrict__ x, u64 xlen, double *val, const u32 ublock)
 {
     extern __shared__ __attribute__((aligned(16))) double tile[];
-    const u32 band = unit[5 * ublock];
+    const u32 band = unit[LZX_PB_UNIT_WORDS * ublock];
     const u64 base = (u64)band * CB;
     if (base + CB <= xlen) {
         const double2 *src = reinterpret_cast<const double2 *>(x + base);
@@ -356,9 +397,9 @@
     constexpr u32 W = 1024 / 64;
 
     {
-        const u32 beg = unit[5 * ublock + 1], end = unit[5 * ublock + 2];
+        const u32 beg = unit[LZX_PB_UNIT_WORDS * ublock + 1], end = unit[LZX_PB_UNIT_WORDS * ublock + 2];
         double *carry = tile + CB + 2 + wv * 66;
-        auto body_scan = [&](const uint4 &c, u32 pos) {
+        auto body_scan = [&](const uint4 &c, u32 pos, const auto seg) {
             const u32 w[4] = {c.x, c.y, c.z, c.w};
             double xv[8];
             bool f[8];
@@ -383,15 +424,16 @@
             for (int e = 0; e < 8; ++e) {
                 const unsigned long long m = __ballot(f[e]);
                 if (m) {
+                    const unsigned long long ms = seg(m);
                     if (f[e]) {
-                        out[done + lanes_below(m)] = pv[e] + carry;
+                        out[done + lanes_below(ms)] = pv[e] + carry;
                         carry = 0.0;
                     }
-                    done += (u32)__popcll(m);
+                    done += (u32)__popcll(ms);
                 }
             }
         };
-        auto body_lds = [&](const uint4 &c, u32 pos) {
+        auto body_lds = [&](const uint4 &c, u32 pos, const auto seg) {
             double xv[8];
 #pragma unroll
             for (int e = 0; e < 8; ++e) xv[e] = tile[pbr_half(c, e) & 0x7fffu];
@@ -426,11 +468,12 @@
                 s += xv[e];
                 const unsigned long long m = __ballot(f);
                 if (m) {
+                    const unsigned long long ms = seg(m);
                     if (f) {
-                        out[done + lanes_below(m)] = s;
+                        out[done + lanes_below(ms)] = s;
                         s = 0.0;
                     }
-                    done += (u32)__popcll(m);
+                    done += (u32)__popcll(ms);
                 }
             }
         };
@@ -445,8 +488,8 @@
             }
 #pragma unroll
             for (int u = 0; u < 4; ++u) {
-                if (SCAN) body_scan(c[u], b[u]);
-                else body_lds(c[u], b[u]);
+                if (SCAN) body_scan(c[u], b[u], StepWhole{});
+                else body_lds(c[u], b[u], StepWhole{});
             }
         }
         if (s < end) {
@@ -462,14 +505,56 @@
 #pragma unroll
             for (int u = 0; u < 3; ++u)
                 if (s + u * W < end) {
-                    if (SCAN) body_scan(c[u], b[u]);
-                    else body_lds(c[u], b[u]);
+                    if (SCAN) body_scan(c[u], b[u], StepWhole{});
+                    else body_lds(c[u], b[u], StepWhole{});
                 }
         }
+        const u32 pbeg = unit[LZX_PB_UNIT_WORDS * ublock + 5], pend = unit[LZX_PB_UNIT_WORDS * ublock + 6];
+        auto packed_step = [&](const uint4 &c, const u32 rw) {
+            u32 first = 0, lo = 0, hi = 64;
+#pragma unroll
+            for (int k = 0; k < (int)LZX_PBR_SEG_MAX; ++k) {
+                const u32 sk = ((u32)__builtin_amdgcn_readlane((int)rw, (int)LZX_PBR_SEG_MAX + (k >> 2)) >> (8 * (k & 3))) & 0xffu;
+                const u32 bk = (u32)__builtin_amdgcn_readlane((int)rw, k);
+                if (lane >= sk) {
+                    first = bk;
+                    lo = sk;
+                }
+            }
+#pragma unroll
+            for (int k = (int)LZX_PBR_SEG_MAX - 1; k > 0; --k) {
+                const u32 sk = ((u32)__builtin_amdgcn_readlane((int)rw, (int)LZX_PBR_SEG_MAX + (k >> 2)) >> (8 * (k & 3))) & 0xffu;
+                if (lane < sk) hi = sk;
+            }
+            const unsigned long long below_hi = hi >= 64 ? ~0ull : (1ull << hi) - 1ull;
+            const StepSegment seg{below_hi & ~((1ull << lo) - 1ull)};
+            if (SCAN) body_scan(c, first, seg);
+            else body_lds(c, first, seg);
+        };
+        u32 p = pbeg + wv;
+        if (p < pend) {
+            uint4 c = sld<NTC>(pcode + (size_t)p * 64 + lane);
+            u32 rw = prec[(size_t)p * LZX_PBR_PACK_WORDS + (lane < LZX_PBR_PACK_WORDS ? lane : 0u)];
+            for (;;) {
+                const u32 pn = p + W;
+                const bool more = pn < pend;
+                uint4 cn = c;
+                u32 rn = rw;
+                if (more) {
+                    cn = sld<NTC>(pcode + (size_t)pn * 64 + lane);
+                    rn = prec[(size_t)pn * LZX_PBR_PACK_WORDS + (lane < LZX_PBR_PACK_WORDS ? lane : 0u)];
+                }
+                packed_step(c, rw);
+                if (!more) break;
+                c = cn;
+                rw = rn;
+                p = pn;
+            }
+        }
     }
 
     {
-        const u32 beg = unit[5 * ublock + 3], end = unit[5 * ublock + 4];
+        const u32 beg = unit[LZX_PB_UNIT_WORDS * ublock + 3], end = unit[LZX_PB_UNIT_WORDS * ublock + 4];
         for (u32 blk = beg + wv * 256u; blk < end; blk += W * 256u) {
         const u32 wend = blk + 256u < end ? blk + 256u : end;
         u32 j = blk + lane;
@@ -522,24 +607,24 @@
 
 template <u32 CB, bool SCAN, bool NTC>
 __global__ void __launch_bounds__(1024)
-k_pb_scatter(const u32 *unit, const uint4 *scode, const u32 *sbase, const uint2 *q_lcol, const u32 *q_dst,
+k_pb_scatter(const u32 *unit, const uint4 *scode, const u32 *sbase, const uint4 *pcode, const u32 *prec, const uint2 *q_lcol, const u32 *q_dst,
              const double *__restrict__ x, u64 xlen, double *val)
 {
-    pb_scatter_body<CB, SCAN, NTC>(unit, scode, sbase, q_lcol, q_dst, x, xlen, val, blockIdx.x);
+    pb_scatter_body<CB, SCAN, NTC>(unit, scode, sbase, pcode, prec, q_lcol, q_dst, x, xlen, val, blockIdx.x);
 }
 
 template <u32 CB, bool SCAN, bool NTC>
 __global__ void __launch_bounds__(1024)
-k_pb_scatter_spmv(const u32 *unit, u32 n_units, const uint4 *scode, const u32 *sbase, const uint2 *q_lcol, const u32 *q_dst,
+k_pb_scatter_spmv(const u32 *unit, u32 n_units, const uint4 *scode, const u32 *sbase, const uint4 *pcode, const u32 *prec, const uint2 *q_lcol, const u32 *q_dst,
                   const double *__restrict__ x, u64 xlen, double *val, const SpmvArgs a, const u32 spmv_first)
 {
     const u32 spmv_blocks = gridDim.x - n_units;
     if (spmv_first) {
         if (blockIdx.x < spmv_blocks) spmv_body<2, false>(a, blockIdx.x, spmv_blocks);
-        else pb_scatter_body<CB, SCAN, NTC>(unit, scode, sbase, q_lcol, q_dst, x, xlen, val, blockIdx.x - spmv_blocks);
+        else pb_scatter_body<CB, SCAN, NTC>(unit, scode, sbase, pcode, prec, q_lcol, q_dst, x, xlen, val, blockIdx.x - spmv_blocks);
         return;
     }
-    if (blockIdx.x < n_units) pb_scatter_body<CB, SCAN, NTC>(unit, scode, sbase, q_lcol, q_dst, x, xlen, val, blockIdx.x);
+    if (blockIdx.x < n_units) pb_scatter_body<CB, SCAN, NTC>(unit, scode, sbase, pcode, prec, q_lcol, q_dst, x, xlen, val, blockIdx.x);
     else spmv_body<2, false>(a, blockIdx.x - n_units, spmv_blocks);
 }
 
@@ -1032,6 +1117,8 @@
     c->pb_defer_ok = c->pb_deferring = false;
     pb_free(c->d_pbr_code);
     pb_free(c->d_pbr_base);
+    pb_free(c->d_pbr_pack);
+    c->pbr_packed = c->pbr_packed_seg_max = 0;
     c->pb = false;
     c->pb_entries = c->pb_values = c->pbr_entries = 0;
     c->pb_units = c->pb_units0 = c->pb_nr = c->pb_gather_grid = c->pb_n_items = c->pb_n_static = c->pb_n_dyn = c->pb_n_multi = c->pb_finish_grid = 0;
@@ -1102,16 +1189,18 @@
     return LZX_OK;
 }
 
-int pb_units(lzx_ctx *c, hipStream_t st, const std::vector<u32> &sstart, const std::vector<u32> &qstart, u32 nb, u32 cap)
+int pb_units(lzx_ctx *c, hipStream_t st, const std::vector<u32> &sstart, const std::vector<u32> &qstart, const std::vector<u32> &pstart, u32 nb, u32 cap)
 {
     std::vector<u32> units;
     u64 all = 0, done = 0;
     for (u32 b = 0; b < nb; ++b)
-        all += (u64)((sstart.empty() ? 0 : sstart[b + 1] - sstart[b])) * LZX_PBR_STEP + (u64)((qstart.empty() ? 0 : qstart[b + 1] - qstart[b])) * 4;
+        all += (u64)((sstart.empty() ? 0 : sstart[b + 1] - sstart[b]) + (pstart.empty() ? 0 : pstart[b + 1] - pstart[b])) * LZX_PBR_STEP +
+               (u64)((qstart.empty() ? 0 : qstart[b + 1] - qstart[b])) * 4;
     for (u32 b = 0; b < nb; ++b) {
         const u32 s0 = sstart.empty() ? 0 : sstart[b], s1 = sstart.empty() ? 0 : sstart[b + 1];
         const u32 q0 = qstart.empty() ? 0 : qstart[b], q1 = qstart.empty() ? 0 : qstart[b + 1];
-        const u64 entries = (u64)(s1 - s0) * LZX_PBR_STEP + (u64)(q1 - q0) * 4;
+        const u32 p0 = pstart.empty() ? 0 : pstart[b], p1 = pstart.empty() ? 0 : pstart[b + 1];
+        const u64 entries = (u64)(s1 - s0 + p1 - p0) * LZX_PBR_STEP + (u64)(q1 - q0) * 4;
         if (entries == 0) continue;
         u64 capb = cap;
         if (c->pb_taper_opt != 0) capb = done * 10 < all * 7 ? 2ull * cap : done * 10 < all * 9 ? cap : std::max<u64>(16384, cap / 2);
@@ -1123,14 +1212,16 @@
             units.push_back(s0 + (u32)((u64)(s1 - s0) * (i + 1) / parts));
             units.push_back(q0 + (u32)((u64)(q1 - q0) * i / parts));
             units.push_back(q0 + (u32)((u64)(q1 - q0) * (i + 1) / parts));
-        }
-    }
-    c->pb_units = (u32)(units.size() / 5);
+            units.push_back(p0 + (u32)((u64)(p1 - p0) * i / parts));
+            units.push_back(p0 + (u32)((u64)(p1 - p0) * (i + 1) / parts));
+        }
+    }
+    c->pb_units = (u32)(units.size() / LZX_PB_UNIT_WORDS);
     c->pb_units0 = c->pb_units;
     if (c->overlap) {
         const u64 chunk0_end = (u64)c->world * c->xs0;
         u32 u0 = 0;
-        while (u0 < c->pb_units && ((u64)units[5 * u0] + 1) * c->pb_cb <= chunk0_end) ++u0;
+        while (u0 < c->pb_units && ((u64)units[LZX_PB_UNIT_WORDS * u0] + 1) * c->pb_cb <= chunk0_end) ++u0;
         c->pb_units0 = u0;
     }
     LZX_TRY(pb_alloc(&c->d_pb_unit, units.size()));
@@ -1170,6 +1261,8 @@
 
     const bool reduce = c->pb_reduce_opt != 0;
     const u32 min_run = !reduce ? 0xffffffffu : c->pb_reduce_opt > 1 ? (u32)c->pb_reduce_opt : LZX_PBR_MIN_RUN;
+    const bool pack_tails = c->pb_pack_opt >= 0 ? c->pb_pack_opt > 0 : LZX_PBR_PACK_TAILS;
+    const u32 pack_segments = c->pb_pack_seg_opt >= 0 ? (u32)std::min<int64_t>(c->pb_pack_seg_opt, LZX_PBR_SEG_MAX) : LZX_PBR_PACK_SEGMENTS;
     const u32 band_rows = std::min(c->n_loc_real, c->rows_live);
     std::vector<u32> row0;
     row0.push_back(0);
@@ -1347,23 +1440,98 @@
     ar.drop(d_sorted); ar.drop(d_runid); ar.drop(d_runstart); ar.drop(d_estart); ar.drop(d_fmt); ar.drop(d_vpos);
     ar.drop(d_rrow); ar.drop(d_step_run); ar.drop(d_step_excl);
 
-    std::vector<u32> sstart, qstart;
+    std::vector<u32> sstart, qstart, pstart;
+    u32 n_unpacked = nsteps, n_packed = 0, seg_max = 0;
     if (nsteps) {
         u32 *skey = nullptr, *skey_s = nullptr, *sidx = nullptr, *ssorted = nullptr, *bstart = nullptr;
         LZX_TRY(ar.get(&skey, nsteps)); LZX_TRY(ar.get(&skey_s, nsteps)); LZX_TRY(ar.get(&sidx, nsteps)); LZX_TRY(ar.get(&ssorted, nsteps));
         hipLaunchKernelGGL(k_pb_iota_widen, GRID(nsteps), d_step_cband, nsteps, skey, sidx);
         LZX_TRY(pb_sort_pairs16(st, skey, skey_s, sidx, ssorted, nsteps));
-        LZX_TRY(pb_alloc(&c->d_pbr_code, (u64)nsteps * 64 + 1));
-        LZX_TRY(pb_alloc(&c->d_pbr_base, (u64)nsteps + 1));
-        hipLaunchKernelGGL(k_pbr_steps, dim3(nsteps), dim3(64), 0, st, ssorted, reinterpret_cast<const uint4 *>(d_rcode), d_step_base,
-                           c->d_pbr_code, c->d_pbr_base);
         LZX_TRY(ar.get(&bstart, (u64)nb + 1));
         hipLaunchKernelGGL(k_pb_bounds_u32, GRID(nb + 1), skey_s, nsteps, nb, bstart);
         LZX_TRY(pb_download(st, bstart, (size_t)nb + 1, sstart));
-        ar.drop(skey); ar.drop(skey_s); ar.drop(sidx); ar.drop(ssorted); ar.drop(bstart);
+        ar.drop(skey); ar.drop(skey_s); ar.drop(sidx); ar.drop(bstart);
+        std::vector<u32> keep, plan;
+        if (pack_tails && pack_segments >= 2) {
+            uint8_t *d_lanes = nullptr;
+            LZX_TRY(ar.get(&d_lanes, nsteps));
+            hipLaunchKernelGGL(k_pbr_lanes, dim3(nsteps), dim3(64), 0, st, ssorted, reinterpret_cast<const uint4 *>(d_rcode), c->pb_cb, d_lanes);
+            std::vector<uint8_t> lanes(nsteps);
+            LZX_HIP(hipMemcpyAsync(lanes.data(), d_lanes, nsteps, hipMemcpyDeviceToHost, st));
+            LZX_HIP(hipStreamSynchronize(st));
+            ar.drop(d_lanes);
+            std::vector<u32> ustart((size_t)nb + 1, 0u), tails, bin;
+            std::vector<uint8_t> tail_lanes, lane0;
+            pstart.assign((size_t)nb + 1, 0u);
+            keep.reserve(nsteps);
+            for (u32 b = 0; b < nb; ++b) {
+                ustart[b] = (u32)keep.size();
+                pstart[b] = n_packed;
+                tails.clear();
+                tail_lanes.clear();
+                for (u32 j = sstart[b]; j < sstart[b + 1]; ++j)
+                    if (lanes[j] > 0 && lanes[j] < 64) {
+                        tails.push_back(j);
+                        tail_lanes.push_back(lanes[j]);
+                    }
+                const u32 made = lzx_pbr_pack_tails(tail_lanes.data(), tail_lanes.size(), pack_segments, bin, lane0);
+                plan.resize((size_t)(n_packed + made) * LZX_PBR_PACK_WORDS, 0xffffffffu);
+                for (u32 m = 0; m < made; ++m)
+                    for (u32 w = 0; w < LZX_PBR_SEG_MAX / 4; ++w) plan[(size_t)(n_packed + m) * LZX_PBR_PACK_WORDS + LZX_PBR_SEG_MAX + w] = 0x40404040u;
+                size_t t = 0;
+                std::vector<u32> filled(made, 0u);
+                for (u32 j = sstart[b]; j < sstart[b + 1]; ++j) {
+                    const bool tail = t < tails.size() && tails[t] == j;
+                    if (!tail || bin[t] == LZX_PBR_PACK_NONE) keep.push_back(j);
+                    else {
+                        u32 *rec = plan.data() + (size_t)(n_packed + bin[t]) * LZX_PBR_PACK_WORDS;
+                        const u32 k = filled[bin[t]]++;
+                        rec[k] = j;
+                        u32 &w = rec[LZX_PBR_SEG_MAX + (k >> 2)];
+                        w = (w & ~(0xffu << (8 * (k & 3)))) | ((u32)lane0[t] << (8 * (k & 3)));
+                        seg_max = std::max(seg_max, k + 1);
+                    }
+                    if (tail) ++t;
+                }
+                n_packed += made;
+            }
+            ustart[nb] = (u32)keep.size();
+            pstart[nb] = n_packed;
+            n_unpacked = (u32)keep.size();
+            sstart.swap(ustart);
+        }
+        LZX_TRY(pb_alloc(&c->d_pbr_code, (u64)(n_unpacked + n_packed) * 64 + 1));
+        LZX_TRY(pb_alloc(&c->d_pbr_base, (u64)n_unpacked + 1));
+        if (!n_packed) {
+            hipLaunchKernelGGL(k_pbr_steps, dim3(nsteps), dim3(64), 0, st, ssorted, reinterpret_cast<const uint4 *>(d_rcode), d_step_base,
+                               c->d_pbr_code, c->d_pbr_base);
+            pstart.clear();
+        } else {
+            u32 *d_keep = nullptr, *d_plan = nullptr;
+            LZX_TRY(ar.get(&d_keep, (u64)n_unpacked + 1)); LZX_TRY(ar.get(&d_plan, plan.size()));
+            LZX_TRY(pb_alloc(&c->d_pbr_pack, plan.size()));
+            if (n_unpacked) LZX_HIP(hipMemcpyAsync(d_keep, keep.data(), sizeof(u32) * n_unpacked, hipMemcpyHostToDevice, st));
+            LZX_HIP(hipMemcpyAsync(d_plan, plan.data(), sizeof(u32) * plan.size(), hipMemcpyHostToDevice, st));
+            if (n_unpacked)
+                hipLaunchKernelGGL(k_pbr_steps_kept, dim3(n_unpacked), dim3(64), 0, st, d_keep, ssorted, reinterpret_cast<const uint4 *>(d_rcode),
+                                   d_step_base, c->d_pbr_code, c->d_pbr_base);
+            hipLaunchKernelGGL(k_pbr_packed, dim3(n_packed), dim3(64), 0, st, d_plan, ssorted, reinterpret_cast<const uint4 *>(d_rcode), d_step_base,
+                               c->d_pbr_code + (size_t)n_unpacked * 64, c->d_pbr_pack);
+            LZX_HIP(hipStreamSynchronize(st));
+            ar.drop(d_keep); ar.drop(d_plan);
+        }
+        ar.drop(ssorted);
     }
     ar.drop(d_rcode); ar.drop(d_step_cband); ar.drop(d_step_base);
-    c->pbr_steps = nsteps;
+    c->pbr_steps = n_unpacked + n_packed;
+    c->pbr_packed = n_packed;
+    c->pbr_packed_seg_max = n_packed ? seg_max : 0;
+#ifdef LZX_DEBUG_KNOBS
+    if (getenv("LZX_PB_STATS"))
+        fprintf(stderr, "[lzx pb stats] tail packing %s (up to %u segments): %u steps -> %u unpacked + %u packed (most segments %u), padding %llu -> %llu entries\n",
+                pack_tails ? "on" : "off", pack_segments, nsteps, n_unpacked, n_packed, c->pbr_packed_seg_max,
+                (unsigned long long)((u64)nsteps * LZX_PBR_STEP - red_entries), (unsigned long long)((u64)c->pbr_steps * LZX_PBR_STEP - red_entries));
+#endif
     if (nquads) {
         u32 *qkey = nullptr, *qkey_s = nullptr, *qidx = nullptr, *qsorted = nullptr, *bstart = nullptr;
         LZX_TRY(ar.get(&qkey, nquads)); LZX_TRY(ar.get(&qkey_s, nquads)); LZX_TRY(ar.get(&qidx, nquads)); LZX_TRY(ar.get(&qsorted, nquads));
@@ -1386,7 +1554,7 @@
         ar.drop(qkey_s); ar.drop(qsorted); ar.drop(bstart);
     }
     ar.drop(d_plcol); ar.drop(d_qcband);
-    LZX_TRY(pb_units(c, st, sstart, qstart, nb, unit_cap));
+    LZX_TRY(pb_units(c, st, sstart, qstart, pstart, nb, unit_cap));
     LZX_HIP(hipGetLastError());
 
     u32 *d_rstart_pad = nullptr, *d_step0 = nullptr;
@@ -1668,7 +1836,7 @@
     const size_t lds1 = ((size_t)c->pb_cb + 2 + (scan ? 0 : 16 * 66)) * sizeof(double);
     const bool ntc = c->pb_scatter_nt_opt >= 0 ? c->pb_scatter_nt_opt > 0
                                                : (LZX_PB_SCATTER_NT && 10ull * c->pb_values > LZX_PB_NT_BYTES && 2 * c->pbr_entries > c->pb_entries);
-    using scatter_fn = void (*)(const u32 *, const uint4 *, const u32 *, const uint2 *, const u32 *, const double *, u64, double *);
+    using scatter_fn = void (*)(const u32 *, const uint4 *, const u32 *, const uint4 *, const u32 *, const uint2 *, const u32 *, const double *, u64, double *);
     auto pick_scatter = [&]() -> scatter_fn {
         if (c->pb_cb == 8192) {
             if (scan) return ntc ? k_pb_scatter<8192, true, true> : k_pb_scatter<8192, true, false>;
@@ -1679,12 +1847,13 @@
         return ntc ? k_pb_scatter<LZX_PB_CB, false, true> : k_pb_scatter<LZX_PB_CB, false, false>;
     };
     scatter_fn kern = pick_scatter();
+    const uint4 *pcode = c->d_pbr_code ? c->d_pbr_code + (size_t)(c->pbr_steps - c->pbr_packed) * 64 : nullptr;
     if (c->pb_units)
         LZX_HIP(hipFuncSetAttribute(reinterpret_cast<const void *>(kern), hipFuncAttributeMaxDynamicSharedMemorySize, (int)lds1));
     auto scatter = [&](u32 u0, u32 u1, bool may_fuse) {
         if (u1 <= u0 && !(may_fuse && fuse && fused)) return;
         if (may_fuse && fuse && fused && (c->pb_cb == LZX_PB_CB || c->pb_cb == 8192 || c->pb_cb == LZX_PB_CB_WIDE) && u0 == 0) {
-            using fused_fn = void (*)(const u32 *, u32, const uint4 *, const u32 *, const uint2 *, const u32 *, const double *, u64, double *, const SpmvArgs, const u32);
+            using fused_fn = void (*)(const u32 *, u32, const uint4 *, const u32 *, const uint4 *, const u32 *, const uint2 *, const u32 *, const double *, u64, double *, const SpmvArgs, const u32);
             fused_fn kf;
             if (c->pb_cb == 8192) {
                 if (scan) kf = ntc ? k_pb_scatter_spmv<8192, true, true> : k_pb_scatter_spmv<8192, true, false>;
@@ -1697,13 +1866,13 @@
             }
             const size_t ldsf = std::max(lds1, c->spmv_lds);
             (void)hipFuncSetAttribute(reinterpret_cast<const void *>(kf), hipFuncAttributeMaxDynamicSharedMemorySize, (int)ldsf);
-            hipLaunchKernelGGL(kf, dim3(u1 + fuse_blocks), dim3(1024), ldsf, c->stream, c->d_pb_unit, u1, c->d_pbr_code, c->d_pbr_base,
+            hipLaunchKernelGGL(kf, dim3(u1 + fuse_blocks), dim3(1024), ldsf, c->stream, c->d_pb_unit, u1, c->d_pbr_code, c->d_pbr_base, pcode, c->d_pbr_pack,
                                reinterpret_cast<const uint2 *>(c->d_pb_lcol), c->d_pb_dst, x, c->xlen, c->d_pb_val, *fuse, c->fuse_opt == 1 ? 0u : 1u);
             *fused = true;
             return;
         }
-        hipLaunchKernelGGL(kern, dim3(u1 - u0), dim3(1024), lds1, c->stream, c->d_pb_unit + 5 * (size_t)u0, c->d_pbr_code,
-                           c->d_pbr_base, reinterpret_cast<const uint2 *>(c->d_pb_lcol), c->d_pb_dst, x, c->xlen, c->d_pb_val);
+        hipLaunchKernelGGL(kern, dim3(u1 - u0), dim3(1024), lds1, c->stream, c->d_pb_unit + LZX_PB_UNIT_WORDS * (size_t)u0, c->d_pbr_code,
+                           c->d_pbr_base, pcode, c->d_pbr_pack, reinterpret_cast<const uint2 *>(c->d_pb_lcol), c->d_pb_dst, x, c->xlen, c->d_pb_val);
     };
     if ((c->phase_mask_opt & 4) || !do_scatter) {
     } else if (chunk1_ready) {
diff --git a/msc-hpc-final-project_amd/csrc/lzx_pb_pack.h b/msc-hpc-final-project_amd/csrc/lzx_pb_pack.h
--- /dev/null
+++ b/msc-hpc-final-project_amd/csrc/lzx_pb_pack.h
@@ -0,0 +1,49 @@
+#pragma once
+#include <cstddef>
+#include <cstdint>
+#include <vector>
+
+static constexpr uint32_t LZX_PBR_PACK_NONE = 0xffffffffu;
+static constexpr uint32_t LZX_PBR_PACK_WINDOW = 32;
+static constexpr uint32_t LZX_PBR_PACK_GRANULE = 16;
+static constexpr uint32_t LZX_PBR_PACK_GRANULES = 64 / LZX_PBR_PACK_GRANULE;
+
+inline uint32_t lzx_pbr_pack_tails(const uint8_t *lanes, size_t count, uint32_t max_segments, std::vector<uint32_t> &bin,
+                                   std::vector<uint8_t> &lane0)
+{
+    bin.assign(count, LZX_PBR_PACK_NONE);
+    lane0.assign(count, 0);
+    if (max_segments < 2) return 0;
+    struct Open { uint32_t id, used, segments; };
+    std::vector<Open> open;
+    std::vector<uint32_t> segments;
+    for (size_t i = 0; i < count; ++i) {
+        const uint32_t need = ((uint32_t)lanes[i] + LZX_PBR_PACK_GRANULE - 1) / LZX_PBR_PACK_GRANULE;
+        if (need == 0 || need >= LZX_PBR_PACK_GRANULES) continue;
+        size_t k = 0;
+        while (k < open.size() && (open[k].used + need > LZX_PBR_PACK_GRANULES || need > 2)) ++k;
+        if (k == open.size()) {
+            if (open.size() == LZX_PBR_PACK_WINDOW) open.erase(open.begin());
+            open.push_back(Open{(uint32_t)segments.size(), 0, 0});
+            segments.push_back(0);
+            k = open.size() - 1;
+        }
+        Open &o = open[k];
+        bin[i] = o.id;
+        lane0[i] = (uint8_t)(o.used * LZX_PBR_PACK_GRANULE);
+        o.used += need;
+        ++o.segments;
+        ++segments[o.id];
+        if (o.used == LZX_PBR_PACK_GRANULES || o.segments == max_segments) open.erase(open.begin() + (std::ptrdiff_t)k);
+    }
+    std::vector<uint32_t> renumber(segments.size(), LZX_PBR_PACK_NONE);
+    uint32_t packed = 0;
+    for (size_t b = 0; b < segments.size(); ++b)
+        if (segments[b] >= 2) renumber[b] = packed++;
+    for (size_t i = 0; i < count; ++i)
+        if (bin[i] != LZX_PBR_PACK_NONE) {
+            bin[i] = renumber[bin[i]];
+            if (bin[i] == LZX_PBR_PACK_NONE) lane0[i] = 0;
+        }
+    return packed;
+}
```

Result: no change. 1801, median of 2 (-0.1%).
